# redmod-team/SympGPR

Hardware: AMD Instinct MI355X
Metric: Gram-build GB/s + Cholesky fp64 TFLOP/s at N=65536 d=2; |alpha-alpha_ref|/|alpha_ref| (higher is better)
Workload: dtype f64

## Files before the change

include/sympgpr_probe.h:

```cpp
#ifndef SYMPGPR_PROBE_H
#define SYMPGPR_PROBE_H
#include <stddef.h>
#ifdef __cplusplus
extern "C" {
#endif

int sgpr_probe_mfma_f64(int waves_per_simd, int iters, double *tflops);
int sgpr_probe_hbm_write(size_t bytes, int reps, double *gbs);
int sgpr_probe_mfma_clock(int nacc, int waves_per_simd, int iters, double *out3);
int sgpr_probe_gemm(int m, int n, int k, int lower, double *out4);
int sgpr_probe_gemm_debug(int bits);
int sgpr_probe_leaf(double *out8);
int sgpr_probe_lat(double *out8);
int sgpr_probe_xcc(int nblocks, int *host_out);
int sgpr_probe_cumask(const unsigned *mask_words, int nwords, int nblocks, int *host_out);

int sgpr_probe_generated_eval(int family, int which, int m, const double *xa, const double *ya,
                              const double *xb, const double *yb, const double *l, int nl, double *out);

int sgpr_probe_queue_plan(int n, int nworkers, int *starts_out, int max_starts, unsigned *tasks_out, int max_tasks,
                          int *counts);
int sgpr_probe_queue_plan_partial(int n, int nworkers, int nq, int *starts_out, int max_starts, unsigned *tasks_out,
                                  int max_tasks, int *counts);
int sgpr_probe_queue_trace_begin(int max_tasks);
int sgpr_probe_queue_trace_end(unsigned long long *out, int max_tasks);
int sgpr_probe_queue_trace_clear(void);
int sgpr_probe_queue_postmortem(int always);
int sgpr_probe_queue_force_giveup(int on);
int sgpr_probe_tune(const char *name, double value);
int sgpr_probe_strassen_plan(int m, int n, int k, int lower, long smin, long kslab, long scratch_doubles, long long *out,
                             int max_records, int *count);
int sgpr_probe_gemm_strassen_dev(int m, int n, int k, double alpha, const double *A, size_t lda, const double *B, size_t ldb,
                                 double beta, double *C, size_t ldc, int lower, void *stream);
int sgpr_probe_gemm_nt2_dev(int m, int n, int k, double alpha, const double *A, size_t lda, const double *B, size_t ldb,
                            double beta, double *C, size_t ldc, double alpha2, double *C2, size_t ldc2, void *stream);
int sgpr_probe_strassen2_plan(int m, int n, int k, int lower, long smin, long kslab, long smin2, long kslab2, long scratch_doubles,
                              long long *out, int max_records, int *count);
int sgpr_probe_gemm_nt4_dev(int m, int n, int k, const double *A, size_t lda, const double *B, size_t ldb, double beta, int count,
                            double *const *C, const size_t *ldc, const double *alpha, void *stream);
unsigned sgpr_probe_map_calls(void);
int sgpr_probe_map_team(int ntest, int n0);

int sgpr_probe_trsm_piece(int ticket, int cap, int strips, int out[5]);
int sgpr_probe_trsm_counts(int strips, int cap, unsigned long long out[2]);

int sgpr_probe_census(int na, int threads_a, int lds_a, int spin_a, const unsigned *mask_a, int nwords_a,
                      int nb, int threads_b, int lds_b, int spin_b, const unsigned *mask_b, int nwords_b,
                      unsigned long long *host_out);

#ifdef __cplusplus
}
#endif
#endif
```

sympgpr_amd/_lib.py:

```python
import ctypes as C
import os

import numpy as np

FAMILIES = {"A": 0, "B": 1, "C": 2, "D": 3, "USER": 4}
K_KERN, K_DXDX0, K_DYDY0, K_DXDY0 = 0, 1, 2, 3
K_DLX, K_DLY = 4, 8
K_DX, K_DY, K_DX0, K_DY0, K_DXDX0DY0, K_DYDY0DY0, K_DXDY0DY0 = 16, 17, 18, 19, 20, 21, 22
G_QQ, G_PQ, G_QP, G_PP, G_ALL, G_LOWER, G_OCML, G_DLX, G_DLY = 1, 2, 4, 8, 15, 16, 32, 64, 128
FIT_LOWER_ONLY, FIT_REG, FIT_BLOCK_QQ, FIT_BLOCK_PP = 1, 4, 8, 16
MAP_WRAP_Q, MAP_WRAP_P, MAP_EXPLICIT, MAP_LOSS_NEGP = 1, 2, 4, 8
E_ARG, E_NODEVICE, E_HIP, E_NOMEM, E_STATE = -1, -2, -3, -4, -5

ABI_VERSION = 5
_dp = C.POINTER(C.c_double)
_vp = C.c_void_p


class SympGPRError(RuntimeError):
    code = None
    detail = ""


class NoDeviceError(SympGPRError):
    pass


def lib_path():
    return os.path.join(os.path.dirname(os.path.abspath(__file__)), "lib", "libsympgpr_hip.so")


SIGNATURES = {
    "sgpr_abi_version": (C.c_int, []),
    "sgpr_last_error": (C.c_char_p, []),
    "sgpr_device_count": (C.c_int, []),
    "sgpr_set_device": (C.c_int, [C.c_int]),
    "sgpr_build_k_host": (C.c_int, [C.c_int, C.c_int, C.c_int, _dp, _dp, _dp, _dp, _dp, C.c_int, _dp, C.c_size_t]),
    "sgpr_buildkreg_host": (C.c_int, [C.c_int, C.c_int, C.c_int, _dp, _dp, _dp, _dp, _dp, C.c_int, _dp, C.c_size_t]),
    "sgpr_build_dk_host": (C.c_int, [C.c_int, C.c_int, C.c_int, C.c_int, _dp, _dp, _dp, _dp, _dp, C.c_int, _dp,
                                     C.c_size_t]),
    "sgpr_build_dkreg_host": (C.c_int, [C.c_int, C.c_int, C.c_int, C.c_int, _dp, _dp, _dp, _dp, _dp, C.c_int, _dp,
                                        C.c_size_t]),
    "sgpr_build_k_nd_host": (C.c_int, [C.c_int, C.c_int, C.c_int, C.c_int, _dp, C.c_size_t, _dp, C.c_size_t, _dp,
                                       C.c_int, _dp, C.c_size_t]),
    "sgpr_kernel_eval_host": (C.c_int, [C.c_int, C.c_int, C.c_int, _dp, _dp, _dp, _dp, _dp, C.c_int, _dp]),
    "sgpr_potrf_host": (C.c_int, [C.c_int, _dp, C.c_size_t]),
    "sgpr_potrs_host": (C.c_int, [C.c_int, _dp, C.c_size_t, _dp, C.c_size_t, C.c_int]),
    "sgpr_fit_create": (C.c_int, [C.c_int, C.c_int, _dp, _dp, _dp, _dp, C.c_int, C.c_double, C.c_uint, _vp,
                                  C.POINTER(_vp)]),
    "sgpr_fit_create_nd": (C.c_int, [C.c_int, C.c_int, C.c_int, _dp, C.c_size_t, _dp, _dp, C.c_int, C.c_double,
                                     C.c_uint, _vp, C.POINTER(_vp)]),
    "sgpr_fit_set_hyp": (C.c_int, [_vp, _dp, C.c_int, C.c_double]),
    "sgpr_fit_set_targets": (C.c_int, [_vp, _dp]),
    "sgpr_fit_build": (C.c_int, [_vp]),
    "sgpr_fit_factor": (C.c_int, [_vp]),
    "sgpr_fit_solve": (C.c_int, [_vp]),
    "sgpr_fit_run": (C.c_int, [_vp]),
    "sgpr_fit_alpha": (C.c_int, [_vp, _dp]),
    "sgpr_fit_nll": (C.c_int, [_vp, _dp]),
    "sgpr_fit_ldiag": (C.c_int, [_vp, _dp]),
    "sgpr_fit_get_matrix": (C.c_int, [_vp, _dp, C.c_size_t]),
    "sgpr_fit_solve_rhs": (C.c_int, [_vp, _dp, C.c_size_t, C.c_int]),
    "sgpr_fit_solve_rhs_dev": (C.c_int, [C.c_void_p, C.c_void_p, C.c_size_t, C.c_int]),
    "sgpr_fit_predict_rows": (C.c_int, [_vp, C.c_int, _dp, _dp, _dp, _dp]),
    "sgpr_fit_nll_grad": (C.c_int, [_vp, _dp]),
    "sgpr_fit_nll_grad_terms": (C.c_int, [_vp, _dp]),
    "sgpr_fit_eig": (C.c_int, [_vp, _dp, _dp]),
    "sgpr_syev_host": (C.c_int, [C.c_int, _dp, C.c_size_t, _dp]),
    "sgpr_fit_inverse": (C.c_int, [_vp, _dp, C.c_size_t]),
    "sgpr_fit_predict_nd": (C.c_int, [_vp, C.c_int, _dp, C.c_size_t, _dp]),
    "sgpr_fit_predict_cov": (C.c_int, [_vp, C.c_int, _dp, C.c_size_t, _dp, _dp]),
    "sgpr_fit_predict_genfun": (C.c_int, [_vp, C.c_int, _dp, C.c_size_t, _dp, _dp, _dp]),
    "sgpr_fit_nll_grad_full": (C.c_int, [_vp, _dp, C.c_int]),
    "sgpr_fit_loo": (C.c_int, [_vp, _dp, _dp, _dp, _dp]),
    "sgpr_fit_stage_ms": (C.c_int, [_vp, _dp, _dp, _dp]),
    "sgpr_fit_cond_estimate": (C.c_int, [_vp, C.c_int, _dp]),
    "sgpr_fit_trim": (C.c_int, [_vp]),
    "sgpr_fit_solve_rhs_ms": (C.c_int, [_vp, _dp]),
    "sgpr_potrf_info_dev": (C.c_int, [C.c_int, _vp]),
    "sgpr_trim": (C.c_int, []),
    "sgpr_fit_device_ptrs": (C.c_int, [_vp, C.POINTER(_vp), C.POINTER(C.c_size_t), C.POINTER(_vp)]),
    "sgpr_fit_destroy": (C.c_int, [_vp]),
    "sgpr_gram_pairs_dev": (C.c_int, [C.c_int, C.c_int, C.c_int, _vp, _vp, _vp, _vp, _dp, C.c_int, _vp, _vp, _vp,
                                      _vp, C.c_size_t, C.c_long, C.c_double, C.c_uint, _vp]),
    "sgpr_gram_nd_dev": (C.c_int, [C.c_int, C.c_int, C.c_int, C.c_int, _vp, C.c_size_t, _vp, C.c_size_t, _dp, C.c_int,
                                   _vp, C.c_size_t, C.c_size_t, C.c_size_t, C.c_long, C.c_double, _vp]),
    "sgpr_gram_reg_dev": (C.c_int, [C.c_int, C.c_int, C.c_int, _vp, _vp, _vp, _vp, _dp, C.c_int, _vp, C.c_size_t,
                                    C.c_long, C.c_double, _vp]),
    "sgpr_gram_nd_sel_dev": (C.c_int, [C.c_int, C.c_int, C.c_int, C.c_int, _vp, C.c_size_t, _vp, C.c_size_t, _dp, C.c_int,
                                       _vp, C.c_size_t, C.POINTER(C.c_long), C.POINTER(C.c_long), _vp]),
    "sgpr_potrf_workspace": (C.c_size_t, [C.c_int]),
    "sgpr_potrf_inverses_bytes": (C.c_size_t, [C.c_int]),
    "sgpr_release_device_streams": (C.c_int, [C.c_int]),
    "sgpr_family_has_p": (C.c_int, [C.c_int]),
    "sgpr_potrf_dev": (C.c_int, [C.c_int, _vp, C.c_size_t, _vp, C.c_size_t, _vp, _vp]),
    "sgpr_trsm_rlt_dev": (C.c_int, [C.c_int, C.c_int, _vp, C.c_size_t, _vp, C.c_size_t, _vp, _vp]),
    "sgpr_gemm_nt_dev": (C.c_int, [C.c_int, C.c_int, C.c_int, C.c_double, _vp, C.c_size_t, _vp, C.c_size_t,
                                   C.c_double, _vp, C.c_size_t, C.c_int, C.c_long, _vp]),
    "sgpr_profile_begin": (C.c_int, []),
    "sgpr_profile_end": (C.c_int, [_dp]),
    "sgpr_profile_launches": (C.c_int, [_dp, C.c_int]),
    "sgpr_gemm_nt_bc_dev": (C.c_int, [C.c_int, C.c_int, C.c_int, C.c_double, _vp, C.c_size_t, _vp, C.c_size_t,
                                      C.c_double, _vp, C.c_size_t, C.c_int, C.c_int, C.c_int, C.c_int, C.c_int, _vp]),
    "sgpr_trsv_dev": (C.c_int, [C.c_int, _vp, C.c_size_t, _vp, _vp, C.c_int, _vp]),
    "sgpr_gemv_sub_dev": (C.c_int, [C.c_int, C.c_int, C.c_int, _vp, C.c_size_t, _vp, _vp, _vp]),
    "sgpr_gemm_nn_dev": (C.c_int, [C.c_int, C.c_int, C.c_int, C.c_double, _vp, C.c_size_t, _vp, C.c_size_t, C.c_double, _vp,
                                   C.c_size_t, _vp]),
    "sgpr_trsm_rl_dev": (C.c_int, [C.c_int, C.c_int, _vp, C.c_size_t, _vp, C.c_size_t, _vp, _vp]),
    "sgpr_copy_blocks_dev": (C.c_int, [C.c_int, C.c_int, C.c_int, _vp, C.c_size_t, C.c_size_t, _vp, C.c_size_t, C.c_size_t, _vp]),
    "sgpr_predict_rows_dev": (C.c_int, [C.c_int, C.c_int, _vp, _vp, C.c_int, _vp, _vp, _dp, C.c_int, _vp, _vp, _vp,
                                        _vp]),
    "sgpr_predict_nd_dev": (C.c_int, [C.c_int, C.c_int, C.c_int, _vp, C.c_size_t, C.c_int, _vp, C.c_size_t, _dp, C.c_int,
                                      _vp, _vp, _vp]),
    "sgpr_predict_reg_dev": (C.c_int, [C.c_int, C.c_int, _vp, _vp, C.c_int, _vp, _vp, _dp, C.c_int, _vp, _vp, _vp]),
    "sgpr_applymap_host": (C.c_int, [C.c_int, C.c_int, C.c_int, C.c_int, _dp, C.c_int, C.c_int, _dp, _dp, _dp, _dp,
                                     C.c_int, C.c_int, _dp, _dp, _dp, _dp, _dp, _dp, _dp, _dp]),
    "sgpr_applymap_sections_host": (C.c_int, [C.c_int, C.c_int, C.c_int, C.c_int, C.c_int, C.c_int, _dp, C.c_int, C.c_int, _dp, _dp,
                                              _dp, _dp, C.c_int, C.c_int, _dp, _dp, _dp, _dp, _dp, _dp, _dp, _dp]),
    "sgpr_fit_applymap_nd": (C.c_int, [_vp, C.c_int, C.c_int, C.c_int, _dp, C.c_size_t, _dp, C.c_size_t, _dp, _dp,
                                       C.POINTER(C.c_int)]),
    "sgpr_applymap_nd_host": (C.c_int, [C.c_int, C.c_int, C.c_int, C.c_int, C.c_int, _dp, C.c_int, C.c_int, _dp, C.c_size_t,
                                        _dp, _dp, C.c_size_t, _dp, C.c_size_t, _dp, _dp, C.POINTER(C.c_int)]),
    "sgpr_fit_applymap_nd_tangent": (C.c_int, [_vp, C.c_int, C.c_int, C.c_int, _dp, C.c_size_t, _dp, C.c_size_t, _dp, _dp,
                                               C.POINTER(C.c_int), _dp, _dp, _dp]),
    "sgpr_applymap_nd_tangent_host": (C.c_int, [C.c_int, C.c_int, C.c_int, C.c_int, C.c_int, _dp, C.c_int, C.c_int, _dp,
                                                C.c_size_t, _dp, _dp, C.c_size_t, _dp, C.c_size_t, _dp, _dp, C.POINTER(C.c_int),
                                                _dp, _dp, _dp]),
    "sgpr_potrs_vec_dev": (C.c_int, [C.c_int, _vp, C.c_size_t, _vp, _vp, _vp]),
    "sgpr_solve_status_dev": (C.c_int, [C.c_int, _vp, C.c_size_t, _vp, _vp]),
    "sgpr_fit_batch_max_order": (C.c_int, []),
    "sgpr_fit_batch": (C.c_int, [C.c_int, C.c_int, C.c_int, _dp, _dp, _dp, _dp, C.c_int, _dp, C.c_uint, _dp, _dp,
                                 C.POINTER(C.c_int)]),
    "sgpr_fit_batch_grad": (C.c_int, [C.c_int, C.c_int, C.c_int, _dp, _dp, _dp, _dp, C.c_int, _dp, C.c_uint, _dp, _dp, _dp,
                                      C.POINTER(C.c_int)]),
    "sgpr_fit_batch_grad_mid": (C.c_int, [C.c_int, C.c_int, C.c_int, _dp, _dp, _dp, _dp, C.c_int, _dp, C.c_uint, _dp, _dp, _dp,
                                          C.POINTER(C.c_int)]),
    "sgpr_fit_batch_loo": (C.c_int, [C.c_int, C.c_int, C.c_int, _dp, _dp, _dp, _dp, C.c_int, _dp, C.c_uint, _dp, _dp, _dp,
                                     C.POINTER(C.c_int)]),
}

PROBE_SIGNATURES = {
    "sgpr_probe_mfma_f64": (C.c_int, [C.c_int, C.c_int, _dp]),
    "sgpr_probe_mfma_clock": (C.c_int, [C.c_int, C.c_int, C.c_int, _dp]),
    "sgpr_probe_gemm": (C.c_int, [C.c_int, C.c_int, C.c_int, C.c_int, _dp]),
    "sgpr_probe_gemm_debug": (C.c_int, [C.c_int]),
    "sgpr_probe_leaf": (C.c_int, [_dp]),
    "sgpr_probe_lat": (C.c_int, [_dp]),
    "sgpr_probe_cumask": (C.c_int, [C.POINTER(C.c_uint), C.c_int, C.c_int, C.POINTER(C.c_int)]),
    "sgpr_probe_xcc": (C.c_int, [C.c_int, C.POINTER(C.c_int)]),
    "sgpr_probe_hbm_write": (C.c_int, [C.c_size_t, C.c_int, _dp]),
    "sgpr_probe_generated_eval": (C.c_int, [C.c_int, C.c_int, C.c_int, _dp, _dp, _dp, _dp, _dp, C.c_int, _dp]),
    "sgpr_probe_queue_plan": (C.c_int, [C.c_int, C.c_int, C.POINTER(C.c_int), C.c_int, C.POINTER(C.c_uint), C.c_int,
                                        C.POINTER(C.c_int)]),
    "sgpr_probe_queue_plan_partial": (C.c_int, [C.c_int, C.c_int, C.c_int, C.POINTER(C.c_int), C.c_int, C.POINTER(C.c_uint),
                                                C.c_int, C.POINTER(C.c_int)]),
    "sgpr_probe_queue_trace_begin": (C.c_int, [C.c_int]),
    "sgpr_probe_queue_trace_end": (C.c_int, [C.POINTER(C.c_ulonglong), C.c_int]),
    "sgpr_probe_queue_postmortem": (C.c_int, [C.c_int]),
    "sgpr_probe_queue_force_giveup": (C.c_int, [C.c_int]),
    "sgpr_probe_tune": (C.c_int, [C.c_char_p, C.c_double]),
    "sgpr_probe_map_calls": (C.c_uint, []),
    "sgpr_probe_map_team": (C.c_int, [C.c_int, C.c_int]),
    "sgpr_probe_trsm_piece": (C.c_int, [C.c_int, C.c_int, C.c_int, C.POINTER(C.c_int)]),
    "sgpr_probe_trsm_counts": (C.c_int, [C.c_int, C.c_int, C.POINTER(C.c_ulonglong)]),
    "sgpr_probe_queue_trace_clear": (C.c_int, []),
    "sgpr_probe_strassen_plan": (C.c_int, [C.c_int, C.c_int, C.c_int, C.c_int, C.c_long, C.c_long, C.c_long,
                                           C.POINTER(C.c_longlong), C.c_int, C.POINTER(C.c_int)]),
    "sgpr_probe_gemm_strassen_dev": (C.c_int, [C.c_int, C.c_int, C.c_int, C.c_double, C.c_void_p, C.c_size_t, C.c_void_p, C.c_size_t,
                                               C.c_double, C.c_void_p, C.c_size_t, C.c_int, C.c_void_p]),
    "sgpr_probe_gemm_nt2_dev": (C.c_int, [C.c_int, C.c_int, C.c_int, C.c_double, C.c_void_p, C.c_size_t, C.c_void_p, C.c_size_t,
                                          C.c_double, C.c_void_p, C.c_size_t, C.c_double, C.c_void_p, C.c_size_t, C.c_void_p]),
    "sgpr_probe_strassen2_plan": (C.c_int, [C.c_int, C.c_int, C.c_int, C.c_int, C.c_long, C.c_long, C.c_long, C.c_long, C.c_long,
                                            C.POINTER(C.c_longlong), C.c_int, C.POINTER(C.c_int)]),
    "sgpr_probe_gemm_nt4_dev": (C.c_int, [C.c_int, C.c_int, C.c_int, C.c_void_p, C.c_size_t, C.c_void_p, C.c_size_t, C.c_double, C.c_int,
                                          C.POINTER(C.c_void_p), C.POINTER(C.c_size_t), C.POINTER(C.c_double), C.c_void_p]),
    "sgpr_probe_census": (C.c_int, [C.c_int, C.c_int, C.c_int, C.c_int, C.POINTER(C.c_uint), C.c_int,
                                    C.c_int, C.c_int, C.c_int, C.c_int, C.POINTER(C.c_uint), C.c_int,
                                    C.POINTER(C.c_ulonglong)]),
}

_LIB = None
_PROBE = None


def load_library():
    global _LIB
    if _LIB is not None:
        return _LIB
    path = lib_path()
    if os.environ.get("SYMPGPR_NO_TORCH_PRELOAD") != "1":
        try:
            import torch
        except ImportError:
            pass
    if not os.path.exists(path):
        raise SympGPRError("%s is missing: run `python -c 'import __graft_entry__ as g; g.build()'` "
                           "(or make -C sympgpr_amd/csrc); there is no CPU fallback" % path)
    lib = C.CDLL(path)
    for name, (res, args) in SIGNATURES.items():
        fn = getattr(lib, name)
        fn.restype = res
        fn.argtypes = args
    if lib.sgpr_abi_version() != ABI_VERSION:
        raise SympGPRError("ABI version mismatch: %s is version %d, this package binds version %d -- rebuild it "
                           "(make -C sympgpr_amd/csrc)" % (path, lib.sgpr_abi_version(), ABI_VERSION))
    _LIB = lib
    import atexit
    atexit.register(_release_streams_at_exit)
    return lib


def _release_streams_at_exit():
    lib = _LIB
    if lib is None:
        return
    try:
        for dev in range(max(0, lib.sgpr_device_count())):
            lib.sgpr_release_device_streams(dev)
    except Exception:
        pass


def load_probe_library():
    global _PROBE
    if _PROBE is not None:
        return _PROBE
    load_library()
    path = os.path.join(os.path.dirname(lib_path()), "libsympgpr_probe.so")
    if not os.path.exists(path):
        raise SympGPRError("%s is missing: run make -C sympgpr_amd/csrc" % path)
    lib = C.CDLL(path)
    for name, (res, args) in PROBE_SIGNATURES.items():
        fn = getattr(lib, name)
        fn.restype = res
        fn.argtypes = args
    _PROBE = lib
    return lib


def device_count():
    return load_library().sgpr_device_count()


def check(rc, what=""):
    if rc == 0:
        return
    if rc > 0:
        raise np.linalg.LinAlgError("%d-th leading minor of the array is not positive definite" % rc)
    msg = load_library().sgpr_last_error().decode(errors="replace")
    err = (NoDeviceError(msg) if rc == E_NODEVICE else
           SympGPRError("%s failed (%d): %s" % (what or "libsympgpr_hip call", rc, msg)))
    err.code, err.detail = rc, msg
    raise err


def dptr(a):
    return a.ctypes.data_as(_dp)


def f64(a):
    return np.ascontiguousarray(np.asarray(a, dtype=np.float64))


def family_has_p(fam):
    return bool(load_library().sgpr_family_has_p(family_id(fam)))


def family_id(fam):
    if isinstance(fam, str):
        return FAMILIES[fam]
    return int(fam)
```

sympgpr_amd/csrc/chol.hip:

```cpp
#include <algorithm>
#include <cstdlib>
#include <mutex>
#include <vector>

#include "cholq.h"
#include "common.h"
#include "gemm_tile.h"
#include "leaf.h"

namespace sgpr {

namespace {

using namespace leaf;


__global__ __launch_bounds__(LT) void leaf_kernel(int nb, double *A, size_t lda, double *inv,
                                                  int *dinfo, int goff, int mode,
                                                  unsigned long long *stamps)
{
    __shared__ double s[LEAF_LDS];
    if (nb == LEAF) leaf_body(s, (int)LEAF, A, lda, inv, dinfo, goff, mode, stamps);
    else            leaf_body(s, nb, A, lda, inv, dinfo, goff, mode, stamps);
}
// ... 472 lines not shown
            __syncthreads();
        };
        auto wait_helper = [&](int cp) -> bool {
            if (!((helped >> cp) & 1u)) return true;
            idx[0] = F0 + cp * PW_MAX + g;
            return panel_wait_ge(a.flags, idx, 1, 3, a.dinfo, sh + 1, a.abort);
        };
        for (int c = 0; c + 1 < g; ++c) {
            double *X = tileptr(g, c);
            XTile x;
            CTile cd;
            if (!wait_helper(c)) return false;
            asm volatile("s_waitcnt vmcnt(0)" ::: "memory");
            __syncthreads();
            trsm_prefetch(X, a.lda, x);
            diag_prefetch(tileptr(g, g), a.lda, cd);
            idx[0] = E0 + c;
            if (!panel_wait(a.flags, idx, 1, a.dinfo, sh + 1, a.abort)) return false;
            trsm_solve(s, tileptr(c, c), a.inv + (size_t)c * LEAF * LEAF, a.lda, x);
            trsm_store(X, a.lda, x);
            panel_publish_wt(a.flags + F0 + g * PW_MAX + c);
            diag_update_global(s, x, cd, tileptr(g, g), a.lda);
            if (c == 0 && a.NH > 0) claim_tiles();
            int cnt = 0;
            for (int cc = c + 1; cc < g; ++cc)
                if (!((helped >> cc) & 1u)) idx[cnt++] = F0 + cc * PW_MAX + c;
            if (cnt && !panel_wait(a.flags, idx, cnt, a.dinfo, sh + 1, a.abort)) return false;
            for (int t = 1; t < g - c; ++t)
                if (!((helped >> (c + t)) & 1u))
                    panel_product(s, -1.0, X, a.lda, tileptr(c + t, c), a.lda, 1.0, tileptr(g, c + t), a.lda);
        }
        if (g > 0) {
            const int c = g - 1;
            double *X = tileptr(g, c);
            XTile x;
            CTile cd;
            if (!wait_helper(c)) return false;
            asm volatile("s_waitcnt vmcnt(0)" ::: "memory");
            __syncthreads();
            trsm_prefetch(X, a.lda, x);
            diag_prefetch(tileptr(g, g), a.lda, cd);
            idx[0] = E0 + c;
            if (dbg) a.dbg[16 * g + 2] = __builtin_amdgcn_s_memrealtime();
            if (!panel_wait(a.flags, idx, 1, a.dinfo, sh + 1, a.abort)) return false;
            if (dbg) a.dbg[16 * g + 0] = __builtin_amdgcn_s_memrealtime();
            trsm_solve(s, tileptr(c, c), a.inv + (size_t)c * LEAF * LEAF, a.lda, x, a.dbg ? a.dbg + 16 * g + 6 : nullptr);
            trsm_store(X, a.lda, x);
            if (dbg) a.dbg[16 * g + 1] = __builtin_amdgcn_s_memrealtime();
            diag_update_into_leaf(s, x, cd, a.dbg ? a.dbg + 16 * g + 8 : nullptr);
            if (tid == 0) __hip_atomic_store((gint *)(a.flags + F0 + g * PW_MAX + c), 1, __ATOMIC_RELAXED, __HIP_MEMORY_SCOPE_AGENT);
        }
        asm volatile("s_waitcnt vmcnt(0)" ::: "memory");
        __syncthreads();
        if (dbg) a.dbg[16 * g + 4] = __builtin_amdgcn_s_memrealtime();
        leaf_body(s, (int)LEAF, tileptr(g, g), a.lda,
                  a.inv + (size_t)g * LEAF * LEAF, a.dinfo, a.goff + g * LEAF, (int)LEAF_FACTOR, nullptr,
                  a.flags + E0 + g, g > 0, dbg ? a.dbg + 16 * g + 11 : nullptr);
        panel_publish(a.flags + 2 + g);
        if (a.abort && tid == 0)
            __hip_atomic_fetch_add((gint *)(a.abort + (cholq::Q_PROG - cholq::Q_ABORT)), 1, __ATOMIC_RELAXED, __HIP_MEMORY_SCOPE_AGENT);
        if (dbg) a.dbg[16 * g + 5] = __builtin_amdgcn_s_memrealtime();
        if (cen && tid == 0) cen[2] = __builtin_amdgcn_s_memrealtime();
        return true;
    }
    if (g < W + a.NH) {
        int h = g - W, cp = 1, gg = 2;
        while (h >= W - 1 - cp) { h -= W - 1 - cp; ++cp; }
        gg = cp + 1 + h;
        int *word = a.flags + F0 + cp * PW_MAX + gg;
        if (tid == 0) sh[1] = atomicCAS(word, 0, 1);
        __syncthreads();
        const int old = sh[1];
        __syncthreads();
        if (old != 0) return true;
        if (a.ver) {
            idx[0] = ((a.ver_i0 + (gg >> 1)) * a.ver_ld + a.ver_j0 + cp) * (int)cholq::VS;
            if (!panel_wait_ge(a.ver, idx, 1, a.ver_need, a.dinfo, sh + 1, a.abort)) return false;
        }
        for (int c = 0; c < cp; ++c) {
            idx[0] = F0 + gg * PW_MAX + c;
            idx[1] = F0 + cp * PW_MAX + c;
            if (!panel_wait(a.flags, idx, 2, a.dinfo, sh + 1, a.abort)) return false;
            panel_product(s, -1.0, tileptr(gg, c), a.lda, tileptr(cp, c), a.lda, 1.0, tileptr(gg, cp), a.lda);
        }
        panel_publish_val(word, 3);
        return true;
    }
    const int gb = g - a.NH;
    if (a.tiles) {
        const int nbel = R - W, ntiles = nbel * W;
        int *const counter = a.flags + 2 * PFLAG_STRIDE - 1;
        for (;;) {
            if (tid == 0) sh[1] = atomicAdd(counter, 1);
            __syncthreads();
            const int q = sh[1];
            __syncthreads();
            if (q >= ntiles) return true;
            const int cp = q / nbel, r = W + q % nbel;
            const int pword = PFLAG_STRIDE + (r - W);
            if (a.ver) {
                idx[0] = ((a.ver_i0 + (r >> 1)) * a.ver_ld + a.ver_j0 + cp) * (int)cholq::VS;
                if (!panel_wait_ge(a.ver, idx, 1, a.ver_need, a.dinfo, sh + 1, a.abort)) return false;
            }
            for (int c = 0; c < cp; ++c) {
                idx[0] = pword;
                if (!panel_wait_ge(a.flags, idx, 1, c + 1, a.dinfo, sh + 1, a.abort)) return false;
                idx[0] = F0 + cp * PW_MAX + c;
                if (!panel_wait(a.flags, idx, 1, a.dinfo, sh + 1, a.abort)) return false;
                panel_product(s, -1.0, tileptr(r, c), a.lda, tileptr(cp, c), a.lda, 1.0, tileptr(r, cp), a.lda);
            }
            {
                double *X = tileptr(r, cp);
                XTile x;
                asm volatile("s_waitcnt vmcnt(0)" ::: "memory");
                __syncthreads();
                trsm_prefetch(X, a.lda, x);
                idx[0] = E0 + cp;
                if (!panel_wait(a.flags, idx, 1, a.dinfo, sh + 1, a.abort)) return false;
                trsm_solve(s, tileptr(cp, cp), a.inv + (size_t)cp * LEAF * LEAF, a.lda, x);
                trsm_store(X, a.lda, x);
            }
            asm volatile("s_waitcnt vmcnt(0)" ::: "memory");
            __syncthreads();
            if (tid == 0) __hip_atomic_store((gint *)(a.flags + pword), cp + 1, __ATOMIC_RELAXED, __HIP_MEMORY_SCOPE_AGENT);
            if (cp == W - 1) {
                if (a.tver) panel_publish_val(a.tver + (size_t)(a.tver_r0 + r) * cholq::VS, a.tver_val);
                if (a.abort && tid == 0)
                    __hip_atomic_fetch_add((gint *)(a.abort + (cholq::Q_PROG - cholq::Q_ABORT)), 1, __ATOMIC_RELAXED, __HIP_MEMORY_SCOPE_AGENT);
            }
        }
    }
    const int nw = G - W;
    const int r_first = W + (gb - W), r_step = nw > 0 ? nw : R;
    if (a.ver) {
        const int vi = a.ver_i0 + (r_first >> 1);
        for (int c = 0; c < W; ++c) idx[c] = (vi * a.ver_ld + a.ver_j0 + c) * (int)cholq::VS;
        if (r_first < R && !panel_wait_ge(a.ver, idx, W, a.ver_need, a.dinfo, sh + 1, a.abort)) return false;
    }
    const bool below_early = a.below_early != 0;
    for (int c = 0; c < W; ++c) {
        bool have_inv = false, have_early = false, have_rows = false;
        for (int r = r_first; r < R; r += r_step) {
            double *X = tileptr(r, c);
            if (c == W - 1 || below_early) {
                XTile x;
                asm volatile("s_waitcnt vmcnt(0)" ::: "memory");
                __syncthreads();
                trsm_prefetch(X, a.lda, x);
                if (!have_early) {
                    idx[0] = E0 + c;
                    if (!panel_wait(a.flags, idx, 1, a.dinfo, sh + 1, a.abort)) return false;
                    have_early = true;
                }
                trsm_solve(s, tileptr(c, c), a.inv + (size_t)c * LEAF * LEAF, a.lda, x);
                trsm_store(X, a.lda, x);
                if (c == W - 1) continue;
            } else {
                if (!have_inv) {
                    idx[0] = 2 + c;
                    if (!panel_wait(a.flags, idx, 1, a.dinfo, sh + 1, a.abort)) return false;
                    have_inv = true;
                }
                panel_product(s, 1.0, X, a.lda, a.inv + (size_t)c * LEAF * LEAF, (size_t)LEAF, 0.0, X, a.lda);
            }
            for (int t = 1; t <= W - 1 - c; ++t) {
                if (t == 1 && !have_rows) {
                    int cnt = 0;
                    for (int cc = c + 1; cc < W; ++cc) idx[cnt++] = F0 + cc * PW_MAX + c;
                    if (cnt && !panel_wait(a.flags, idx, cnt, a.dinfo, sh + 1, a.abort)) return false;
                    have_rows = true;
                }
                panel_product(s, -1.0, X, a.lda, tileptr(c + t, c), a.lda, 1.0, tileptr(r, c + t), a.lda);
            }
        }
    }
    if (a.tver && r_first < R) panel_publish_val(a.tver + (size_t)(a.tver_r0 + r_first) * cholq::VS, a.tver_val);
    if (a.abort && tid == 0)
        __hip_atomic_fetch_add((gint *)(a.abort + (cholq::Q_PROG - cholq::Q_ABORT)), 1, __ATOMIC_RELAXED, __HIP_MEMORY_SCOPE_AGENT);
    if (cen && tid == 0) cen[2] = __builtin_amdgcn_s_memrealtime();
    return true;
}

__global__ __launch_bounds__(LT) void panel_kernel(const PanelArgs a)
{
    __shared__ double s[LEAF * ILD];
    __shared__ int sh[2];
    static_assert(2 * tile::BK * 2 * (LEAF + tile::PAD) <= LEAF_LDS && LEAF_LDS <= LEAF * ILD, "product staging and the leaf fit the buffer");
    const int tid = threadIdx.x;
    const int W = a.W, G = a.G;
    if (tid == 0) {
        int t = -1;
        if ((blockIdx.x & 7) == 0) {
            t = atomicAdd(a.flags, 1);
            if (t >= W) t = -1;
        }
        if (t < 0) t = W + atomicAdd(a.flags + 1, 1);
        sh[0] = t;
    }
    __syncthreads();
    const int g = sh[0];
    __syncthreads();
    if (g >= G + a.NH) return;
    (void)panel_strip(a, g, s, sh);
}

struct PanelSeq {
    double *A;
    size_t lda;
    int nblk;
    int nblk_all;
    const int *pstart;
    double *inv;
    int *dinfo;
    int goff;
    int *flags;
    const int *ver;
    int ver_ld;
    int *tver;
    int *abort;
    unsigned long long *census;
    int helpers, tiles;
};

__global__ __launch_bounds__(LT) void panel_seq_kernel(const PanelSeq q)
{
    __shared__ double s[LEAF * ILD];
    __shared__ int sh[2];
    const int g = blockIdx.x;
    for (int k = 0; k < q.nblk; ++k) {
        const int k0 = q.pstart[k], w = q.pstart[k + 1] - k0, wnext = k + 1 < q.nblk_all ? q.pstart[k + 2] - q.pstart[k + 1] : 0;
        PanelArgs a{};
        a.P = q.A + k0 + (size_t)k0 * q.lda; a.lda = q.lda;
        a.W = w / LEAF;
        a.R = a.G = (w + wnext) / LEAF;
        a.below_early = q.tiles;
        a.NH = (q.helpers && a.W > 2 && a.G + (a.W - 1) * (a.W - 2) / 2 <= (int)gridDim.x) ? (a.W - 1) * (a.W - 2) / 2 : 0;
        if (q.tiles && wnext > 0 && a.W >= 2 && (int)gridDim.x - a.W - a.NH >= 1) {
            a.tiles = 1;
            a.G = a.W + min((int)gridDim.x - a.W - a.NH, (a.R - a.W) * a.W);
        }
        a.inv = q.inv + (size_t)(k0 / LEAF) * LEAF * LEAF;
        a.dinfo = q.dinfo; a.goff = q.goff + k0;
        a.flags = q.flags + (size_t)(k0 / LEAF) * PFLAG_STRIDE;
        a.dbg = nullptr;
        a.ver = q.ver; a.ver_ld = q.ver_ld; a.ver_i0 = k0 / cholq::TM; a.ver_j0 = k0 / cholq::TN; a.ver_need = k0 / LEAF;
        a.tver = q.tver; a.tver_r0 = k0 / LEAF; a.tver_val = (k0 + w) / LEAF;
        a.abort = q.abort;
        a.census = (q.census && k < (int)cholq::TRACE_PANELS) ? q.census + 4 * cholq::TRACE_PANEL_WGS * (size_t)k : nullptr;
        if (g < a.G + a.NH && !panel_strip(a, g, s, sh)) return;
        asm volatile("s_waitcnt vmcnt(0)" ::: "memory");
        __syncthreads();
    }
}

struct PanelBatch {
    double *A;
    size_t stride_a, lda;
    double *inv;
    size_t stride_inv;
    int *flags;
    int *info;
    int *ticket;
    int W, nbatch;
    int R;
    int k0;
    int G;
};

__global__ __launch_bounds__(LT) void panel_batch_kernel(const PanelBatch q)
{
    __shared__ double s[LEAF * ILD];
    __shared__ int sh[2];
    if (threadIdx.x == 0) sh[0] = atomicAdd(q.ticket, 1);
    __syncthreads();
    const int t = sh[0];
    __syncthreads();
    const int p = t / q.G, g = t - p * q.G;
    if (p >= q.nbatch) return;
    PanelArgs a{};
    a.P = q.A + (size_t)p * q.stride_a + (size_t)q.k0 + (size_t)q.k0 * q.lda; a.lda = q.lda;
    a.W = q.W; a.R = q.R; a.G = q.G;
    a.inv = q.inv + (size_t)p * q.stride_inv + (size_t)(q.k0 / (int)LEAF) * LEAF * LEAF;
    a.dinfo = q.info + p; a.goff = q.k0;
    a.flags = q.flags + (size_t)p * PFLAG_STRIDE;
    a.below_early = 1;
    (void)panel_strip(a, g, s, sh);
}

inline int split(int n)
{
    int n1 = ((n / 2 + LEAF - 1) / LEAF) * LEAF;
    if (n1 >= n) n1 -= LEAF;
    return n1;
}

struct Ctx {
    double *inv;
    int *dinfo;
    hipStream_t st;
    int la_max = 0;
    int *flags = nullptr;
    void *qws = nullptr;
    bool strassen = false;
};

int potrf_lookahead(int n, double *A, size_t lda, const Ctx &c, int nb, int off0);
inline int la_block(int n) { return n <= 4096 ? 256 : (n <= 24576 ? 512 : (n <= 40960 ? 1024 : 2048)); }

int trsm_rec(int m, int n, const double *L, size_t ldl, double *B, size_t ldb, int off, const Ctx &c)
{
    if (n <= LEAF) {
        return gemm_nt(m, n, n, 1.0, B, ldb, c.inv + (size_t)(off / LEAF) * LEAF * LEAF, LEAF, 0.0,
                       B, ldb, 0, 0, c.st);
    }
    const int n1 = split(n), n2 = n - n1;
    int rc = trsm_rec(m, n1, L, ldl, B, ldb, off, c);
    if (rc) return rc;
    if (c.strassen) rc = gemm_nt_strassen(m, n2, n1, -1.0, B, ldb, L + n1, ldl, 1.0, B + (size_t)n1 * ldb, ldb, 0, c.st);
    else            rc = gemm_nt(m, n2, n1, -1.0, B, ldb, L + n1, ldl, 1.0, B + (size_t)n1 * ldb, ldb, 0, 0, c.st);
    if (rc) return rc;
    return trsm_rec(m, n2, L + n1 + (size_t)n1 * ldl, ldl, B + (size_t)n1 * ldb, ldb, off + n1, c);
}

int trsm_rl_rec(int m, int n, const double *L, size_t ldl, double *B, size_t ldb, int off, const Ctx &c)
{
    if (n <= LEAF)
        return gemm_nn(m, n, n, 1.0, B, ldb, c.inv + (size_t)(off / LEAF) * LEAF * LEAF, LEAF, 0.0, B, ldb, c.st);
    const int n1 = split(n), n2 = n - n1;
    int rc = trsm_rl_rec(m, n2, L + n1 + (size_t)n1 * ldl, ldl, B + (size_t)n1 * ldb, ldb, off + n1, c);
    if (rc) return rc;
    rc = gemm_nn(m, n1, n2, -1.0, B + (size_t)n1 * ldb, ldb, L + n1, ldl, 1.0, B, ldb, c.st);
    if (rc) return rc;
    return trsm_rl_rec(m, n1, L, ldl, B, ldb, off, c);
}

int potrf_rec(int n, double *A, size_t lda, int off, const Ctx &c)
{
    if (n <= LEAF) {
        hipLaunchKernelGGL(leaf_kernel, dim3(1), dim3(LT), 0, c.st, n, A, lda,
                           c.inv + (size_t)(off / LEAF) * LEAF * LEAF, c.dinfo, off, (int)LEAF_FACTOR,
                           (unsigned long long *)nullptr);
        SGPR_CHECK_LAUNCH();
        return 0;
    }
    if (n > 4 * LEAF && n <= c.la_max) return potrf_lookahead(n, A, lda, c, 0, off);
    const int n1 = split(n), n2 = n - n1;
    double *A21 = A + n1, *A22 = A + n1 + (size_t)n1 * lda;
    int rc = potrf_rec(n1, A, lda, off, c);
    if (rc) return rc;
    rc = trsm_rec(n2, n1, A, lda, A21, lda, off, c);
    if (rc) return rc;
    if (c.strassen) rc = gemm_nt_strassen(n2, n2, n1, -1.0, A21, lda, A21, lda, 1.0, A22, lda, 1, c.st);
    else            rc = gemm_nt(n2, n2, n1, -1.0, A21, lda, A21, lda, 1.0, A22, lda, 1, 0, c.st);
    if (rc) return rc;
    return potrf_rec(n2, A22, lda, off + n1, c);
}

int trsv_n_rec(int n, const double *L, size_t ldl, double *b, int off, const Ctx &c)
{
    if (n <= LEAF) {
        hipLaunchKernelGGL(leaf_matvec_kernel, dim3(1), dim3(MV_T), 0, c.st, n,
                           c.inv + (size_t)(off / LEAF) * LEAF * LEAF, b, 0);
        SGPR_CHECK_LAUNCH();
        return 0;
    }
    if (n <= TRSV_BLOCK) {
        hipLaunchKernelGGL(trsv_block_kernel, dim3(1), dim3(MV_T), 0, c.st, n, L, ldl,
                           c.inv + (size_t)(off / LEAF) * LEAF * LEAF, b, 0);
        SGPR_CHECK_LAUNCH();
        return 0;
    }
    const int n1 = split(n), n2 = n - n1;
    int rc = trsv_n_rec(n1, L, ldl, b, off, c);
    if (rc) return rc;
    rc = gemv_n_sub(n2, n1, L + n1, ldl, b, b + n1, c.st);
    if (rc) return rc;
    return trsv_n_rec(n2, L + n1 + (size_t)n1 * ldl, ldl, b + n1, off + n1, c);
}

int trsv_t_rec(int n, const double *L, size_t ldl, double *b, int off, const Ctx &c)
{
    if (n <= LEAF) {
        hipLaunchKernelGGL(leaf_matvec_kernel, dim3(1), dim3(MV_T), 0, c.st, n,
                           c.inv + (size_t)(off / LEAF) * LEAF * LEAF, b, 1);
        SGPR_CHECK_LAUNCH();
        return 0;
    }
    if (n <= TRSV_BLOCK) {
        hipLaunchKernelGGL(trsv_block_kernel, dim3(1), dim3(MV_T), 0, c.st, n, L, ldl,
                           c.inv + (size_t)(off / LEAF) * LEAF * LEAF, b, 1);
        SGPR_CHECK_LAUNCH();
        return 0;
    }
    const int n1 = split(n), n2 = n - n1;
    int rc = trsv_t_rec(n2, L + n1 + (size_t)n1 * ldl, ldl, b + n1, off + n1, c);
    if (rc) return rc;
    rc = gemv_t_sub(n2, n1, L + n1, ldl, b + n1, b, c.st);
    if (rc) return rc;
    return trsv_t_rec(n1, L, ldl, b, off, c);
}

int leaves_invert_only(int n, double *L, size_t ldl, const Ctx &c)
{
    for (int off = 0; off < n; off += LEAF) {
        const int nb = n - off < LEAF ? n - off : LEAF;
        hipLaunchKernelGGL(leaf_kernel, dim3(1), dim3(LT), 0, c.st, nb, L + off + (size_t)off * ldl, ldl,
                           c.inv + (size_t)(off / LEAF) * LEAF * LEAF, c.dinfo, off,
                           (int)LEAF_INVERT_ONLY, (unsigned long long *)nullptr);
        SGPR_CHECK_LAUNCH();
    }
    return 0;
}

inline size_t inv_bytes(int n)
{
    return (size_t)((n + LEAF - 1) / LEAF) * LEAF * LEAF * sizeof(double);
}
inline size_t flag_bytes(int n)
{
    return (((size_t)((n + LEAF - 1) / LEAF) * PFLAG_STRIDE * sizeof(int)) + 255) / 256 * 256;
}


}

inline size_t pub_bytes(int n) { return ((size_t)2 * n * sizeof(double) + 255) / 256 * 256; }
size_t potrf_workspace(int n) { return n <= 0 ? 256 : inv_bytes(n) + flag_bytes(n) + pub_bytes(n) + cholq::ws_bytes(n) + 256; }

namespace {

struct EventPool {
    std::vector<hipEvent_t> ev;
    size_t top = 0;
};
thread_local EventPool t_event_pool[64];

struct EventSet {
    std::vector<hipEvent_t> ev;
    EventPool *pool = nullptr;
    size_t base = 0;
    int create(size_t count)
    {
        int dev = 0;
        SGPR_HIP(hipGetDevice(&dev));
        if (dev < 0 || dev >= 64) { set_error("potrf: device index out of range"); return SGPR_E_ARG; }
        pool = &t_event_pool[dev];
        base = pool->top;
        while (pool->ev.size() < base + count) {
            hipEvent_t e = nullptr;
            SGPR_HIP(hipEventCreateWithFlags(&e, hipEventDisableTiming));
            pool->ev.push_back(e);
        }
        pool->top = base + count;
        ev.assign(pool->ev.begin() + (long)base, pool->ev.begin() + (long)(base + count));
        return 0;
    }
    ~EventSet()
    {
        if (pool) pool->top = base;
    }
};
struct StreamJoin {
    hipStream_t side, caller;
    hipEvent_t ev;
    ~StreamJoin()
    {
        if (hipEventRecord(ev, side) != hipSuccess || hipStreamWaitEvent(caller, ev, 0) != hipSuccess)
            (void)hipStreamSynchronize(side);
        gemm_set_overlap(0);
    }
};

hipStream_t g_side[64] = {};
std::mutex g_side_mu;

void release_all_streams_at_exit();
void register_exit_release()
{
    static std::once_flag once;
    std::call_once(once, [] { (void)atexit(release_all_streams_at_exit); });
}

int side_stream(hipStream_t caller, hipStream_t *out, int *dev_out)
{
    hipStream_t *const side = g_side;
    int dev = -1;
    if (caller) {
        SGPR_HIP(hipStreamGetDevice(caller, &dev));
    } else {
        SGPR_HIP(hipGetDevice(&dev));
    }
    if (dev < 0 || dev >= 64) { set_error("potrf: device index out of range"); return SGPR_E_ARG; }
    std::lock_guard<std::mutex> lock(g_side_mu);
    if (!side[dev]) {
        int cur = -1, lo = 0, hi = 0;
        SGPR_HIP(hipGetDevice(&cur));
        if (cur != dev) SGPR_HIP(hipSetDevice(dev));
        hipError_t e = hipDeviceGetStreamPriorityRange(&lo, &hi);
        if (e == hipSuccess) e = hipStreamCreateWithPriority(&side[dev], hipStreamNonBlocking, hi);
        if (e == hipSuccess) register_exit_release();
        if (cur != dev) (void)hipSetDevice(cur);
        SGPR_HIP(e);
    }
    *out = side[dev];
    *dev_out = dev;
    return 0;
}

struct QueueDevice {
    std::mutex mu;
    hipEvent_t done = nullptr;
    int ncu = 0;
    hipStream_t workers[4] = {}, panels[4] = {};
    bool overlap_ok[4] = {};
    bool failed = false;
};
QueueDevice g_qdev[64];

__global__ void overlap_probe_kernel(int *w, int me)
{
    __hip_atomic_store((gint *)(w + me), 1, __ATOMIC_RELAXED, __HIP_MEMORY_SCOPE_AGENT);
    const unsigned long long t0 = __builtin_amdgcn_s_memrealtime();
    int seen = 0;
    while (!(seen = __hip_atomic_load((gint *)(w + 1 - me), __ATOMIC_RELAXED, __HIP_MEMORY_SCOPE_AGENT))) {
        __builtin_amdgcn_s_sleep(32);
        if (__builtin_amdgcn_s_memrealtime() - t0 > 5000000ull) break;
    }
    w[2 + me] = seen ? 1 : 2;
}
static bool queue_overlap_ok(hipStream_t sw, hipStream_t sp)
{
    int *w = nullptr;
    if (hipMalloc((void **)&w, 4 * sizeof(int)) != hipSuccess) { (void)hipGetLastError(); return false; }
    int h[4] = {0, 0, 0, 0};
    bool ok = hipMemset(w, 0, sizeof(h)) == hipSuccess;
    if (ok) {
        hipLaunchKernelGGL(overlap_probe_kernel, dim3(1), dim3(1), 0, sp, w, 0);
        hipLaunchKernelGGL(overlap_probe_kernel, dim3(1), dim3(1), 0, sw, w, 1);
        ok = hipGetLastError() == hipSuccess && hipStreamSynchronize(sp) == hipSuccess && hipStreamSynchronize(sw) == hipSuccess &&
             hipMemcpy(h, w, sizeof(h), hipMemcpyDeviceToHost) == hipSuccess && h[2] == 1 && h[3] == 1;
    }
    (void)hipFree(w);
    (void)hipGetLastError();
    return ok;
}

int queue_streams(QueueDevice &qd, int dev, int R, hipStream_t *sw, hipStream_t *sp)
{
    if (!qd.workers[R - 1]) {
        int cur = -1;
        SGPR_HIP(hipGetDevice(&cur));
        if (cur != dev) SGPR_HIP(hipSetDevice(dev));
        const int words = qd.ncu / 32;
        std::vector<uint32_t> mp((size_t)words, 0u), mw((size_t)words, 0xFFFFFFFFu);
        for (int b = 0; b < 8 * R; ++b) { mp[b / 32] |= 1u << (b % 32); mw[b / 32] &= ~(1u << (b % 32)); }
        hipError_t e = hipExtStreamCreateWithCUMask(&qd.panels[R - 1], (uint32_t)words, mp.data());
        if (e == hipSuccess) e = hipExtStreamCreateWithCUMask(&qd.workers[R - 1], (uint32_t)words, mw.data());
        if (e == hipSuccess) register_exit_release();
        if (cur != dev) (void)hipSetDevice(cur);
        if (e != hipSuccess) {
            (void)hipGetLastError();
            qd.failed = true;
            return SGPR_E_HIP;
        }
    }
    if (!qd.overlap_ok[R - 1]) {
        if (!queue_overlap_ok(qd.workers[R - 1], qd.panels[R - 1])) {
            qd.failed = true;
            return SGPR_E_HIP;
        }
        qd.overlap_ok[R - 1] = true;
    }
    *sw = qd.workers[R - 1];
    *sp = qd.panels[R - 1];
    return 0;
}

thread_local bool t_last_potrf_used_queue = false;

int potrf_queue(int n, double *A, size_t lda, const Ctx &c, int off0)
{
    int dev = -1;
    if (c.st) {
        SGPR_HIP(hipStreamGetDevice(c.st, &dev));
    } else {
        SGPR_HIP(hipGetDevice(&dev));
    }
    if (dev < 0 || dev >= 64) { set_error("potrf: device index out of range"); return SGPR_E_ARG; }
    QueueDevice &qd = g_qdev[dev];
    std::lock_guard<std::mutex> lock(qd.mu);
    if (qd.failed) return 1;
    if (!qd.ncu) {
        SGPR_HIP(hipDeviceGetAttribute(&qd.ncu, hipDeviceAttributeMultiprocessorCount, dev));
        SGPR_HIP(hipEventCreateWithFlags(&qd.done, hipEventDisableTiming));
        SGPR_HIP(hipEventRecord(qd.done, c.st));
    }
    if (qd.ncu % 64 != 0 || qd.ncu < 64) { qd.failed = true; return 1; }
    const std::vector<int> starts = cholq::default_starts(n);
    int band = 0;
    for (size_t k = 0; k + 1 < starts.size(); ++k)
        band = std::max(band, (starts[k + 1] - starts[k] + (k + 2 < starts.size() ? starts[k + 2] - starts[k + 1] : 0)) / LEAF);
    static const int q_helpers = (int)tune("q_helpers", 0), q_tiles = (int)tune("q_tiles", 0);
    int nh_max = 0;
    for (size_t k = 0; k + 1 < starts.size(); ++k) {
        const int W = (starts[k + 1] - starts[k]) / LEAF;
        if (q_helpers && W > 2) nh_max = std::max(nh_max, (W - 1) * (W - 2) / 2);
    }
    const int pgrid = band + nh_max + std::max(0, q_tiles);
    const int R = (pgrid + 7) / 8;
    if (R > 4) return 1;
    hipStream_t sw = nullptr, sp = nullptr;
    if (queue_streams(qd, dev, R, &sw, &sp)) return 1;
    static const int qslack = (int)tune("q_slack", 0);
    const int nworkers = qd.ncu - 8 * R - std::max(0, std::min(qslack, 64));
    const cholq::Plan *plan = cholq::get_plan(n, nworkers);
    if (!plan) return 1;
    const cholq::Ws ws = cholq::carve(c.qws, n);
    const hipStream_t su = c.st;
    int rc;
    SGPR_HIP(hipStreamWaitEvent(su, qd.done, 0));
    if ((rc = cholq::prepare(*plan, ws, su))) return rc;
    if (cholq::forced_giveup()) {
        static const int k_timeout = POTRF_HANDOFF_TIMEOUT;
        SGPR_HIP(hipMemcpyAsync(c.dinfo, &k_timeout, sizeof(int), hipMemcpyHostToDevice, su));
    }
    EventSet es;
    if ((rc = es.create(3))) return rc;
    const int tn = n / cholq::TN;
    double *inv_blk = c.inv + (size_t)(off0 / LEAF) * LEAF * LEAF;
    int *flags_blk = c.flags + (size_t)(off0 / LEAF) * PFLAG_STRIDE;
    {
        SGPR_HIP(hipEventRecord(es.ev[0], su));
        SGPR_HIP(hipStreamWaitEvent(sp, es.ev[0], 0));
        SGPR_HIP(hipStreamWaitEvent(sw, es.ev[0], 0));
        StreamJoin join_p{sp, su, es.ev[1]};
        StreamJoin join_w{sw, su, es.ev[2]};
        PanelSeq ps{};
        ps.A = A; ps.lda = lda; ps.nblk = plan->nq; ps.nblk_all = plan->nblk; ps.pstart = ws.pstart;
        ps.inv = inv_blk; ps.dinfo = c.dinfo; ps.goff = off0; ps.flags = flags_blk;
        ps.ver = ws.ver; ps.ver_ld = tn; ps.tver = ws.tver; ps.abort = cholq::abort_word(ws);
        ps.census = cholq::trace_panel_base((int)(plan->tasks.size() / 2));
        ps.helpers = q_helpers != 0; ps.tiles = q_tiles > 0;
        t_last_potrf_used_queue = true;
        hipLaunchKernelGGL(panel_seq_kernel, dim3(pgrid), dim3(LT), 0, sp, ps);
        SGPR_CHECK_LAUNCH();
        if ((rc = cholq::launch_workers(*plan, ws, A, lda, inv_blk, flags_blk, c.dinfo, PFLAG_STRIDE, sw))) return rc;
    }
    SGPR_HIP(hipEventRecord(qd.done, su));
    cholq::remember(ws, n, (int)(plan->tasks.size() / 2));
    cholq::remember_plan(plan);
    static const bool qdebug = tune("q_debug", 0) != 0;
    if (qdebug) {
        SGPR_HIP(hipStreamSynchronize(su));
        cholq::postmortem(false);
    }
    if (plan->nq < plan->nblk) {
        const int S = plan->starts[plan->nq];
        Ctx ct = c;
        ct.qws = nullptr;
        static const bool nosync = tune("q_nosync", 0) != 0;
        if (!nosync) SGPR_HIP(hipStreamSynchronize(su));
        return potrf_lookahead(n - S, A + S + (size_t)S * lda, lda, ct, 0, off0 + S);
    }
    return 0;
}

void release_all_streams_at_exit()
{
    int ndev = 0;
    if (hipGetDeviceCount(&ndev) != hipSuccess) { (void)hipGetLastError(); return; }
    for (int dev = 0; dev < ndev && dev < 64; ++dev) {
        hipStream_t drop[9] = {};
        int nd = 0;
        {
            std::lock_guard<std::mutex> lock(g_side_mu);
            if (g_side[dev]) { drop[nd++] = g_side[dev]; g_side[dev] = nullptr; }
        }
        {
            QueueDevice &qd = g_qdev[dev];
            std::lock_guard<std::mutex> lock(qd.mu);
            for (int r = 0; r < 4; ++r) {
                if (qd.workers[r]) { drop[nd++] = qd.workers[r]; qd.workers[r] = nullptr; }
                if (qd.panels[r]) { drop[nd++] = qd.panels[r]; qd.panels[r] = nullptr; }
            }
            qd.failed = true;
        }
        if (!nd) continue;
        int cur = -1;
        (void)hipGetDevice(&cur);
        if (cur != dev) (void)hipSetDevice(dev);
        for (int q = 0; q < nd; ++q) (void)hipStreamDestroy(drop[q]);
        if (cur != dev && cur >= 0) (void)hipSetDevice(cur);
    }
    (void)hipGetLastError();
}

int release_streams(int dev)
{
    {
        bool any = false;
        {
            std::lock_guard<std::mutex> lock(g_side_mu);
            any = g_side[dev] != nullptr;
        }
        QueueDevice &qd = g_qdev[dev];
        std::lock_guard<std::mutex> lock(qd.mu);
        for (int r = 0; r < 4; ++r) any = any || qd.workers[r] || qd.panels[r];
        any = any || qd.done;
        if (!any) return 0;
    }
    int cur = -1;
    SGPR_HIP(hipGetDevice(&cur));
    if (cur != dev) SGPR_HIP(hipSetDevice(dev));
    hipError_t first = hipSuccess;
    auto drop = [&](hipStream_t &s) {
        if (!s) return;
        hipError_t e = hipStreamSynchronize(s);
        if (e == hipSuccess) e = hipStreamDestroy(s);
        if (e != hipSuccess && first == hipSuccess) first = e;
        s = nullptr;
    };
    {
        std::lock_guard<std::mutex> lock(g_side_mu);
        drop(g_side[dev]);
    }
    {
        QueueDevice &qd = g_qdev[dev];
        std::lock_guard<std::mutex> lock(qd.mu);
        for (int r = 0; r < 4; ++r) { drop(qd.workers[r]); drop(qd.panels[r]); }
        if (qd.done) {
            const hipError_t e = hipEventDestroy(qd.done);
            if (e != hipSuccess && first == hipSuccess) first = e;
            qd.done = nullptr;
        }
        qd.ncu = 0;
        qd.failed = false;
        for (int r = 0; r < 4; ++r) qd.overlap_ok[r] = false;
    }
    if (cur != dev) (void)hipSetDevice(cur);
    SGPR_HIP(first);
    return 0;
}

int potrf_lookahead(int n, double *A, size_t lda, const Ctx &c, int nb, int off0)
{
    if (nb == 0 && c.qws && c.flags && cholq::eligible(n) && (lda & 1) == 0 && (((uintptr_t)A & 15) == 0) && off0 % LEAF == 0) {
        const int rq = potrf_queue(n, A, lda, c, off0);
        if (rq <= 0) return rq;
    }
    hipStream_t sp = nullptr;
    {
        int dev = -1;
        const int rc0 = side_stream(c.st, &sp, &dev);
        if (rc0) return rc0;
    }
    static const int pmode = (int)tune("la_panel", 3);
    const bool fused_cap = pmode == 3 && c.flags && n % LEAF == 0 && (lda & 1) == 0 && (((uintptr_t)A & 15) == 0) &&
                           off0 % LEAF == 0;
    std::vector<int> starts;
    {
        static const int t0_env = (int)tune("la_t0", 0);
        const int t0 = t0_env > 0 ? t0_env : (n >= 24576 ? 12288 : 1 << 30);
        static const int t1 = (int)tune("la_t1", 6144);
        static const int t2 = (int)tune("la_t2", 2048);
        for (int pos = 0; pos < n;) {
            starts.push_back(pos);
            const int rem = n - pos;
            int w = nb > 0 ? nb : (rem > t0 ? 2048 : (rem > t1 ? 1024 : (rem > t2 ? 512 : 256)));
            if (nb == 0 && !fused_cap) w = la_block(n);
            pos += std::min(w, rem);
        }
        starts.push_back(n);
    }
    const int nblk = (int)starts.size() - 1;
    int wmax = 0;
    for (int k = 0; k < nblk; ++k) wmax = std::max(wmax, starts[k + 1] - starts[k]);
    EventSet es;
    {
        const int rc0 = es.create(3 * (size_t)nblk + 3);
        if (rc0) return rc0;
    }
    std::vector<hipEvent_t> &ev = es.ev;
    const hipStream_t su = c.st;
    Ctx cp{c.inv, c.dinfo, sp, 0, c.flags};
    const bool fused_ok = fused_cap && wmax % LEAF == 0 && wmax / LEAF <= PW_MAX;
    const bool left = pmode != 2, right_in = pmode == 0 || pmode == 3;
    auto panel = [&](int k) -> int {
        const int k0 = starts[k], w = starts[k + 1] - k0, rows = n - k0, below = rows - w;
        double *Akk = A + k0 + (size_t)k0 * lda;
        if (fused_ok) {
            PanelArgs pa{};
            pa.P = Akk; pa.lda = lda;
            pa.R = rows / LEAF; pa.W = w / LEAF;
            const int nbelow = pa.R - pa.W;
            const double m_u2 = (double)(rows + w);
            const double u2_us = k > 0 ? m_u2 * m_u2 * (starts[k] - starts[k - 1]) / 55e6 : 0.0;
            static const double split_ratio = tune("panel_split_ratio", 3.0);
            const bool split = nbelow > 0 && k > 0 && u2_us > split_ratio * (125.0 * pa.W + 100.0);
            if (split) {
                pa.R = pa.W;
                pa.G = pa.W;
            } else {
                const double strip_us = 30.0 * (pa.W * (pa.W + 1) / 2 + pa.W), chain_us = 125.0 * pa.W;
                int per_wg = (int)((0.7 * u2_us - 0.5 * chain_us) / strip_us);
                per_wg = std::max(1, std::min(per_wg, 4));
                const int nwg = std::min((nbelow + per_wg - 1) / per_wg, PANEL_G_MAX - pa.W);
                pa.G = pa.W + (nbelow > 0 ? std::max(1, nwg) : 0);
            }
            static const bool helpers_on = tune("panel_helpers", 1) != 0, below_early_on = tune("panel_below_early", 1) != 0;
            pa.NH = helpers_on && pa.W > 2 ? (pa.W - 1) * (pa.W - 2) / 2 : 0;
            if (pa.G + pa.NH > PANEL_G_MAX) pa.NH = 0;
            pa.below_early = below_early_on ? 1 : 0;
            static const bool tiles_on = tune("panel_tiles", 1) != 0;
            static const double tile_mult = tune("panel_tile_mult", 1.0);
            if (tiles_on && !split && nbelow > 0 && pa.W >= 2 && nbelow < PFLAG_STRIDE) {
                const double chain_us = 60.0 * pa.W + 50.0;
                int nt = u2_us < chain_us ? nbelow * pa.W : (int)(tile_mult * (pa.G - pa.W));
                nt = std::max(1, std::min(std::min(nt, nbelow * pa.W), PANEL_G_MAX - pa.W - pa.NH));
                pa.tiles = 1;
                pa.G = pa.W + nt;
            }
            const int t0 = (off0 + k0) / LEAF;
            pa.inv = cp.inv + (size_t)t0 * LEAF * LEAF;
            pa.dinfo = cp.dinfo; pa.goff = off0 + k0;
            pa.flags = c.flags + (size_t)t0 * PFLAG_STRIDE;
            pa.dbg = (PANEL_DBG && g_panel_dbg) ? g_panel_dbg + (size_t)16 * t0 : nullptr;
            hipLaunchKernelGGL(panel_kernel, dim3(std::max(pa.G + pa.NH, 8 * (pa.W - 1) + 1)), dim3(LT), 0, sp, pa);
            SGPR_CHECK_LAUNCH();
            if (split) return trsm_rec(below, w, Akk, lda, Akk + w, lda, off0 + k0, cp);
            return 0;
        }
        if (!left) {
            int rc = potrf_rec(w, Akk, lda, off0 + k0, cp);
            if (rc) return rc;
            if (below > 0) rc = trsm_rec(below, w, Akk, lda, Akk + w, lda, off0 + k0, cp);
            return rc;
        }
        for (int c0 = 0; c0 < w; c0 += LEAF) {
            const int nj = std::min((int)LEAF, w - c0), mrows = rows - c0;
            double *Pj = Akk + c0 + (size_t)c0 * lda;
            int rc;
            if (!right_in && c0 > 0 &&
                (rc = gemm_nt(mrows, nj, c0, -1.0, Akk + c0, lda, Akk + c0, lda, 1.0, Pj, lda, 0, 0, sp)))
                return rc;
            double *invj = cp.inv + (size_t)((off0 + k0 + c0) / LEAF) * LEAF * LEAF;
            hipLaunchKernelGGL(leaf_kernel, dim3(1), dim3(LT), 0, sp, nj, Pj, lda, invj, cp.dinfo, off0 + k0 + c0,
                               (int)LEAF_FACTOR, (unsigned long long *)nullptr);
            SGPR_CHECK_LAUNCH();
            if (mrows > nj && (rc = gemm_nt(mrows - nj, nj, nj, 1.0, Pj + nj, lda, invj, LEAF, 0.0, Pj + nj, lda, 0, 0, sp)))
                return rc;
            const int ncols = w - c0 - nj;
            if (right_in && ncols > 0 &&
                (rc = gemm_nt(mrows - nj, ncols, nj, -1.0, Pj + nj, lda, Pj + nj, lda, 1.0, Pj + nj + (size_t)nj * lda, lda, 1, 0, sp)))
                return rc;
        }
        return 0;
    };
    int rc;
    SGPR_HIP(hipEventRecord(ev[2 * nblk], su));
    SGPR_HIP(hipStreamWaitEvent(sp, ev[2 * nblk], 0));
    StreamJoin join{sp, su, ev[2 * nblk + 1]};
    gemm_set_overlap(1);
    if ((rc = panel(0))) return rc;
    SGPR_HIP(hipEventRecord(ev[0], sp));
    for (int k = 0; k < nblk; ++k) {
        const int k0 = starts[k], w = starts[k + 1] - k0;
        const int k1 = k0 + w;
        if (k1 >= n) break;
        const int w1 = starts[k + 2] - k1, k2 = k1 + w1;
        const double *Lk = A + (size_t)k0 * lda;
        if (k > 0) SGPR_HIP(hipStreamWaitEvent(sp, ev[2 * (k - 1) + 1], 0));
        if ((rc = gemm_nt(n - k1, w1, w, -1.0, Lk + k1, lda, Lk + k1, lda, 1.0, A + k1 + (size_t)k1 * lda, lda, 1, 0, sp)))
            return rc;
        const double u2_us = (double)(n - k2) * (n - k2) * w / 55e6;
        const bool chain_bound = u2_us < 1.5 * (125.0 * (w1 / LEAF) + 100.0);
        if (chain_bound) SGPR_HIP(hipEventRecord(ev[2 * nblk + 2 + k], sp));
        if ((rc = panel(k + 1))) return rc;
        SGPR_HIP(hipEventRecord(ev[2 * (k + 1)], sp));
        SGPR_HIP(hipStreamWaitEvent(su, chain_bound ? ev[2 * nblk + 2 + k] : ev[2 * k], 0));
        if (k2 < n &&
            (rc = gemm_nt(n - k2, n - k2, w, -1.0, Lk + k2, lda, Lk + k2, lda, 1.0, A + k2 + (size_t)k2 * lda, lda, 1, 0, su)))
            return rc;
        SGPR_HIP(hipEventRecord(ev[2 * k + 1], su));
    }
    return 0;
}

}

size_t potrf_batch_flag_bytes(int nbatch) { return ((size_t)nbatch * PFLAG_STRIDE + 1) * sizeof(int); }
int potrf_batch_max_order() { return PW_MAX * (int)LEAF; }

int potrf_batch(int nbatch, int npad, double *A, size_t stride_a, size_t lda, double *inv, size_t stride_inv, int *flags,
                int *info, hipStream_t st)
{
    if (nbatch < 0 || npad <= 0 || npad % LEAF != 0 || npad > PW_MAX * (int)LEAF || lda < (size_t)npad || (lda & 1) != 0 ||
        ((uintptr_t)A & 15) != 0 || (stride_a & 1) != 0) {
        set_error("potrf_batch: bad order / leading dimension / alignment");
        return SGPR_E_ARG;
    }
    if (nbatch == 0) return 0;
    SGPR_HIP(hipMemsetAsync(info, 0, (size_t)nbatch * sizeof(int), st));
    return potrf_batch_panel(nbatch, npad, 0, npad / (int)LEAF, A, stride_a, lda, inv, stride_inv, flags, info, st);
}

int potrf_batch_panel(int nbatch, int npad, int k0, int Wd, double *A, size_t stride_a, size_t lda, double *inv, size_t stride_inv,
                      int *flags, int *info, hipStream_t st)
{
    const int R = (npad - k0) / (int)LEAF;
    if (nbatch <= 0 || k0 < 0 || k0 % LEAF != 0 || Wd < 1 || Wd > PW_MAX || Wd > R || R > PANEL_G_MAX) {
        set_error("potrf_batch_panel: bad panel");
        return SGPR_E_ARG;
    }
    SGPR_HIP(hipMemsetAsync(flags, 0, potrf_batch_flag_bytes(nbatch), st));
    const int below_max = (int)tune("batch_below", 0);
    const int below = R - Wd <= 0 ? 0 : (below_max > 0 && below_max < R - Wd ? below_max : R - Wd);
    PanelBatch q{A, stride_a, lda, inv, stride_inv, flags, info, flags + (size_t)nbatch * PFLAG_STRIDE, Wd, nbatch, R, k0, Wd + below};
    hipLaunchKernelGGL(panel_batch_kernel, dim3((unsigned)(nbatch * (Wd + below))), dim3(LT), 0, st, q);
    SGPR_CHECK_LAUNCH();
    return 0;
}

bool potrf_queue_mark_failed(hipStream_t st)
{
    const bool used = t_last_potrf_used_queue;
    if (!used) return false;
    int dev = -1;
    if ((st ? hipStreamGetDevice(st, &dev) : hipGetDevice(&dev)) != hipSuccess || dev < 0 || dev >= 64) { (void)hipGetLastError(); return false; }
    QueueDevice &qd = g_qdev[dev];
    std::lock_guard<std::mutex> lock(qd.mu);
    qd.failed = true;
    return true;
}

int potrf_trim()
{
    for (int dev = 0; dev < 64; ++dev) {
        EventPool &p = t_event_pool[dev];
        if (p.ev.empty() || p.top != 0) continue;
        for (hipEvent_t e : p.ev) (void)hipEventDestroy(e);
        p.ev.clear();
    }
    (void)hipGetLastError();
    return strassen_trim();
}

int release_device_streams(int dev)
{
    if (dev < 0 || dev >= 64) { set_error("release_device_streams: device index out of range"); return SGPR_E_ARG; }
    return release_streams(dev);
}

int potrf(int n, double *A, size_t lda, void *work, size_t lwork, int *dinfo, hipStream_t st)
{
    if (n < 0 || (n > 0 && lda < (size_t)n)) { set_error("potrf: bad n / lda"); return SGPR_E_ARG; }
    if (lwork < potrf_workspace(n)) { set_error("potrf: workspace too small"); return SGPR_E_ARG; }
    SGPR_HIP(hipMemsetAsync(dinfo, 0, sizeof(int), st));
    if (n == 0) return 0;
    int *flags = reinterpret_cast<int *>(static_cast<char *>(work) + inv_bytes(n));
    SGPR_HIP(hipMemsetAsync(flags, 0, flag_bytes(n), st));
    static const int mode = [] { const char *e = getenv("SGPR_POTRF"); return !e ? 0 : (e[0] == 'r' ? 1 : 2); }();
    static const int nb_env = [] { const char *e = getenv("SGPR_POTRF_NB"); return e ? atoi(e) : 0; }();
    static const int la_max_env = [] { const char *e = getenv("SGPR_LA_MAX"); return (int)tune("la_max", e ? atoi(e) : 57344); }();
    t_last_potrf_used_queue = false;
    Ctx c{static_cast<double *>(work), dinfo, st, mode == 1 ? 0 : la_max_env, flags};
    if (cholq::ws_bytes(n) > 0) c.qws = static_cast<char *>(work) + inv_bytes(n) + flag_bytes(n) + pub_bytes(n);
    c.strassen = true;
    if (n > c.la_max && n > LEAF) {
        const int n1 = split(n), n2 = n - n1, n11 = split(n1);
        auto need = [&](int levels) {
            return std::max(strassen_scratch_doubles(n2, n2, n1, 1, levels), strassen_scratch_doubles(n2, n1 - n11, n11, 0, levels));
        };
        strassen_reserve(need(2), need(1), st);
    }
    const bool dbg = PANEL_DBG && getenv("SGPR_PANEL_DBG") != nullptr;
    const int T = (n + LEAF - 1) / LEAF;
    if (dbg) {
        (void)hipMalloc((void **)&g_panel_dbg, sizeof(unsigned long long) * 16 * T);
        (void)hipMemset(g_panel_dbg, 0, sizeof(unsigned long long) * 16 * T);
    }
    int rc;
    if (mode == 2 || (nb_env > 0 && mode == 0 && n > 4 * LEAF && n <= c.la_max))
        rc = potrf_lookahead(n, A, lda, c, nb_env > 0 ? nb_env : 0, 0);
    else
        rc = potrf_rec(n, A, lda, 0, c);
    if (dbg) {
        (void)hipStreamSynchronize(st);
        std::vector<unsigned long long> h(16 * (size_t)T);
        (void)hipMemcpy(h.data(), g_panel_dbg, h.size() * 8, hipMemcpyDeviceToHost);
        (void)hipFree(g_panel_dbg);
        g_panel_dbg = nullptr;
        std::vector<double> d[9];
        for (int t = 1; t + 1 < T; ++t) {
            const unsigned long long *p = &h[16 * t], *q = &h[16 * (t + 1)];
            if (!p[0] || !p[5] || !q[0]) continue;
            d[0].push_back((p[1] - p[0]) * 0.01);
            d[1].push_back((p[2] - p[1]) * 0.01);
            d[2].push_back((p[3] - p[2]) * 0.01);
            d[3].push_back((p[4] - p[3]) * 0.01);
            d[4].push_back(((double)q[0] - (double)p[4]) * 0.01);
            d[5].push_back((p[5] - p[4]) * 0.01);
            d[3].back() = ((double)p[4] - (double)p[1]) * 0.01;
            d[1].back() = (p[6] - p[0]) * 0.01;
            d[2].back() = (p[7] - p[6]) * 0.01;
            d[6].push_back((p[11] - p[4]) * 0.01);
            d[7].push_back((p[12] - p[11]) * 0.01);
            d[8].push_back(((double)q[2] - (double)p[4]) * 0.01);
            if (getenv("SGPR_PANEL_DBG_ALL"))
                fprintf(stderr, "  col %3d: leaf entry -> factor %.1f -> flag %.1f | next strip at wait %.1f, saw E %.1f | its solve %.1f, update %.1f\n", t,
                        (p[11] - p[4]) * 0.01, (p[12] - p[4]) * 0.01, ((double)q[2] - (double)p[4]) * 0.01, ((double)q[0] - (double)p[4]) * 0.01,
                        (q[1] - q[0]) * 0.01, ((double)q[4] - (double)q[1]) * 0.01);
        }
        auto med = [](std::vector<double> &x) { std::sort(x.begin(), x.end()); return x.empty() ? 0.0 : x[x.size() / 2]; };
        fprintf(stderr, "panel chain n=%d (%zu columns): E seen -> solve stored %.1f | E seen -> staged %.1f | -> MFMA part done %.1f | (solve stored -> leaf entry %.1f) | "
                "leaf entry -> next E seen %.1f (factor %.1f, -> flag set %.1f; next strip at its wait %.1f) | whole leaf %.1f us\n", n, d[0].size(), med(d[0]), med(d[1]), med(d[2]), med(d[3]), med(d[4]),
                med(d[6]), med(d[7]), med(d[8]), med(d[5]));
    }
    return rc;
}

int trsm_rlt(int m, int n, const double *L, size_t ldl, double *B, size_t ldb, const void *work,
             hipStream_t st)
{
    if (m <= 0 || n <= 0) return 0;
    Ctx c{const_cast<double *>(static_cast<const double *>(work)), nullptr, st};
    return trsm_rec(m, n, L, ldl, B, ldb, 0, c);
}

static bool use_strips(int n, const double *L, size_t ldl)
{
    static const bool off = [] { const char *e = getenv("SGPR_TRSV"); return e && e[0] == 'r'; }();
    return !off && n > TRSV_BLOCK && trsv_strips_ok(n, L, ldl);
}
static int *solve_state(int n, const void *work)
{
    return reinterpret_cast<int *>(const_cast<char *>(static_cast<const char *>(work)) + inv_bytes(n));
}
static double *solve_pub(int n, const void *work)
{
    return reinterpret_cast<double *>(const_cast<char *>(static_cast<const char *>(work)) + inv_bytes(n) + flag_bytes(n));
}

bool trsv_uses_strips(int n, const double *L, size_t ldl) { return use_strips(n, L, ldl); }

int solve_status(int n, const double *L, size_t ldl, const void *work, hipStream_t st)
{
    if (n <= 0 || !use_strips(n, L, ldl)) { SGPR_HIP(hipStreamSynchronize(st)); return 0; }
    int h[8] = {};
    SGPR_HIP(hipMemcpyAsync(h, solve_state(n, work), sizeof(h), hipMemcpyDeviceToHost, st));
    SGPR_HIP(hipStreamSynchronize(st));
    if (h[2] || h[6]) { set_error("triangular solve: a hand-off between strips timed out"); return SGPR_E_HIP; }
    return 0;
}
const int *trsv_state(int n, const void *work) { return solve_state(n, work); }

int potrs_vec(int n, const double *L, size_t ldl, void *work, double *b, hipStream_t st)
{
    if (n <= 0) return 0;
    Ctx c{const_cast<double *>(static_cast<const double *>(work)), nullptr, st};
    if (use_strips(n, L, ldl)) {
        int *state = solve_state(n, work);
        double *pub = solve_pub(n, work);
        SGPR_HIP(hipMemsetAsync(state, 0, 8 * sizeof(int), st));
        SGPR_HIP(hipMemsetAsync(pub, 0xFF, (size_t)2 * n * sizeof(double), st));
        int rc = trsv_strips(n, L, ldl, c.inv, b, 0, state, pub, st);
        if (rc) return rc;
        return trsv_strips(n, L, ldl, c.inv, b, 1, state + 4, pub + n, st);
    }
    int rc = trsv_n_rec(n, L, ldl, b, 0, c);
    if (rc) return rc;
    return trsv_t_rec(n, L, ldl, b, 0, c);
}

int trsm_rl(int m, int n, const double *L, size_t ldl, double *B, size_t ldb, const void *work, hipStream_t st)
{
    if (m <= 0 || n <= 0) return 0;
    Ctx c{const_cast<double *>(static_cast<const double *>(work)), nullptr, st};
    return trsm_rl_rec(m, n, L, ldl, B, ldb, 0, c);
}

int trsm_rlt_off(int m, int n, const double *L, size_t ldl, double *B, size_t ldb, const void *work, int off, hipStream_t st)
{
    if (m <= 0 || n <= 0) return 0;
    if (off < 0 || off % (int)LEAF) { set_error("trsm_rlt_off: offset not on a leaf boundary"); return SGPR_E_ARG; }
    Ctx c{const_cast<double *>(static_cast<const double *>(work)), nullptr, st};
    return trsm_rec(m, n, L, ldl, B, ldb, off, c);
}
int trsm_rl_off(int m, int n, const double *L, size_t ldl, double *B, size_t ldb, const void *work, int off, hipStream_t st)
{
    if (m <= 0 || n <= 0) return 0;
    if (off < 0 || off % (int)LEAF) { set_error("trsm_rl_off: offset not on a leaf boundary"); return SGPR_E_ARG; }
    Ctx c{const_cast<double *>(static_cast<const double *>(work)), nullptr, st};
    return trsm_rl_rec(m, n, L, ldl, B, ldb, off, c);
}

bool potrs_mat_uses_strips(int n, int nrhs, const double *L, size_t ldl)
{
    return nrhs >= 2 && nrhs <= 256 && use_strips(n, L, ldl) && trsm_strips_ok(n, L, ldl);
}
size_t potrs_mat_scratch(int n, int nrhs, const double *L, size_t ldl)
{
    if (n <= 0 || nrhs <= 0) return 8;
    return potrs_mat_uses_strips(n, nrhs, L, ldl) ? trsm_strips_scratch(n) : (size_t)n * nrhs * sizeof(double);
}

int potrs_mat(int n, const double *L, size_t ldl, const void *work, double *B, size_t ldb, int nrhs,
              double *scratch, hipStream_t st)
{
    if (n <= 0 || nrhs <= 0) return 0;
    if (potrs_mat_uses_strips(n, nrhs, L, ldl))
        return potrs_strips(n, L, ldl, static_cast<const double *>(work), B, ldb, nrhs, solve_state(n, work), scratch, st);
    int rc = transpose(n, nrhs, B, ldb, scratch, (size_t)nrhs, st);
    if (rc) return rc;
    if ((rc = trsm_rlt(nrhs, n, L, ldl, scratch, (size_t)nrhs, work, st))) return rc;
    if ((rc = trsm_rl(nrhs, n, L, ldl, scratch, (size_t)nrhs, work, st))) return rc;
    return transpose(nrhs, n, scratch, (size_t)nrhs, B, ldb, st);
}

int potrs_mat_fwd(int n, const double *L, size_t ldl, const void *work, double *B, size_t ldb, int nrhs,
                  double *scratch, hipStream_t st)
{
    if (n <= 0 || nrhs <= 0) return 0;
    if (potrs_mat_uses_strips(n, nrhs, L, ldl))
        return trsm_strips_fwd(n, L, ldl, static_cast<const double *>(work), B, ldb, nrhs, solve_state(n, work), scratch, st);
    int rc = transpose(n, nrhs, B, ldb, scratch, (size_t)nrhs, st);
    if (rc) return rc;
    if ((rc = trsm_rlt(nrhs, n, L, ldl, scratch, (size_t)nrhs, work, st))) return rc;
    return transpose(nrhs, n, scratch, (size_t)nrhs, B, ldb, st);
}

int trsv(int n, const double *L, size_t ldl, void *work, double *b, int trans, hipStream_t st)
{
    if (n <= 0) return 0;
    Ctx c{const_cast<double *>(static_cast<const double *>(work)), nullptr, st};
    if (use_strips(n, L, ldl)) {
        int *state = solve_state(n, work);
        double *pub = solve_pub(n, work);
        SGPR_HIP(hipMemsetAsync(state, 0, 4 * sizeof(int), st));
        SGPR_HIP(hipMemsetAsync(pub, 0xFF, (size_t)n * sizeof(double), st));
        return trsv_strips(n, L, ldl, c.inv, b, trans, state, pub, st);
    }
    return trans ? trsv_t_rec(n, L, ldl, b, 0, c) : trsv_n_rec(n, L, ldl, b, 0, c);
}

int leaf_probe(double *A, size_t lda, double *inv, int *dinfo, unsigned long long *stamps, hipStream_t st)
{
    hipLaunchKernelGGL(leaf_kernel, dim3(1), dim3(LT), 0, st, (int)LEAF, A, lda, inv, dinfo, 0, (int)LEAF_FACTOR, stamps);
    SGPR_CHECK_LAUNCH();
    return 0;
}

int leaf_inverses(int n, const double *L, size_t ldl, void *work, int *dinfo, hipStream_t st)
{
    if (n <= 0) return 0;
    Ctx c{static_cast<double *>(work), dinfo, st};
    return leaves_invert_only(n, const_cast<double *>(L), ldl, c);
}

}
```

sympgpr_amd/csrc/common.h:

```cpp
#pragma once
#include <hip/hip_runtime.h>
#include <cstddef>
#include <cstdint>
#include <string>
#include <type_traits>
#include <vector>

#include "../../include/sympgpr_hip.h"

namespace sgpr {

void set_error(const std::string &msg);
double tune(const char *name, double dflt);
void tune_set(const char *name, double v);
int hip_fail(hipError_t e, const char *what, const char *file, int line);

#define SGPR_HIP(call)                                                          \
    do {                                                                        \
        hipError_t e__ = (call);                                                \
        if (e__ != hipSuccess) return ::sgpr::hip_fail(e__, #call, __FILE__, __LINE__); \
    } while (0)

#define SGPR_CHECK_LAUNCH() SGPR_HIP(hipGetLastError())

struct KConst {
    double lx, ly, p, sig;
    double lx2, ly2;
    double inv_lx2, inv_ly2;
    double cxx, cyy, cxy;
    double hscale;
    double inv_lx, inv_ly, inv_lx3, inv_ly3;
    double gxx;
};
enum { DERIV_NONE = 0, DERIV_LX = 1, DERIV_LY = 2 };
int make_kconst(int family, const double *hyp, int nhyp, KConst *out);
bool family_has_p(int family);
int make_kconst_l(int family, const double *l, int nl, KConst *out);

template <typename F>
int dispatch_family(int family, F &&f)
{
    switch (family) {
    case SGPR_FAM_A: return f(std::integral_constant<int, SGPR_FAM_A>());
    case SGPR_FAM_B: return f(std::integral_constant<int, SGPR_FAM_B>());
    case SGPR_FAM_C: return f(std::integral_constant<int, SGPR_FAM_C>());
    case SGPR_FAM_D: return f(std::integral_constant<int, SGPR_FAM_D>());
    case SGPR_FAM_USER: return f(std::integral_constant<int, SGPR_FAM_USER>());
    }
    set_error("unknown kernel family");
    return SGPR_E_ARG;
}

int gram_pairs(int family, int mi, int mj, const double *xb, const double *yb, const double *xa,
               const double *ya, const KConst &kc, double *qq, double *Pq, double *qP, double *PP,
               size_t ld, long diag_off, double noise, unsigned flags, hipStream_t st);
int gram_reg(int family, int mi, int mj, const double *xb, const double *yb, const double *xa,
             const double *ya, const KConst &kc, double *G, size_t ld, long diag_off, double noise,
             hipStream_t st, int deriv = DERIV_NONE);
int kernel_eval(int family, int which, int m, const double *xa, const double *ya, const double *xb,
                const double *yb, const KConst &kc, double *out, hipStream_t st);
int predict_rows(int family, int m, const double *q, const double *P, int n0, const double *xtr,
                 const double *ytr, const KConst &kc, const double *alpha, double *out_p,
                 double *out_q, hipStream_t st);
int predict_reg(int family, int m, const double *q, const double *P, int n0, const double *xtr,
                const double *ytr, const KConst &kc, const double *alpha, double *out,
                hipStream_t st);

int applymap_team(int ntest, int n0);
size_t applymap_team_ws(int ntest, int n0);
int applymap(int family, int mode, int nm, int ntest, int n0, const double *xtr, const double *ytr,
             const KConst &kc, const double *alpha, int n0p, const double *xtrp, const double *ytrp,
             const KConst &kcp, const double *alphap, const double *Q0, const double *P0, double *qmap,
             double *pmap, double *pdiff, void *team_ws, hipStream_t st);
int applymap_status(const void *team_ws, int ntest, int n0);
unsigned applymap_last_calls();
int applymap_sections(int family, int mode, int nsec, int first, int nm, int ntest, int n0, const double *xtr, const double *ytr,
                      const double *alpha, const KConst *kcs, int n0p, const double *xtrp, const double *ytrp,
                      const double *alphap, const KConst *kcps, const double *Q0, const double *P0, double *qmap, double *pmap,
                      double *pdiff, hipStream_t st);

int gram_nd(int family, int d, int mi, int mj, const double *Xb, size_t ldxb, const double *Xa, size_t ldxa,
            const double *hyp, int nhyp, double *K, size_t ld, size_t rstride, size_t cstride, long diag_off,
            double noise, hipStream_t st);
int gram_nd_sel(int family, int d, int mi, int mj, const double *Xb, size_t ldxb, const double *Xa, size_t ldxa,
                const double *hyp, int nhyp, double *K, size_t ld, const long *roff, const long *coff, hipStream_t st);
int predict_nd(int family, int d, int m, const double *Xt, size_t ldxt, int n0, const double *Xtr, size_t ldxtr,
               const double *hyp, int nhyp, const double *alpha, double *out, hipStream_t st);
int applymap_nd(int family, int d, int mode, int nm, int ntest, int n0, const double *Xtr, size_t ldxtr, const double *hyp,
                int nhyp, const double *alpha, const double *Q0, const double *P0, double *qmap, double *pmap, int *iters,
                hipStream_t st);
int applymap_nd_tangent(int family, int d, int mode, int nm, int ntest, int n0, const double *Xtr, size_t ldxtr, const double *hyp,
                        int nhyp, const double *alpha, const double *Q0, const double *P0, double *qmap, double *pmap, int *iters,
                        double *jac, double *mono, double *lyap, hipStream_t st);
int genfun_nd(int family, int d, int m, const double *Xt, size_t ldxt, bool has_ref, int n0, const double *Xtr, size_t ldxtr,
              const double *hyp, int nhyp, const double *alpha, double *F, hipStream_t st);
int genfun_cross_nd(int family, int d, int mc, const double *Xt, size_t ldxt, const double *x0, size_t ldx0, int n0,
                    const double *Xtr, size_t ldxtr, const double *hyp, int nhyp, double *V, size_t ldv, double *prior,
                    size_t prior_stride, hipStream_t st);
bool family_is_sum(int family);

int gemm_nt(int m, int n, int k, double alpha, const double *A, size_t lda, const double *B,
            size_t ldb, double beta, double *C, size_t ldc, int lower, long diag_off,
            hipStream_t st);
int gemm_nt_bc(int m, int n, int k, double alpha, const double *A, size_t lda, const double *B,
               size_t ldb, double beta, double *C, size_t ldc, int lower, const int *bc5,
               hipStream_t st);
int gemm_nn(int m, int n, int k, double alpha, const double *A, size_t lda, const double *B, size_t ldb,
            double beta, double *C, size_t ldc, hipStream_t st);
int gemm_nt_two(int m, int n, int k, double alpha, const double *A, size_t lda, const double *B, size_t ldb, double beta,
             double *C, size_t ldc, double alpha2, double *C2, size_t ldc2, hipStream_t st);
constexpr int STRASSEN_REC = 16;
enum { PLAN_SUM = 1, PLAN_PROD = 2, PLAN_CLASSIC = 3 };
int gemm_nt_strassen(int m, int n, int k, double alpha, const double *A, size_t lda, const double *B, size_t ldb, double beta,
                     double *C, size_t ldc, int lower, hipStream_t st);
int strassen_plan(int m, int n, int k, int lower, long smin, long kslab, size_t scratch_doubles, std::vector<long long> &out);
enum { PLAN2_SUM = 4, PLAN2_PROD = 5 };
int strassen_outer_plan(int m, int n, int k, int lower, long smin, long kslab, long smin2, long kslab2, size_t scratch_doubles,
                   std::vector<long long> &out);
int gemm_nt_multi(int m, int n, int k, const double *A, size_t lda, const double *B, size_t ldb, double beta, int count,
                  double *const *C, const size_t *ldc, const double *alpha, hipStream_t st);
size_t strassen_scratch_doubles(int m, int n, int k, int lower, int levels);
void strassen_reserve(size_t both, size_t one, hipStream_t st);
int strassen_trim();
int gemm_profile_begin();
int gemm_profile_end(double *out12);
int gemm_profile_launches(double *buf, int max_records);
void gemm_set_overlap(int on);
int gemm_nt_diag(int m, int n, int k, double alpha, const double *A, size_t lda, const double *B, size_t ldb,
                 double beta, double *C, size_t ldc, int lower, unsigned long long *stamps, int dbg, hipStream_t st);

constexpr int LEAF = 128;
constexpr int POTRF_HANDOFF_TIMEOUT = -1000001;
constexpr int SOLVE_HANDOFF_TIMEOUT = -1000002;
inline int info_status(int info)
{
    if (info >= 0) return info;
    set_error(info == POTRF_HANDOFF_TIMEOUT ? "potrf: a hand-off inside the panel kernel timed out"
              : info == SOLVE_HANDOFF_TIMEOUT ? "solve: a hand-off between the strips of a triangular solve timed out" : "potrf: internal error");
    return SGPR_E_HIP;
}
size_t potrf_workspace(int n);
int potrf(int n, double *A, size_t lda, void *work, size_t lwork, int *dinfo, hipStream_t st);
size_t potrf_batch_flag_bytes(int nbatch);
int potrf_batch_max_order();
int potrf_batch(int nbatch, int npad, double *A, size_t stride_a, size_t lda, double *inv, size_t stride_inv, int *flags,
                int *info, hipStream_t st);
int potrf_batch_panel(int nbatch, int npad, int k0, int Wd, double *A, size_t stride_a, size_t lda, double *inv, size_t stride_inv,
                      int *flags, int *info, hipStream_t st);
bool potrf_queue_mark_failed(hipStream_t st);
int release_device_streams(int dev);
int trsm_rlt(int m, int n, const double *L, size_t ldl, double *B, size_t ldb, const void *work,
             hipStream_t st);
int potrs_vec(int n, const double *L, size_t ldl, void *work, double *b, hipStream_t st);
int solve_status(int n, const double *L, size_t ldl, const void *work, hipStream_t st);
int trsm_rl(int m, int n, const double *L, size_t ldl, double *B, size_t ldb, const void *work, hipStream_t st);
int trsm_rlt_off(int m, int n, const double *L, size_t ldl, double *B, size_t ldb, const void *work, int off, hipStream_t st);
int trsm_rl_off(int m, int n, const double *L, size_t ldl, double *B, size_t ldb, const void *work, int off, hipStream_t st);
int potrs_mat(int n, const double *L, size_t ldl, const void *work, double *B, size_t ldb, int nrhs, double *scratch,
              hipStream_t st);
int potrs_mat_fwd(int n, const double *L, size_t ldl, const void *work, double *B, size_t ldb, int nrhs, double *scratch,
                  hipStream_t st);
size_t potrs_mat_scratch(int n, int nrhs, const double *L, size_t ldl);
bool potrs_mat_uses_strips(int n, int nrhs, const double *L, size_t ldl);
int trsv(int n, const double *L, size_t ldl, void *work, double *b, int trans, hipStream_t st);
bool trsv_uses_strips(int n, const double *L, size_t ldl);
const int *trsv_state(int n, const void *work);
int leaf_probe(double *A, size_t lda, double *inv, int *dinfo, unsigned long long *stamps, hipStream_t st);
int leaf_inverses(int n, const double *L, size_t ldl, void *work, int *dinfo, hipStream_t st);

bool trsv_strips_ok(int n, const double *L, size_t ldl);
int trsv_strips(int n, const double *L, size_t ldl, const double *inv, double *b, int trans, int *state ,
                double *pub , hipStream_t st);
int trsv_strips_batch(int nbatch, int n, const double *L, size_t sL, size_t ldl, const double *inv, size_t sInv, double *b, size_t sB,
                      int trans, int *state, int sState, double *pub, hipStream_t st);

constexpr int TRSM_YLD = 80;
constexpr int TRSM_FOLD = 5;
constexpr int TRSM_STATE_INTS = 16;
bool trsm_strips_ok(int n, const double *L, size_t ldl);
void trsm_piece_of(int u, int C, int T, int out[5]);
void trsm_piece_counts(int T, int C, size_t out[2]);
size_t trsm_strips_scratch(int n);
int potrs_strips(int n, const double *L, size_t ldl, const double *inv, double *B, size_t ldb, int nrhs, int *state ,
                 double *scratch, hipStream_t st);
int trsm_strips_fwd(int n, const double *L, size_t ldl, const double *inv, double *B, size_t ldb, int nrhs, int *state,
                    double *scratch, hipStream_t st);

constexpr int POSTCOV_COLS = 256;
size_t postcov_partial_doubles(int n, int D, int mc);
int postcov(int D, int n, int mc, const double *V, size_t ldv, const double *Kss, size_t ldk, double *part, double *cov,
            hipStream_t st);

size_t nll_grad_full_scratch(int n, int N, int nacc);
int nll_grad_full(int family, int d, bool reg, int N, int n, const double *L, size_t ldl, const void *work, const double *X,
                  const double *alpha, const double *l, const double *pp, int nacc, double *scratch, double *out,
                  hipStream_t st);

int kyinv_panel_width(int n, const char *knob);
int kyinv_row_panel(int n, int J, int rows, const double *L, size_t ldl, const void *work, double *R, size_t ldr, hipStream_t st);

struct LooLayout { size_t panel, blocks, part, resid, cov, lpd, sums, total; };
LooLayout loo_layout(int n, int N, int D);
int fit_loo(int D, int N, int n, const double *L, size_t ldl, const void *work, const double *alpha, double *scratch,
            hipStream_t st);

int fit_batch_max_order();
int fit_batch_trim();
int potrf_trim();
int fit_batch(int family, int nbatch, int npts, const double *x, const double *y, const double *z, const double *hyp,
              int nhyp, const double *sig2n, unsigned flags, double *alpha, double *nll, int *info);
int fit_batch_grad_max_order();
int fit_batch_grad(int family, int nbatch, int npts, const double *x, const double *y, const double *z, const double *hyp,
                   int nhyp, const double *sig2n, unsigned flags, double *alpha, double *nll, double *grad, int *info);
int fit_batch_grad_mid(int family, int nbatch, int npts, const double *x, const double *y, const double *z, const double *hyp,
                       int nhyp, const double *sig2n, unsigned flags, double *alpha, double *nll, double *grad, int *info);
int fit_batch_loo(int family, int nbatch, int npts, const double *x, const double *y, const double *z, const double *hyp,
                  int nhyp, const double *sig2n, unsigned flags, double *alpha, double *nll, double *loo, int *info);

int zero_strict_upper(int n, double *A, size_t lda, hipStream_t st);
int sym_fill_upper(int n, double *A, size_t lda, hipStream_t st);
int nll_reduce(int n, const double *L, size_t ldl, const double *z, const double *alpha,
               double *dout , hipStream_t st);
int copy_diag(int n, const double *A, size_t lda, double *d, hipStream_t st);
int dot(int n, const double *a, const double *b, double *out, hipStream_t st);
constexpr int SUMSQ_SCRATCH = 1024;
int syev_jacobi(int n, double *A, size_t lda, double *V, size_t ldv, double *w_host, int max_sweeps,
                int *sweeps_done, hipStream_t st);
int sumsq(size_t count, const double *a, double *part, double *out, hipStream_t st);
int trace(int n, const double *A, size_t lda, double *out, hipStream_t st);
int transpose(int m, int n, const double *A, size_t lda, double *B, size_t ldb, hipStream_t st);
int gemv_n_sub(int m, int k, const double *A, size_t lda, const double *x, double *y,
               hipStream_t st);
int gemv_t_sub(int m, int k, const double *A, size_t lda, const double *x, double *y,
               hipStream_t st);

}
```

sympgpr_amd/csrc/gemm_f64.hip:

```cpp
#include <algorithm>
#include <atomic>
#include <cstdlib>
#include <mutex>
#include <type_traits>
#include <vector>

#include "common.h"
#include "gemm_tile.h"

namespace sgpr {

namespace {

struct ProfRec { double flop; int big; int m, n, k, lower, overlap; };
struct Prof {
    std::mutex mu;
    std::atomic<bool> on{false};
    std::vector<hipEvent_t> pool;
    std::vector<ProfRec> recs;
    long dropped = 0;
};
constexpr int PROF_POOL = 8192;
Prof g_prof;
thread_local int t_overlap = 0;

using namespace tile;

template <int BM, int BN>
__global__ __launch_bounds__(64 * (BM / 64) * (BN / 64), (BM >= 128 ? 2 : 1)) void gemm_nt_kernel(const GemmArgs g)
{
    constexpr int LDA_S = BM + PAD, LDB_S = BN + PAD;
    constexpr int STAGES = (BM == 256 && BN == 128) ? SGPR_GEMM_STAGES : 2;
    __shared__ double smem[STAGES * BK * (LDA_S + LDB_S)];
    int tile_r, tile_c;
    if (!tile_of<(SR * BM) / (4 * BN)>(g, tile_r, tile_c)) return;
    const int row0 = tile_r * BM, col0 = tile_c * BN;
    if (g.lower) {
        const long rb = ((long)min(row0 + BM, g.m) - 1) / g.lblk, cb = (long)col0 / g.lblk;
        if (rb * g.lpr + g.lpi < cb * g.lpc + g.lpj) return;
    }
    const bool aligned = ((((uintptr_t)g.A | (uintptr_t)g.B) & 15) == 0) && (((g.lda | g.ldb) & 1) == 0);
    const bool fast = aligned && (row0 + BM <= g.m) && (col0 + BN <= g.n) && (g.k % BK == 0);
    if (g.transb) {
        if (fast) gemm_body<BM, BN, true, true>(g, smem, tile_r, tile_c);
        else      gemm_body<BM, BN, false, true>(g, smem, tile_r, tile_c);
        return;
    }
    if constexpr (BM % 128 == 0) {
        if (fast && !(g.dbg & 16)) { gemm_body_dma<BM, BN, STAGES>(g, smem, tile_r, tile_c); return; }
    }
    if (fast) gemm_body<BM, BN, true>(g, smem, tile_r, tile_c);
    else      gemm_body<BM, BN, false>(g, smem, tile_r, tile_c);
}

__global__ __launch_bounds__(512, 2) void gemm_nt2_kernel(const GemmArgs g)
{
    constexpr int BM = 256, BN = 128, LDA_S = BM + PAD, LDB_S = BN + PAD;
    __shared__ double smem[SGPR_GEMM_STAGES * BK * (LDA_S + LDB_S)];
    int tile_r, tile_c;
    if (!tile_of<(SR * BM) / (4 * BN)>(g, tile_r, tile_c)) return;
    const int row0 = tile_r * BM, col0 = tile_c * BN;
    const bool aligned = ((((uintptr_t)g.A | (uintptr_t)g.B) & 15) == 0) && (((g.lda | g.ldb) & 1) == 0);
    const bool fast = aligned && (row0 + BM <= g.m) && (col0 + BN <= g.n) && (g.k % BK == 0);
    if (fast) gemm_body_dma<BM, BN, SGPR_GEMM_STAGES, true>(g, smem, tile_r, tile_c);
    else      gemm_body<BM, BN, false, false, true>(g, smem, tile_r, tile_c);
}

__global__ __launch_bounds__(512, 2) void gemm_nt4_kernel(const GemmArgs g)
{
    constexpr int BM = 256, BN = 128, LDA_S = BM + PAD, LDB_S = BN + PAD;
    __shared__ double smem[SGPR_GEMM_STAGES * BK * (LDA_S + LDB_S)];
    int tile_r, tile_c;
    if (!tile_of<(SR * BM) / (4 * BN)>(g, tile_r, tile_c)) return;
    const int row0 = tile_r * BM, col0 = tile_c * BN;
    const bool aligned = ((((uintptr_t)g.A | (uintptr_t)g.B) & 15) == 0) && (((g.lda | g.ldb) & 1) == 0);
    const bool fast = aligned && (row0 + BM <= g.m) && (col0 + BN <= g.n) && (g.k % BK == 0);
    if (fast) gemm_body_dma<BM, BN, SGPR_GEMM_STAGES, false, true>(g, smem, tile_r, tile_c);
    else      gemm_body<BM, BN, false, false, false, true>(g, smem, tile_r, tile_c);
}

struct Dst { double *C; size_t ld; double alpha; };

__global__ __launch_bounds__(256) void block_sum_kernel(int rows, int cols, const double *X, size_t ldx, const double *Y, size_t ldy,
                                                        double sign, double *T)
{
    const int nrc = (rows + 511) / 512, ncg = (cols + 3) / 4;
    const long pieces = (long)nrc * ncg;
    for (long p = blockIdx.x; p < pieces; p += gridDim.x) {
        const int cg = (int)(p / nrc), rc = (int)(p - (long)cg * nrc);
        const int r = rc * 512 + 2 * (int)threadIdx.x;
        if (r >= rows) continue;
        double2_t x[4], y[4];
#pragma unroll
        for (int u = 0; u < 4; ++u) {
            const int c = min(cg * 4 + u, cols - 1);
            x[u] = *reinterpret_cast<const double2_t *>(X + (size_t)r + (size_t)c * ldx);
            y[u] = *reinterpret_cast<const double2_t *>(Y + (size_t)r + (size_t)c * ldy);
        }
#pragma unroll
        for (int u = 0; u < 4; ++u) {
            const int c = cg * 4 + u;
            if (c < cols) *reinterpret_cast<double2_t *>(T + (size_t)r + (size_t)c * (size_t)rows) = x[u] + sign * y[u];
        }
    }
}

}

int gemm_nt(int m, int n, int k, double alpha, const double *A, size_t lda, const double *B,
            size_t ldb, double beta, double *C, size_t ldc, int lower, long diag_off,
            hipStream_t st)
{
    const int bc[5] = {1, 1, (int)diag_off, 1, 0};
    return gemm_nt_bc(m, n, k, alpha, A, lda, B, ldb, beta, C, ldc, lower, bc, st);
}

static int gemm_launch(int m, int n, int k, double alpha, const double *A, size_t lda, const double *B,
                       size_t ldb, double beta, double *C, size_t ldc, int lower, const int *bc, int transb,
                       hipStream_t st, unsigned long long *stamps = nullptr, int dbg = 0, const Dst *x = nullptr, int nx = 0,
                       bool k4 = false);

static int gemm_chunked(int m, int n, int k, double alpha, const double *A, size_t lda, const double *B,
                        size_t ldb, double beta, double *C, size_t ldc, int lower, const int *bc,
                        hipStream_t st, const Dst *x, int nx, bool k4)
{
    static const int kmax = [] { const char *e = getenv("SGPR_GEMM_KMAX"); return e ? atoi(e) : 8192; }();
    if (kmax >= 128 && k > kmax) {
        const int nchunk = (k + kmax - 1) / kmax;
        const int step = ((k + nchunk - 1) / nchunk + 127) / 128 * 128;
        for (int k0 = 0; k0 < k; k0 += step) {
            const int rc = gemm_launch(m, n, std::min(step, k - k0), alpha, A + (size_t)k0 * lda, lda, B + (size_t)k0 * ldb, ldb,
                                       k0 == 0 ? beta : 1.0, C, ldc, lower, bc, 0, st, nullptr, 0, x, nx, k4);
            if (rc) return rc;
        }
        return 0;
    }
    return gemm_launch(m, n, k, alpha, A, lda, B, ldb, beta, C, ldc, lower, bc, 0, st, nullptr, 0, x, nx, k4);
}

int gemm_nt_bc(int m, int n, int k, double alpha, const double *A, size_t lda, const double *B,
               size_t ldb, double beta, double *C, size_t ldc, int lower, const int *bc,
               hipStream_t st)
{
    return gemm_chunked(m, n, k, alpha, A, lda, B, ldb, beta, C, ldc, lower, bc, st, nullptr, 0, false);
}

int gemm_nt_two(int m, int n, int k, double alpha, const double *A, size_t lda, const double *B, size_t ldb, double beta,
             double *C, size_t ldc, double alpha2, double *C2, size_t ldc2, hipStream_t st)
{
    const int bc[5] = {1, 1, 0, 1, 0};
    if (!C2) { set_error("gemm_nt_two: null second destination"); return SGPR_E_ARG; }
    const Dst x{C2, ldc2, alpha2};
    return gemm_chunked(m, n, k, alpha, A, lda, B, ldb, beta, C, ldc, 0, bc, st, &x, 1, false);
}

int gemm_nt_multi(int m, int n, int k, const double *A, size_t lda, const double *B, size_t ldb, double beta, int count,
                  double *const *C, const size_t *ldc, const double *alpha, hipStream_t st)
{
    const int bc[5] = {1, 1, 0, 1, 0};
    if (count < 2 || count > 4 || !C || !ldc || !alpha) { set_error("gemm_nt_multi: 2 to 4 destinations"); return SGPR_E_ARG; }
    Dst x[3];
    for (int d = 0; d < count; ++d) {
        if (!C[d]) { set_error("gemm_nt_multi: null destination"); return SGPR_E_ARG; }
        if (d) x[d - 1] = Dst{C[d], ldc[d], alpha[d]};
    }
    return gemm_chunked(m, n, k, alpha[0], A, lda, B, ldb, beta, C[0], ldc[0], 0, bc, st, x, count - 1, true);
}

static int gemm_launch(int m, int n, int k, double alpha, const double *A, size_t lda, const double *B,
                       size_t ldb, double beta, double *C, size_t ldc, int lower, const int *bc, int transb,
                       hipStream_t st, unsigned long long *stamps, int dbg, const Dst *x, int nx, bool k4)
{
    const bool plain = bc[0] == 1 && bc[1] == 1 && bc[3] == 1 && bc[4] == 0;
    const long diag_off = plain ? bc[2] : 1;
    if (bc[0] < 1 || bc[1] < 1 || bc[3] < 1) { set_error("gemm_nt: bad block-cyclic descriptor"); return SGPR_E_ARG; }
    if (m < 0 || n < 0 || k < 0) { set_error("gemm_nt: negative extent"); return SGPR_E_ARG; }
    if (m == 0 || n == 0) return 0;
    if (lda < (size_t)m || ldb < (size_t)(transb ? k : n) || ldc < (size_t)m) {
        set_error("gemm: leading dimension too small");
        return SGPR_E_ARG;
    }
    if (nx < 0 || nx > 3 || (nx && !x)) { set_error("gemm: bad destination count"); return SGPR_E_ARG; }
    Dst d[3] = {};
    for (int i = 0; i < nx; ++i) {
        d[i] = x[i];
        if (!d[i].C || lower || transb || d[i].ld < (size_t)m) { set_error("gemm: bad second destination"); return SGPR_E_ARG; }
    }
    GemmArgs g{m, n, k, alpha, beta, A, lda, B, ldb, C, ldc, lower, diag_off, transb, stamps, 0, 0, 0, 0, 0, 0,
               0, 0, bc[0], bc[1], bc[2], bc[3], bc[4], dbg, nullptr, d[0].C, d[0].ld, d[0].alpha,
               d[1].C, d[1].ld, d[1].alpha, d[2].C, d[2].ld, d[2].alpha, nx + 1};
    auto set_map = [&](int bm, int bn) {
        g.tiles_m = (m + bm - 1) / bm;
        g.tiles_n = (n + bn - 1) / bn;
        const int SC = (SR * bm) / (4 * bn);
        g.n_sr = (g.tiles_m + SR - 1) / SR;
        g.n_sc = (g.tiles_n + SC - 1) / SC;
        g.tri = (lower && diag_off == 0 && m == n) ? 1 : 0;
        if (g.tri) {
            long full = 0;
            for (int sc = 0; sc < g.n_sc; ++sc) full += std::max(g.n_sr - sc / 4 - 1, 0);
            g.n_full = (int)full;
            g.n_grp = (g.n_sc + 3) / 4;
            g.n_super = g.n_full + 4 * g.n_grp;
        }
        if (!g.tri) g.n_super = g.n_sr * g.n_sc;
        return (unsigned)(((g.n_super + 7) / 8) * 8 * SR * SC);
    };
    int slot = -1;
    ProfRec rec{};
    if (g_prof.on.load(std::memory_order_acquire)) {
        std::lock_guard<std::mutex> lock(g_prof.mu);
        if (g_prof.on.load(std::memory_order_relaxed)) {
            if ((int)g_prof.recs.size() < PROF_POOL) {
                double elems = (double)m * n;
                if (lower && plain) {
                    elems = 0.0;
                    for (int j = 0; j < n; ++j) {
                        long first = (long)j - diag_off;
                        if (first < 0) first = 0;
                        if (first < m) elems += (double)(m - first);
                    }
                } else if (lower) {
                    elems = 0.0;
                    const long blk = bc[0];
                    for (long j = 0; j < n; ++j) {
                        const long cbg = (j / blk) * bc[3] + bc[4], jo = j % blk;
                        for (long rb = 0; rb * blk < m; ++rb) {
                            const long rbg = rb * bc[1] + bc[2], rows = std::min(blk, (long)m - rb * blk);
                            if (rbg > cbg) elems += (double)rows;
                            else if (rbg == cbg) elems += (double)std::max(0L, rows - jo);
                        }
                    }
                }
                rec.flop = 2.0 * k * elems;
                rec.m = m; rec.n = n; rec.k = k; rec.lower = lower; rec.overlap = t_overlap;
                slot = (int)g_prof.recs.size();
                g_prof.recs.push_back(rec);
            } else {
                ++g_prof.dropped;
            }
        }
    }
    if (slot >= 0) SGPR_HIP(hipEventRecord(g_prof.pool[2 * slot], st));
    const long big = (long)((m + 255) / 256) * ((n + 127) / 128);
    static const bool prefer_big = tune("gemm_small_tile", 0) == 0;
    static const double small_mb = tune("gemm_small_mb", 0.0);
    const double op_bytes = 8.0 * (double)k * ((A == B && lda == ldb) ? (double)std::max(m, n) : (double)m + n);
    const bool small_k = op_bytes <= small_mb * 1e6 && m > 128 && n > 128;
    if (nx) {
        const dim3 grid(set_map(256, 128));
        if (k4 || nx > 1) hipLaunchKernelGGL(gemm_nt4_kernel, grid, dim3(512), 0, st, g);
        else              hipLaunchKernelGGL(gemm_nt2_kernel, grid, dim3(512), 0, st, g);
        rec.big = 1;
    } else if (n <= 128 && m <= 32768 && !(dbg & 8)) {
        const dim3 grid(set_map(64, 128));
        hipLaunchKernelGGL((gemm_nt_kernel<64, 128>), grid, dim3(128), 0, st, g);
    } else if (prefer_big && !(dbg & 8) && !small_k && (big >= 256 || (m >= 256 && n == 128))) {
        const dim3 grid(set_map(256, 128));
        hipLaunchKernelGGL((gemm_nt_kernel<256, 128>), grid, dim3(512), 0, st, g);
        rec.big = 1;
    } else {
        const dim3 grid(set_map(128, 128));
        hipLaunchKernelGGL((gemm_nt_kernel<128, 128>), grid, dim3(256), 0, st, g);
    }
    SGPR_CHECK_LAUNCH();
    if (slot >= 0) {
        SGPR_HIP(hipEventRecord(g_prof.pool[2 * slot + 1], st));
        if (rec.big) {
            std::lock_guard<std::mutex> lock(g_prof.mu);
            if (slot < (int)g_prof.recs.size()) g_prof.recs[slot].big = 1;
        }
    }
    return 0;
}

int gemm_nt_diag(int m, int n, int k, double alpha, const double *A, size_t lda, const double *B, size_t ldb,
                 double beta, double *C, size_t ldc, int lower, unsigned long long *stamps, int dbg, hipStream_t st)
{
    const int bc[5] = {1, 1, 0, 1, 0};
    return gemm_launch(m, n, k, alpha, A, lda, B, ldb, beta, C, ldc, lower, bc, 0, st, stamps, dbg);
}

int gemm_nn(int m, int n, int k, double alpha, const double *A, size_t lda, const double *B, size_t ldb,
            double beta, double *C, size_t ldc, hipStream_t st)
{
    const int bc[5] = {1, 1, 0, 1, 0};
    return gemm_launch(m, n, k, alpha, A, lda, B, ldb, beta, C, ldc, 0, bc, 1, st);
}

void gemm_set_overlap(int on) { t_overlap = on; }

int gemm_profile_begin()
{
    std::lock_guard<std::mutex> lock(g_prof.mu);
    if (g_prof.pool.empty()) {
        g_prof.pool.resize(2 * (size_t)PROF_POOL);
        for (size_t i = 0; i < g_prof.pool.size(); ++i) {
            const hipError_t e = hipEventCreate(&g_prof.pool[i]);
            if (e != hipSuccess) {
                for (size_t j = 0; j < i; ++j) (void)hipEventDestroy(g_prof.pool[j]);
                g_prof.pool.clear();
                return hip_fail(e, "hipEventCreate (profile pool)", __FILE__, __LINE__);
            }
        }
        g_prof.recs.reserve(PROF_POOL);
    }
    g_prof.recs.clear();
    g_prof.dropped = 0;
    g_prof.on = true;
    return 0;
}

static std::vector<double> g_last_launches;
int gemm_profile_launches(double *buf, int max_records)
{
    std::lock_guard<std::mutex> lock(g_prof.mu);
    const int n = (int)(g_last_launches.size() / 7);
    if (buf)
        for (int i = 0; i < n && i < max_records; ++i)
            for (int j = 0; j < 7; ++j) buf[7 * i + j] = g_last_launches[7 * i + j];
    return n;
}

int gemm_profile_end(double *out)
{
    std::lock_guard<std::mutex> lock(g_prof.mu);
    g_prof.on = false;
    g_last_launches.clear();
    for (int i = 0; i < 12; ++i) out[i] = 0.0;
    out[11] = (double)g_prof.dropped;
    for (size_t i = 0; i < g_prof.recs.size(); ++i) {
        const ProfRec &r = g_prof.recs[i];
        SGPR_HIP(hipEventSynchronize(g_prof.pool[2 * i + 1]));
        float ms = 0.f;
        SGPR_HIP(hipEventElapsedTime(&ms, g_prof.pool[2 * i], g_prof.pool[2 * i + 1]));
        const int o = r.big ? (r.overlap ? 8 : 0) : 3;
        out[o] += 1.0; out[o + 1] += r.flop; out[o + 2] += ms;
        if (r.flop > out[6]) { out[6] = r.flop; out[7] = ms; }
        for (double v : {(double)r.m, (double)r.n, (double)r.k, (double)r.lower, (double)r.big, (double)ms, (double)r.overlap})
            g_last_launches.push_back(v);
    }
    g_prof.recs.clear();
    return 0;
}

namespace {
struct PlanCfg {
    long smin;
    long kslab;
    size_t scratch;
};
void put(std::vector<long long> &out, std::initializer_list<long long> v)
{
    size_t i = 0;
    for (long long x : v) { out.push_back(x); ++i; }
    for (; i < STRASSEN_REC; ++i) out.push_back(0);
}
long slab_of(long k, const PlanCfg &c)
{
    if (k <= 0 || k % 32 != 0 || c.kslab < 32) return 0;
    const long nslab = (k + c.kslab - 1) / c.kslab;
    const long step = ((k + nslab - 1) / nslab + 31) / 32 * 32;
    const long kmin = std::max(c.smin / 2, 16L);
    const long last = k - (nslab - 1) * step;
    if (last <= 0 || step / 2 < kmin || last / 2 < kmin) return 0;
    return step;
}
bool qualifies(long m, long n, long k, const PlanCfg &c)
{
    if (m <= 0 || n <= 0 || m % 512 != 0 || n % 256 != 0) return false;
    if (m / 2 < c.smin || n / 2 < c.smin) return false;
    const long step = slab_of(k, c);
    if (!step) return false;
    return (size_t)(m / 2 + n / 2) * (size_t)(step / 2) <= c.scratch;
}
void seven(int kind_sum, int kind_prod, long m2, long n2, long k2, long k0, long ar, long br, long cr, long cc, std::vector<long long> &out)
{
    const long a1 = ar, a2 = ar + m2, b1 = br, b2 = br + n2, j1 = k0, j2 = k0 + k2;
    const long c1r = cr, c2r = cr + m2, c1c = cc, c2c = cc + n2;
    auto sum = [&](int side, long xr, long xc, long yr, long yc, int sign) {
        put(out, {kind_sum, side, side ? n2 : m2, k2, xr, xc, yr, yc, sign});
    };
    auto prod = [&](int as, long pr, long pc, int bs, long qr, long qc, long d1r, long d1c, int s1, long d2r, long d2c, int s2) {
        put(out, {kind_prod, as, pr, pc, bs, qr, qc, m2, n2, k2, d1r, d1c, s1, d2r, d2c, s2});
    };
    sum(0, a1, j1, a2, j2, +1); sum(1, b1, j1, b2, j2, +1);
    prod(1, 0, 0, 1, 0, 0, c1r, c1c, +1, c2r, c2c, +1);
    sum(0, a2, j1, a2, j2, +1);
    prod(1, 0, 0, 0, b1, j1, c2r, c1c, +1, c2r, c2c, -1);
    sum(1, b2, j1, b2, j2, -1);
    prod(0, a1, j1, 1, 0, 0, c1r, c2c, +1, c2r, c2c, +1);
    sum(1, b1, j2, b1, j1, -1);
    prod(0, a2, j2, 1, 0, 0, c1r, c1c, +1, c2r, c1c, +1);
    sum(0, a1, j1, a1, j2, +1);
    prod(1, 0, 0, 0, b2, j2, c1r, c1c, -1, c1r, c2c, +1);
    sum(0, a2, j1, a1, j1, -1); sum(1, b1, j1, b2, j1, +1);
    prod(1, 0, 0, 1, 0, 0, c2r, c2c, +1, 0, 0, 0);
    sum(0, a1, j2, a2, j2, -1); sum(1, b1, j2, b2, j2, +1);
    prod(1, 0, 0, 1, 0, 0, c1r, c1c, +1, 0, 0, 0);
}
void plan_gemm(long m, long n, long k, long ar, long br, long cr, long cc, const PlanCfg &c, std::vector<long long> &out)
{
    if (!qualifies(m, n, k, c)) {
        put(out, {PLAN_CLASSIC, 0, ar, 0, br, 0, m, n, k, cr, cc});
        return;
    }
    const long step = slab_of(k, c);
    for (long k0 = 0; k0 < k; k0 += step) seven(PLAN_SUM, PLAN_PROD, m / 2, n / 2, std::min(step, k - k0) / 2, k0, ar, br, cr, cc, out);
}
void plan_syrk(long n, long k, long r0, const PlanCfg &c, std::vector<long long> &out)
{
    const long h = n / 2;
    if (n % 2 != 0 || !qualifies(h, h, k, c)) {
        put(out, {PLAN_CLASSIC, 1, r0, 0, r0, 0, n, n, k, r0, r0});
        return;
    }
    plan_syrk(h, k, r0, c, out);
    plan_gemm(h, h, k, r0 + h, r0, r0 + h, r0, c, out);
    plan_syrk(h, k, r0 + h, c, out);
}
size_t plan_need(const std::vector<long long> &plan)
{
    size_t need[2] = {0, 0};
    for (size_t i = 0; i + STRASSEN_REC <= plan.size(); i += STRASSEN_REC)
        if (plan[i] == PLAN_SUM) need[plan[i + 1]] = std::max(need[plan[i + 1]], (size_t)plan[i + 2] * (size_t)plan[i + 3]);
    return need[0] + need[1];
}

int strassen_levels()
{
    static const int lv = [] { const char *e = getenv("SGPR_GEMM_STRASSEN"); return !e ? 2 : (e[0] == '0' ? 0 : (e[0] == '1' ? 1 : 2)); }();
    return lv;
}
bool strassen_on() { return strassen_levels() > 0; }
PlanCfg default_cfg()
{
    static const long smin = std::max(128L, (long)tune("gemm_strassen_min", 8192));
    static const long kslab = std::max(32L, (long)tune("gemm_strassen_kslab", 16384));
    return PlanCfg{smin, kslab, ~(size_t)0};
}

struct Plan2Cfg {
    PlanCfg in;
    long smin2;
    long kslab2;
    size_t scratch;
};
Plan2Cfg default_cfg2()
{
    static const long smin2 = std::max(256L, (long)tune("gemm_strassen2_min", 16384));
    static const long kslab2 = std::max(64L, (long)tune("gemm_strassen2_kslab", 32768));
    return Plan2Cfg{default_cfg(), smin2, kslab2, ~(size_t)0};
}
bool outer_noscratch()
{
    static const bool forced_fail = tune("gemm_strassen2_noscratch", 0) != 0;
    return forced_fail;
}
bool qualifies2(long m, long n, long k, const Plan2Cfg &c)
{
    if (m <= 0 || n <= 0 || m % 1024 != 0 || n % 512 != 0) return false;
    if (m / 2 < c.smin2 || n / 2 < c.smin2) return false;
    if (c.kslab2 < 64 || c.kslab2 % 64 != 0 || k < c.kslab2) return false;
    const size_t pair = (size_t)(m / 2 + n / 2) * (size_t)(c.kslab2 / 2);
    if (pair > c.scratch) return false;
    PlanCfg ci = c.in;
    ci.scratch = c.scratch - pair;
    return qualifies(m / 2, n / 2, c.kslab2 / 2, ci);
}
PlanCfg inner_of(const Plan2Cfg &c)
{
    PlanCfg ci = c.in;
    ci.scratch = c.scratch;
    return ci;
}
void plan2_gemm(long m, long n, long k, long ar, long br, long cr, long cc, const Plan2Cfg &c, std::vector<long long> &out)
{
    if (!qualifies2(m, n, k, c)) { plan_gemm(m, n, k, ar, br, cr, cc, inner_of(c), out); return; }
    long k0 = 0;
    for (; k0 + c.kslab2 <= k; k0 += c.kslab2) seven(PLAN2_SUM, PLAN2_PROD, m / 2, n / 2, c.kslab2 / 2, k0, ar, br, cr, cc, out);
    if (k0 == k) return;
    size_t i = out.size();
    plan_gemm(m, n, k - k0, ar, br, cr, cc, inner_of(c), out);
    for (; i + STRASSEN_REC <= out.size(); i += STRASSEN_REC) {
        long long *r = &out[i];
        if (r[0] == PLAN_SUM) { r[5] += k0; r[7] += k0; }
        else if (r[0] == PLAN_PROD) { if (!r[1]) r[3] += k0; if (!r[4]) r[6] += k0; }
        else { r[3] += k0; r[5] += k0; }
    }
}
void plan2_syrk(long n, long k, long r0, const Plan2Cfg &c, std::vector<long long> &out)
{
    const long h = n / 2;
    if (n % 2 != 0 || !qualifies2(h, h, k, c)) { plan_syrk(n, k, r0, inner_of(c), out); return; }
    plan2_syrk(h, k, r0, c, out);
    plan2_gemm(h, h, k, r0 + h, r0, r0 + h, r0, c, out);
    plan2_syrk(h, k, r0 + h, c, out);
}
void inner_plan(const long long *r, const PlanCfg &ci, std::vector<long long> &out)
{
    out.clear();
    plan_gemm(r[7], r[8], r[9], 0, 0, 0, 0, ci, out);
}
struct Need2 { size_t v[4] = {0, 0, 0, 0}; size_t inner() const { return v[0] + v[1]; } size_t total() const { return v[0] + v[1] + v[2] + v[3]; } };
Need2 plan2_need(const std::vector<long long> &plan, const Plan2Cfg &c)
{
    Need2 nd;
    std::vector<long long> in;
    auto sums = [&](const long long *r, int base) {
        size_t &v = nd.v[base + r[1]];
        v = std::max(v, (size_t)r[2] * (size_t)r[3]);
    };
    PlanCfg ci = c.in;
    ci.scratch = ~(size_t)0;
    for (size_t i = 0; i + STRASSEN_REC <= plan.size(); i += STRASSEN_REC) {
        const long long *r = &plan[i];
        if (r[0] == PLAN_SUM) sums(r, 0);
        else if (r[0] == PLAN2_SUM) sums(r, 2);
        else if (r[0] == PLAN2_PROD) {
            inner_plan(r, ci, in);
            for (size_t j = 0; j + STRASSEN_REC <= in.size(); j += STRASSEN_REC)
                if (in[j] == PLAN_SUM) sums(&in[j], 0);
        }
    }
    return nd;
}

struct Scratch {
    std::mutex mu;
    double *p = nullptr;
    size_t cap = 0, failed = 0;
    hipEvent_t ev = nullptr;
    hipStream_t last = nullptr;
    bool used = false;
};
Scratch g_scratch[64];

bool scratch_ensure(Scratch &s, size_t need)
{
    static const bool forced_fail = tune("gemm_strassen_noscratch", 0) != 0;
    if (forced_fail) return false;
    if (s.cap >= need) return true;
    if (s.failed && need >= s.failed) return false;
    if (s.p) { (void)hipFree(s.p); s.p = nullptr; s.cap = 0; s.used = false; }
    if (hipMalloc((void **)&s.p, need * sizeof(double)) != hipSuccess) {
        (void)hipGetLastError();
        s.p = nullptr;
        s.failed = need;
        return false;
    }
    s.cap = need;
    return true;
}
int device_of(hipStream_t st)
{
    int dev = -1;
    if ((st ? hipStreamGetDevice(st, &dev) : hipGetDevice(&dev)) != hipSuccess) { (void)hipGetLastError(); return -1; }
    return (dev >= 0 && dev < 64) ? dev : -1;
}

int block_sum(int rows, int cols, const double *X, size_t ldx, const double *Y, size_t ldy, double sign, double *T, hipStream_t st)
{
    const long pieces = (long)((rows + 511) / 512) * ((cols + 3) / 4);
    hipLaunchKernelGGL(block_sum_kernel, dim3((unsigned)std::min(pieces, 2048L)), dim3(256), 0, st, rows, cols, X, ldx, Y, ldy, sign, T);
    SGPR_CHECK_LAUNCH();
    return 0;
}

int run_plan(const long long *recs, size_t nrec, double alpha, const double *A, size_t lda, const double *B, size_t ldb,
             double beta, double *C, size_t ldc, double alpha2, double *C2, size_t ldc2, double *SA, double *SB, hipStream_t st)
{
    for (size_t i = 0; i < nrec; ++i) {
        const long long *r = recs + i * STRASSEN_REC;
        int rc = 0;
        if (r[0] == PLAN_SUM) {
            const double *P = r[1] ? B : A;
            const size_t ld = r[1] ? ldb : lda;
            rc = block_sum((int)r[2], (int)r[3], P + r[4] + (size_t)r[5] * ld, ld, P + r[6] + (size_t)r[7] * ld, ld, (double)r[8],
                           r[1] ? SB : SA, st);
        } else if (r[0] == PLAN_PROD) {
            const int m = (int)r[7], n = (int)r[8], k = (int)r[9];
            const double *Ap = r[1] ? SA : A + r[2] + (size_t)r[3] * lda;
            const double *Bp = r[4] ? SB : B + r[5] + (size_t)r[6] * ldb;
            const size_t la = r[1] ? (size_t)m : lda, lb = r[4] ? (size_t)n : ldb;
            double *C1 = C + r[10] + (size_t)r[11] * ldc;
            if (C2) {
                double *cs[4] = {C1, nullptr, nullptr, nullptr};
                size_t ls[4] = {ldc, 0, 0, 0};
                double as[4] = {alpha * (double)r[12], 0.0, 0.0, 0.0};
                int cnt = 1;
                auto add = [&](double *p, size_t l, double a) { cs[cnt] = p; ls[cnt] = l; as[cnt] = a; ++cnt; };
                if (r[15]) add(C + r[13] + (size_t)r[14] * ldc, ldc, alpha * (double)r[15]);
                add(C2 + r[10] + (size_t)r[11] * ldc2, ldc2, alpha2 * (double)r[12]);
                if (r[15]) add(C2 + r[13] + (size_t)r[14] * ldc2, ldc2, alpha2 * (double)r[15]);
                if (cnt == 2) rc = gemm_nt_two(m, n, k, as[0], Ap, la, Bp, lb, 1.0, cs[0], ls[0], as[1], cs[1], ls[1], st);
                else          rc = gemm_nt_multi(m, n, k, Ap, la, Bp, lb, 1.0, cnt, cs, ls, as, st);
            } else if (r[15]) {
                rc = gemm_nt_two(m, n, k, alpha * (double)r[12], Ap, la, Bp, lb, 1.0, C1, ldc,
                                 alpha * (double)r[15], C + r[13] + (size_t)r[14] * ldc, ldc, st);
            } else {
                rc = gemm_nt(m, n, k, alpha * (double)r[12], Ap, la, Bp, lb, 1.0, C1, ldc, 0, 0, st);
            }
        } else if (r[0] == PLAN_CLASSIC) {
            const double *Ap = A + r[2] + (size_t)r[3] * lda, *Bp = B + r[4] + (size_t)r[5] * ldb;
            if (C2) rc = gemm_nt_two((int)r[6], (int)r[7], (int)r[8], alpha, Ap, lda, Bp, ldb, beta, C + r[9] + (size_t)r[10] * ldc, ldc,
                                     alpha2, C2 + r[9] + (size_t)r[10] * ldc2, ldc2, st);
            else    rc = gemm_nt((int)r[6], (int)r[7], (int)r[8], alpha, Ap, lda, Bp, ldb, beta, C + r[9] + (size_t)r[10] * ldc, ldc, (int)r[1], 0, st);
        } else {
            set_error("run_plan: unknown record");
            rc = SGPR_E_ARG;
        }
        if (rc) return rc;
    }
    return 0;
}
int run_plan(const std::vector<long long> &plan, double alpha, const double *A, size_t lda, const double *B, size_t ldb,
             double beta, double *C, size_t ldc, double *SA, double *SB, hipStream_t st)
{
    return run_plan(plan.data(), plan.size() / STRASSEN_REC, alpha, A, lda, B, ldb, beta, C, ldc, 0.0, nullptr, 0, SA, SB, st);
}
int run_plan2(const std::vector<long long> &plan, const Plan2Cfg &c, const Need2 &nd, double alpha, const double *A, size_t lda,
              const double *B, size_t ldb, double beta, double *C, size_t ldc, double *S, hipStream_t st)
{
    double *const SA = S, *const SB = S + nd.v[0], *const OA = SB + nd.v[1], *const OB = OA + nd.v[2];
    PlanCfg ci = c.in;
    ci.scratch = nd.inner();
    std::vector<long long> in;
    for (size_t i = 0; i + STRASSEN_REC <= plan.size(); i += STRASSEN_REC) {
        const long long *r = &plan[i];
        int rc = 0;
        if (r[0] == PLAN2_SUM) {
            const double *P = r[1] ? B : A;
            const size_t ld = r[1] ? ldb : lda;
            rc = block_sum((int)r[2], (int)r[3], P + r[4] + (size_t)r[5] * ld, ld, P + r[6] + (size_t)r[7] * ld, ld, (double)r[8],
                           r[1] ? OB : OA, st);
        } else if (r[0] == PLAN2_PROD) {
            const double *X = r[1] ? OA : A + r[2] + (size_t)r[3] * lda;
            const double *Y = r[4] ? OB : B + r[5] + (size_t)r[6] * ldb;
            inner_plan(r, ci, in);
            rc = run_plan(in.data(), in.size() / STRASSEN_REC, alpha * (double)r[12], X, r[1] ? (size_t)r[7] : lda, Y, r[4] ? (size_t)r[8] : ldb,
                          1.0, C + r[10] + (size_t)r[11] * ldc, ldc, alpha * (double)r[15], r[15] ? C + r[13] + (size_t)r[14] * ldc : nullptr, ldc,
                          SA, SB, st);
        } else {
            rc = run_plan(r, 1, alpha, A, lda, B, ldb, beta, C, ldc, 0.0, nullptr, 0, SA, SB, st);
        }
        if (rc) return rc;
    }
    return 0;
}
}

int strassen_plan(int m, int n, int k, int lower, long smin, long kslab, size_t scratch_doubles, std::vector<long long> &out)
{
    if (m < 0 || n < 0 || k < 0 || (lower && m != n)) { set_error("strassen_plan: bad extents"); return SGPR_E_ARG; }
    PlanCfg c = default_cfg();
    if (smin >= 0) c.smin = std::max(128L, smin);
    if (kslab >= 0) c.kslab = std::max(32L, kslab);
    c.scratch = scratch_doubles;
    out.clear();
    if (lower) plan_syrk(n, k, 0, c, out);
    else       plan_gemm(m, n, k, 0, 0, 0, 0, c, out);
    return 0;
}

namespace {
Plan2Cfg cfg2_of(long smin, long kslab, long smin2, long kslab2, size_t scratch_doubles)
{
    Plan2Cfg c = default_cfg2();
    if (smin >= 0) c.in.smin = std::max(128L, smin);
    if (kslab >= 0) c.in.kslab = std::max(32L, kslab);
    if (smin2 >= 0) c.smin2 = std::max(256L, smin2);
    if (kslab2 >= 0) c.kslab2 = std::max(64L, kslab2);
    c.scratch = scratch_doubles;
    return c;
}
}

int strassen_outer_plan(int m, int n, int k, int lower, long smin, long kslab, long smin2, long kslab2, size_t scratch_doubles,
                   std::vector<long long> &out)
{
    if (m < 0 || n < 0 || k < 0 || (lower && m != n)) { set_error("strassen_outer_plan: bad extents"); return SGPR_E_ARG; }
    const Plan2Cfg c = cfg2_of(smin, kslab, smin2, kslab2, scratch_doubles);
    out.clear();
    if (lower) plan2_syrk(n, k, 0, c, out);
    else       plan2_gemm(m, n, k, 0, 0, 0, 0, c, out);
    return 0;
}

size_t strassen_scratch_doubles(int m, int n, int k, int lower, int levels)
{
    std::vector<long long> plan;
    if (!strassen_on()) return 0;
    if (levels >= 2 && strassen_levels() >= 2) {
        if (strassen_outer_plan(m, n, k, lower, -1, -1, -1, -1, ~(size_t)0, plan)) return 0;
        return plan2_need(plan, default_cfg2()).total();
    }
    if (strassen_plan(m, n, k, lower, -1, -1, ~(size_t)0, plan)) return 0;
    return plan_need(plan);
}

void strassen_reserve(size_t both, size_t one, hipStream_t st)
{
    const int dev = device_of(st);
    if (dev < 0 || !strassen_on()) return;
    Scratch &s = g_scratch[dev];
    std::lock_guard<std::mutex> lock(s.mu);
    if (both > one && !outer_noscratch() && scratch_ensure(s, both)) return;
    if (one) (void)scratch_ensure(s, one);
}

int strassen_trim()
{
    for (Scratch &s : g_scratch) {
        std::lock_guard<std::mutex> lock(s.mu);
        if (s.p) (void)hipFree(s.p);
        if (s.ev) (void)hipEventDestroy(s.ev);
        s.p = nullptr; s.ev = nullptr; s.cap = 0; s.failed = 0; s.used = false; s.last = nullptr;
    }
    (void)hipGetLastError();
    return 0;
}

int gemm_nt_strassen(int m, int n, int k, double alpha, const double *A, size_t lda, const double *B, size_t ldb, double beta,
                     double *C, size_t ldc, int lower, hipStream_t st)
{
    const bool aligned = ((((uintptr_t)A | (uintptr_t)B) & 15) == 0) && (((lda | ldb) & 1) == 0);
    if (std::min(m, n) / 2 < default_cfg().smin || !strassen_on() || !aligned || beta != 1.0 || (lower && m != n))
        return gemm_nt(m, n, k, alpha, A, lda, B, ldb, beta, C, ldc, lower, 0, st);
    std::vector<long long> plan;
    int rc = 0;
    const int dev = device_of(st);
    auto enqueue = [&](Scratch &s, auto &&run) {
        if (!s.ev) SGPR_HIP(hipEventCreateWithFlags(&s.ev, hipEventDisableTiming));
        if (s.used && s.last != st) SGPR_HIP(hipStreamWaitEvent(st, s.ev, 0));
        const int r = run();
        SGPR_HIP(hipEventRecord(s.ev, st));
        s.last = st;
        s.used = true;
        return r;
    };
    const Plan2Cfg c2 = default_cfg2();
    if (strassen_levels() >= 2 && dev >= 0 && !outer_noscratch() && std::min(lower ? m / 2 : m, lower ? n / 2 : n) / 2 >= c2.smin2) {
        if ((rc = strassen_outer_plan(m, n, k, lower, -1, -1, -1, -1, ~(size_t)0, plan))) return rc;
        const Need2 nd = plan2_need(plan, c2);
        if (nd.v[2] + nd.v[3]) {
            Scratch &s = g_scratch[dev];
            std::lock_guard<std::mutex> lock(s.mu);
            if (scratch_ensure(s, nd.total()))
                return enqueue(s, [&] { return run_plan2(plan, c2, nd, alpha, A, lda, B, ldb, beta, C, ldc, s.p, st); });
        }
    }
    rc = strassen_plan(m, n, k, lower, -1, -1, ~(size_t)0, plan);
    if (rc) return rc;
    const size_t need = plan_need(plan);
    if (!need) return run_plan(plan, alpha, A, lda, B, ldb, beta, C, ldc, nullptr, nullptr, st);
    if (dev < 0) return gemm_nt(m, n, k, alpha, A, lda, B, ldb, beta, C, ldc, lower, 0, st);
    Scratch &s = g_scratch[dev];
    std::lock_guard<std::mutex> lock(s.mu);
    if (!scratch_ensure(s, need)) {
        if ((rc = strassen_plan(m, n, k, lower, -1, -1, s.cap, plan))) return rc;
        if (!plan_need(plan)) return run_plan(plan, alpha, A, lda, B, ldb, beta, C, ldc, nullptr, nullptr, st);
    }
    size_t na = 0;
    for (size_t i = 0; i + STRASSEN_REC <= plan.size(); i += STRASSEN_REC)
        if (plan[i] == PLAN_SUM && plan[i + 1] == 0) na = std::max(na, (size_t)plan[i + 2] * (size_t)plan[i + 3]);
    return enqueue(s, [&] { return run_plan(plan, alpha, A, lda, B, ldb, beta, C, ldc, s.p, s.p + na, st); });
}

}
```

sympgpr_amd/csrc/probe.hip:

```cpp
#include <algorithm>
#include <cstdlib>
#include <vector>

#include "cholq.h"
#include "common.h"
#include "../../include/sympgpr_probe.h"
#include "generated/pair_generated.h"

namespace sgpr {
namespace {
typedef double double4_t __attribute__((ext_vector_type(4)));
typedef double double2_t __attribute__((ext_vector_type(2)));

template <int NACC>
__global__ __launch_bounds__(256) void mfma_clock_kernel(int iters, double *out, unsigned long long *stamps)
{
    double4_t acc[NACC];
    const double a = 1.0 + threadIdx.x * 1e-9, b = 1.0 - threadIdx.x * 1e-9;
#pragma unroll
    for (int i = 0; i < NACC; ++i) acc[i] = double4_t{0.0, 0.0, 0.0, 0.0};
    const unsigned long long t0 = __builtin_amdgcn_s_memtime(), r0 = __builtin_amdgcn_s_memrealtime();
    for (int it = 0; it < iters; ++it) {
#pragma unroll
        for (int i = 0; i < NACC; ++i)
// ... 213 lines not shown
#pragma unroll
    for (int j = 0; j < 16; ++j) {
        const int rj = j >> 2;
        if (V == 0) {
            const double v = D[rj] * rl;
            D = __builtin_amdgcn_mfma_f64_16x16x4f64(v, v, D, 0, 0, 0);
        } else if (V == 1) {
            const double v = D[rj] * rl, x = X[rj] * rl;
            D = __builtin_amdgcn_mfma_f64_16x16x4f64(v, v, D, 0, 0, 0);
            X = __builtin_amdgcn_mfma_f64_16x16x4f64(v, x, X, 0, 0, 0);
        } else if (V == 2) {
            const double a = bcast(acc, (j + 1) & 63), b = bcast(rl, (j + 17) & 63);
            rl = nr(__builtin_fma(-b, b, a + 5.0));
            acc += rl;
        } else if (V == 3) {
            rl = __builtin_amdgcn_rsq(rl + 1.0);
        } else if (V == 4) {
#pragma unroll
            for (int q = 0; q < 8; ++q) rl = __builtin_fma(rl, acc, 0.5);
        } else if (V == 5) {
            rl = bcast(rl, (j + 1) & 63) + acc;
        } else if (V == 6) {
            sh[lane] = rl;
            rl = sh[(lane + 1) & 63] + 1.0;
        } else if (V >= 8) {
            const int g = j & 3;
            const double v = D[rj] * rl;
            const double x = X[rj] * rl;
            double rn = 0.0;
            if (j + 1 < 16) {
                const double dnext = bcast(D[(j + 1) >> 2], (j + 1) + 16 * ((j + 1) & 3));
                const double lnext = bcast(v, (j + 1) + 16 * g);
                rn = nr(__builtin_fma(-lnext, lnext, dnext));
            }
            if (V == 8 || V == 9) {
                if (l4 == g) big[j * 130 + l15] = v;
                sh[j] = rl;
            }
            const double nv = v * mneg[j];
            D = __builtin_amdgcn_mfma_f64_16x16x4f64(nv, v, D, 0, 0, 0);
            if (V == 8 || V == 10) X = __builtin_amdgcn_mfma_f64_16x16x4f64(nv, x, X, 0, 0, 0);
            rl = rn;
        } else if (V == 7) {
            const double v = D[rj] * rl;
            D = __builtin_amdgcn_mfma_f64_16x16x4f64(v, v, D, 0, 0, 0);
            rl = bcast(D[0], 0) * 1e-3;
        }
    }
    double ssum = rl + acc + D[0] + D[1] + D[2] + D[3] + X[0] + X[1] + X[2] + X[3];
    asm volatile("s_nop 0\n\ts_memtime %0\n\ts_waitcnt lgkmcnt(0)" : "=s"(t1), "+v"(ssum) : : "memory");
    if (lane == 0) cyc[V] = t1 - t0;
    if (ssum == 12345.678) io[2] = ssum + big[lane] + sh[lane];
}
} }

extern "C" int sgpr_probe_lat(double *out8 )
{
    double *io = nullptr;
    unsigned long long *cyc = nullptr;
    SGPR_HIP(hipMalloc((void **)&io, 64));
    SGPR_HIP(hipMalloc((void **)&cyc, 128));
    const double h[3] = {0.49, 1.25, 0.0};
    SGPR_HIP(hipMemcpy(io, h, sizeof(h), hipMemcpyHostToDevice));
    for (int rep = 0; rep < 2; ++rep) {
        hipLaunchKernelGGL((sgpr::lat_probe_kernel<0>), dim3(1), dim3(256), 0, 0, io, cyc);
        hipLaunchKernelGGL((sgpr::lat_probe_kernel<1>), dim3(1), dim3(256), 0, 0, io, cyc);
        hipLaunchKernelGGL((sgpr::lat_probe_kernel<2>), dim3(1), dim3(256), 0, 0, io, cyc);
        hipLaunchKernelGGL((sgpr::lat_probe_kernel<3>), dim3(1), dim3(256), 0, 0, io, cyc);
        hipLaunchKernelGGL((sgpr::lat_probe_kernel<4>), dim3(1), dim3(256), 0, 0, io, cyc);
        hipLaunchKernelGGL((sgpr::lat_probe_kernel<5>), dim3(1), dim3(256), 0, 0, io, cyc);
        hipLaunchKernelGGL((sgpr::lat_probe_kernel<6>), dim3(1), dim3(256), 0, 0, io, cyc);
        hipLaunchKernelGGL((sgpr::lat_probe_kernel<7>), dim3(1), dim3(256), 0, 0, io, cyc);
        hipLaunchKernelGGL((sgpr::lat_probe_kernel<8>), dim3(1), dim3(256), 0, 0, io, cyc);
        hipLaunchKernelGGL((sgpr::lat_probe_kernel<9>), dim3(1), dim3(256), 0, 0, io, cyc);
        hipLaunchKernelGGL((sgpr::lat_probe_kernel<10>), dim3(1), dim3(256), 0, 0, io, cyc);
        hipLaunchKernelGGL((sgpr::lat_probe_kernel<11>), dim3(1), dim3(256), 0, 0, io, cyc);
        SGPR_HIP(hipDeviceSynchronize());
    }
    unsigned long long hs[12];
    SGPR_HIP(hipMemcpy(hs, cyc, 96, hipMemcpyDeviceToHost));
    for (int i = 0; i < 12; ++i) out8[i] = (double)hs[i] / 16.0;
    (void)hipFree(io); (void)hipFree(cyc);
    return 0;
}

extern "C" int sgpr_probe_leaf(double *out8)
{
    const int n = LEAF;
    std::vector<double> h((size_t)n * n, 0.0);
    for (int i = 0; i < n; ++i)
        for (int j = 0; j <= i; ++j) h[i + (size_t)j * n] = (i == j) ? 4.0 + 0.01 * i : 1.0 / (1.0 + i + j);
    double *A = nullptr, *inv = nullptr;
    int *info = nullptr;
    unsigned long long *st = nullptr;
    SGPR_HIP(hipMalloc((void **)&A, sizeof(double) * n * n));
    SGPR_HIP(hipMalloc((void **)&inv, sizeof(double) * n * n));
    SGPR_HIP(hipMalloc((void **)&info, 16));
    SGPR_HIP(hipMalloc((void **)&st, 64));
    SGPR_HIP(hipMemset(info, 0, 16));
    for (int rep = 0; rep < 2; ++rep) {
        SGPR_HIP(hipMemcpy(A, h.data(), sizeof(double) * n * n, hipMemcpyHostToDevice));
        int rc = leaf_probe(A, n, inv, info, st, nullptr);
        if (rc) return rc;
        SGPR_HIP(hipDeviceSynchronize());
    }
    unsigned long long hs[8];
    SGPR_HIP(hipMemcpy(hs, st, 64, hipMemcpyDeviceToHost));
    for (int i = 0; i < 8; ++i) out8[i] = (double)hs[i];
    (void)hipFree(A); (void)hipFree(inv); (void)hipFree(info); (void)hipFree(st);
    return 0;
}

namespace sgpr { namespace {
__global__ __launch_bounds__(512) void xcc_probe_kernel(int *out)
{
    const int x = __builtin_amdgcn_s_getreg(20 | (0 << 6) | (3 << 11));
    if (threadIdx.x == 0) out[blockIdx.x] = x;
    unsigned long long t0 = __builtin_amdgcn_s_memtime();
    while (__builtin_amdgcn_s_memtime() - t0 < 20000) {}
}
} }
extern "C" int sgpr_probe_xcc(int nblocks, int *host_out)
{
    int *d = nullptr;
    SGPR_HIP(hipMalloc((void **)&d, sizeof(int) * nblocks));
    hipLaunchKernelGGL(sgpr::xcc_probe_kernel, dim3(nblocks), dim3(512), 0, nullptr, d);
    SGPR_HIP(hipMemcpy(host_out, d, sizeof(int) * nblocks, hipMemcpyDeviceToHost));
    (void)hipFree(d);
    return 0;
}

namespace sgpr { namespace {
__global__ __launch_bounds__(512) void cumask_probe_kernel(int *out)
{
    const int x = __builtin_amdgcn_s_getreg(20 | (0 << 6) | (3 << 11));
    const int hw = __builtin_amdgcn_s_getreg(4 | (0 << 6) | (31 << 11));
    if (threadIdx.x == 0) { out[2 * blockIdx.x] = x; out[2 * blockIdx.x + 1] = hw; }
    unsigned long long t0 = __builtin_amdgcn_s_memtime();
    while (__builtin_amdgcn_s_memtime() - t0 < 200000) {}
}
} }
extern "C" int sgpr_probe_cumask(const unsigned *mask_words, int nwords, int nblocks, int *host_out)
{
    hipStream_t st = nullptr;
    SGPR_HIP(hipExtStreamCreateWithCUMask(&st, (uint32_t)nwords, mask_words));
    int *d = nullptr;
    SGPR_HIP(hipMalloc((void **)&d, sizeof(int) * 2 * nblocks));
    hipLaunchKernelGGL(sgpr::cumask_probe_kernel, dim3(nblocks), dim3(512), 0, st, d);
    SGPR_HIP(hipStreamSynchronize(st));
    SGPR_HIP(hipMemcpy(host_out, d, sizeof(int) * 2 * nblocks, hipMemcpyDeviceToHost));
    (void)hipFree(d);
    (void)hipStreamDestroy(st);
    return 0;
}


namespace sgpr {
template <int FAM>
__global__ void generated_eval_kernel(int which, int m, const double *xa, const double *ya, const double *xb,
                                      const double *yb, double lx, double ly, double p, double *out)
{
    const int i = blockIdx.x * blockDim.x + threadIdx.x;
    if (i >= m) return;
    double o[4];
    const int dl = which >> 2;
    if (dl == 0)      gen::pair<FAM>(xa[i], ya[i], xb[i], yb[i], lx, ly, p, o);
    else if (dl == 1) gen::pair_dlx<FAM>(xa[i], ya[i], xb[i], yb[i], lx, ly, p, o);
    else              gen::pair_dly<FAM>(xa[i], ya[i], xb[i], yb[i], lx, ly, p, o);
    out[i] = o[which & 3];
}
}

extern "C" int sgpr_probe_generated_eval(int family, int which, int m, const double *xa, const double *ya,
                                         const double *xb, const double *yb, const double *l, int nl, double *out)
{
    using namespace sgpr;
    if (m <= 0) return 0;
    if (which < 0 || which > 11 || !l || nl < 2 || (family == SGPR_FAM_D && nl < 3)) { set_error("generated_eval: bad arguments"); return SGPR_E_ARG; }
    double *d[5] = {};
    const double *h[4] = {xa, ya, xb, yb};
    for (int k = 0; k < 5; ++k) SGPR_HIP(hipMalloc((void **)&d[k], sizeof(double) * m));
    for (int k = 0; k < 4; ++k) SGPR_HIP(hipMemcpy(d[k], h[k], sizeof(double) * m, hipMemcpyHostToDevice));
    const double p = family == SGPR_FAM_D ? l[2] : 0.0;
    const dim3 grid((m + 255) / 256);
    switch (family) {
    case SGPR_FAM_A: hipLaunchKernelGGL(generated_eval_kernel<SGPR_FAM_A>, grid, dim3(256), 0, nullptr, which, m, d[0], d[1], d[2], d[3], l[0], l[1], p, d[4]); break;
    case SGPR_FAM_B: hipLaunchKernelGGL(generated_eval_kernel<SGPR_FAM_B>, grid, dim3(256), 0, nullptr, which, m, d[0], d[1], d[2], d[3], l[0], l[1], p, d[4]); break;
    case SGPR_FAM_C: hipLaunchKernelGGL(generated_eval_kernel<SGPR_FAM_C>, grid, dim3(256), 0, nullptr, which, m, d[0], d[1], d[2], d[3], l[0], l[1], p, d[4]); break;
    case SGPR_FAM_D: hipLaunchKernelGGL(generated_eval_kernel<SGPR_FAM_D>, grid, dim3(256), 0, nullptr, which, m, d[0], d[1], d[2], d[3], l[0], l[1], p, d[4]); break;
    default: set_error("unknown kernel family"); return SGPR_E_ARG;
    }
    SGPR_CHECK_LAUNCH();
    SGPR_HIP(hipMemcpy(out, d[4], sizeof(double) * m, hipMemcpyDeviceToHost));
    for (int k = 0; k < 5; ++k) (void)hipFree(d[k]);
    return 0;
}

extern "C" int sgpr_probe_queue_plan(int n, int nworkers, int *starts_out, int max_starts, unsigned *tasks_out,
                                     int max_tasks, int *counts)
{
    cholq::Plan p;
    const int rc = cholq::build_plan(n, cholq::default_starts(n), nworkers, p);
    if (rc) return rc;
    counts[0] = p.nblk;
    counts[1] = (int)(p.tasks.size() / 2);
    counts[2] = (int)p.model_us;
    for (int k = 0; k <= p.nblk && k < max_starts; ++k) starts_out[k] = p.starts[k];
    for (size_t t = 0; t < p.tasks.size() && (int)(t / 2) < max_tasks; ++t) tasks_out[t] = p.tasks[t];
    return 0;
}

extern "C" int sgpr_probe_queue_plan_partial(int n, int nworkers, int nq, int *starts_out, int max_starts, unsigned *tasks_out,
                                             int max_tasks, int *counts)
{
    cholq::Plan p;
    const std::vector<int> st = cholq::default_starts(n);
    const int rc = cholq::build_plan(n, st, nworkers, p, nq < 0 ? cholq::default_nq(n, st) : nq);
    if (rc) return rc;
    counts[0] = p.nblk;
    counts[1] = (int)(p.tasks.size() / 2);
    counts[2] = (int)p.model_us;
    counts[3] = p.nq;
    for (int k = 0; k <= p.nblk && k < max_starts; ++k) starts_out[k] = p.starts[k];
    for (size_t t = 0; t < p.tasks.size() && (int)(t / 2) < max_tasks; ++t) tasks_out[t] = p.tasks[t];
    return 0;
}

static unsigned long long *g_qtrace = nullptr;
static int g_qtrace_cap = 0;
extern "C" int sgpr_probe_queue_trace_begin(int max_tasks)
{
    if (g_qtrace) { cholq::set_trace(nullptr, 0); (void)hipFree(g_qtrace); g_qtrace = nullptr; }
    SGPR_HIP(hipMalloc((void **)&g_qtrace, sizeof(unsigned long long) * cholq::trace_words((size_t)max_tasks)));
    SGPR_HIP(hipMemset(g_qtrace, 0, sizeof(unsigned long long) * cholq::trace_words((size_t)max_tasks)));
    g_qtrace_cap = max_tasks;
    cholq::set_trace(g_qtrace, (size_t)max_tasks);
    return max_tasks;
}
extern "C" int sgpr_probe_queue_trace_clear()
{
    if (!g_qtrace) return 0;
    SGPR_HIP(hipMemset(g_qtrace, 0, sizeof(unsigned long long) * cholq::trace_words((size_t)g_qtrace_cap)));
    return 0;
}
extern "C" int sgpr_probe_queue_trace_end(unsigned long long *out, int max_tasks)
{
    if (!g_qtrace) return 0;
    SGPR_HIP(hipDeviceSynchronize());
    cholq::set_trace(nullptr, 0);
    if (max_tasks < g_qtrace_cap) { set_error("queue_trace_end: buffer smaller than the capacity given to _begin"); return SGPR_E_ARG; }
    const size_t words = cholq::trace_words((size_t)g_qtrace_cap);
    SGPR_HIP(hipMemcpy(out, g_qtrace, sizeof(unsigned long long) * words, hipMemcpyDeviceToHost));
    (void)hipFree(g_qtrace);
    g_qtrace = nullptr;
    return (int)words;
}

extern "C" int sgpr_probe_queue_postmortem(int always) { return cholq::postmortem(always != 0); }
extern "C" int sgpr_probe_queue_force_giveup(int on) { cholq::force_giveup(on); return 0; }
extern "C" int sgpr_probe_tune(const char *name, double value)
{
    if (!name) { set_error("probe_tune: null name"); return SGPR_E_ARG; }
    tune_set(name, value);
    return 0;
}

extern "C" int sgpr_probe_strassen_plan(int m, int n, int k, int lower, long smin, long kslab, long scratch_doubles, long long *out,
                                        int max_records, int *count)
{
    if (!count || scratch_doubles < 0) { set_error("probe_strassen_plan: bad arguments"); return SGPR_E_ARG; }
    std::vector<long long> plan;
    const int rc = strassen_plan(m, n, k, lower, smin, kslab, (size_t)scratch_doubles, plan);
    if (rc) return rc;
    *count = (int)(plan.size() / STRASSEN_REC);
    for (size_t i = 0; out && i < plan.size() && (int)(i / STRASSEN_REC) < max_records; ++i) out[i] = plan[i];
    return 0;
}
extern "C" int sgpr_probe_gemm_strassen_dev(int m, int n, int k, double alpha, const double *A, size_t lda, const double *B, size_t ldb,
                                            double beta, double *C, size_t ldc, int lower, void *stream)
{
    return gemm_nt_strassen(m, n, k, alpha, A, lda, B, ldb, beta, C, ldc, lower, static_cast<hipStream_t>(stream));
}
extern "C" int sgpr_probe_gemm_nt2_dev(int m, int n, int k, double alpha, const double *A, size_t lda, const double *B, size_t ldb,
                                       double beta, double *C, size_t ldc, double alpha2, double *C2, size_t ldc2, void *stream)
{
    return gemm_nt_two(m, n, k, alpha, A, lda, B, ldb, beta, C, ldc, alpha2, C2, ldc2, static_cast<hipStream_t>(stream));
}
extern "C" int sgpr_probe_strassen2_plan(int m, int n, int k, int lower, long smin, long kslab, long smin2, long kslab2,
                                         long scratch_doubles, long long *out, int max_records, int *count)
{
    if (!count || scratch_doubles < 0) { set_error("probe_strassen2_plan: bad arguments"); return SGPR_E_ARG; }
    std::vector<long long> plan;
    const int rc = strassen_outer_plan(m, n, k, lower, smin, kslab, smin2, kslab2, (size_t)scratch_doubles, plan);
    if (rc) return rc;
    *count = (int)(plan.size() / STRASSEN_REC);
    for (size_t i = 0; out && i < plan.size() && (int)(i / STRASSEN_REC) < max_records; ++i) out[i] = plan[i];
    return 0;
}
extern "C" int sgpr_probe_gemm_nt4_dev(int m, int n, int k, const double *A, size_t lda, const double *B, size_t ldb, double beta,
                                       int count, double *const *C, const size_t *ldc, const double *alpha, void *stream)
{
    return gemm_nt_multi(m, n, k, A, lda, B, ldb, beta, count, C, ldc, alpha, static_cast<hipStream_t>(stream));
}
extern "C" unsigned sgpr_probe_map_calls(void) { return applymap_last_calls(); }
extern "C" int sgpr_probe_map_team(int ntest, int n0) { return applymap_team(ntest, n0); }
extern "C" int sgpr_probe_trsm_piece(int ticket, int cap, int strips, int out[5]) { if (ticket < 0 || cap < 1 || strips < 0 || !out) return SGPR_E_ARG; trsm_piece_of(ticket, cap, strips, out); return 0; }
extern "C" int sgpr_probe_trsm_counts(int strips, int cap, unsigned long long out[2])
{
    if (strips < 0 || cap < 1 || !out) return SGPR_E_ARG;
    size_t c[2];
    trsm_piece_counts(strips, cap, c);
    out[0] = c[0]; out[1] = c[1];
    return 0;
}

namespace sgpr { namespace {
__global__ void census_kernel(unsigned long long *out, int spin_us)
{
    extern __shared__ double dyn[];
    const unsigned long long t0 = __builtin_amdgcn_s_memrealtime();
    if (threadIdx.x == 0) {
        dyn[0] = 1.0;
        out[4 * blockIdx.x + 0] = (unsigned long long)__builtin_amdgcn_s_getreg(20 | (0 << 6) | (3 << 11));
        out[4 * blockIdx.x + 1] = (unsigned long long)__builtin_amdgcn_s_getreg(4 | (0 << 6) | (31 << 11));
        out[4 * blockIdx.x + 2] = t0;
    }
    while (__builtin_amdgcn_s_memrealtime() - t0 < (unsigned long long)spin_us * 100ull) __builtin_amdgcn_s_sleep(32);
    if (threadIdx.x == 0) out[4 * blockIdx.x + 3] = __builtin_amdgcn_s_memrealtime();
}
} }
extern "C" int sgpr_probe_census(int na, int threads_a, int lds_a, int spin_a, const unsigned *mask_a, int nwords_a,
                                 int nb, int threads_b, int lds_b, int spin_b, const unsigned *mask_b, int nwords_b,
                                 unsigned long long *host_out)
{
    hipStream_t sa = nullptr, sb = nullptr;
    if (nwords_a > 0) SGPR_HIP(hipExtStreamCreateWithCUMask(&sa, (uint32_t)nwords_a, mask_a));
    else              SGPR_HIP(hipStreamCreateWithFlags(&sa, hipStreamNonBlocking));
    if (nwords_b > 0) SGPR_HIP(hipExtStreamCreateWithCUMask(&sb, (uint32_t)nwords_b, mask_b));
    else {
        int lo = 0, hi = 0;
        SGPR_HIP(hipDeviceGetStreamPriorityRange(&lo, &hi));
        SGPR_HIP(hipStreamCreateWithPriority(&sb, hipStreamNonBlocking, hi));
    }
    unsigned long long *d = nullptr;
    const size_t words = 4 * (size_t)(na + nb);
    SGPR_HIP(hipMalloc((void **)&d, sizeof(unsigned long long) * words));
    SGPR_HIP(hipMemset(d, 0, sizeof(unsigned long long) * words));
    SGPR_HIP(hipFuncSetAttribute((const void *)sgpr::census_kernel, hipFuncAttributeMaxDynamicSharedMemorySize, 160 * 1024));
    SGPR_HIP(hipDeviceSynchronize());
    hipLaunchKernelGGL(sgpr::census_kernel, dim3(na), dim3(threads_a), lds_a, sa, d, spin_a);
    SGPR_CHECK_LAUNCH();
    hipLaunchKernelGGL(sgpr::census_kernel, dim3(nb), dim3(threads_b), lds_b, sb, d + 4 * (size_t)na, spin_b);
    SGPR_CHECK_LAUNCH();
    SGPR_HIP(hipStreamSynchronize(sa));
    SGPR_HIP(hipStreamSynchronize(sb));
    SGPR_HIP(hipMemcpy(host_out, d, sizeof(unsigned long long) * words, hipMemcpyDeviceToHost));
    (void)hipFree(d);
    (void)hipStreamDestroy(sa);
    (void)hipStreamDestroy(sb);
    return 0;
}
```

Measured before the change: 78.93.

## Fuse Strassen operand sums into five-slot kernels and size scratch per product

Adds a block_sum5 kernel that reads the four quadrants of an operand once and writes all five Strassen sum combinations into separate scratch slots. This replaces ten separate block_sum launches per Strassen level, and the products then index into the matching slot. Scratch reservation for potrf now walks every recursive product to choose among several size options, and per-call Strassen thresholds can be set through a StrassenSet. The cost is five times the scratch memory, with fallbacks to the unfused path when that allocation fails.

```diff
diff --git a/include/sympgpr_probe.h b/include/sympgpr_probe.h
--- a/include/sympgpr_probe.h
+++ b/include/sympgpr_probe.h
@@ -38,6 +38,11 @@
                               long long *out, int max_records, int *count);
 int sgpr_probe_gemm_nt4_dev(int m, int n, int k, const double *A, size_t lda, const double *B, size_t ldb, double beta, int count,
                             double *const *C, const size_t *ldc, const double *alpha, void *stream);
+int sgpr_probe_strassen_fuse_groups(const long long *recs, int nrec, int *out3, int *groups);
+int sgpr_probe_potrf_scratch(int n, int la_max, long smin, long smin2, long kslab2b, long long out[4]);
+int sgpr_probe_potrf_products(int n, int la_max, long smin, long smin2, long kslab2b, long long *out, int max_products, int *count);
+int sgpr_probe_strassen_reserved(int dev, long long out[2]);
+int sgpr_probe_strassen_sum_launches(long long out[2]);
 unsigned sgpr_probe_map_calls(void);
 int sgpr_probe_map_team(int ntest, int n0);
 
diff --git a/sympgpr_amd/_lib.py b/sympgpr_amd/_lib.py
--- a/sympgpr_amd/_lib.py
+++ b/sympgpr_amd/_lib.py
@@ -174,6 +174,12 @@
                                             C.POINTER(C.c_longlong), C.c_int, C.POINTER(C.c_int)]),
     "sgpr_probe_gemm_nt4_dev": (C.c_int, [C.c_int, C.c_int, C.c_int, C.c_void_p, C.c_size_t, C.c_void_p, C.c_size_t, C.c_double, C.c_int,
                                           C.POINTER(C.c_void_p), C.POINTER(C.c_size_t), C.POINTER(C.c_double), C.c_void_p]),
+    "sgpr_probe_strassen_fuse_groups": (C.c_int, [C.POINTER(C.c_longlong), C.c_int, C.POINTER(C.c_int), C.POINTER(C.c_int)]),
+    "sgpr_probe_potrf_scratch": (C.c_int, [C.c_int, C.c_int, C.c_long, C.c_long, C.c_long, C.POINTER(C.c_longlong)]),
+    "sgpr_probe_potrf_products": (C.c_int, [C.c_int, C.c_int, C.c_long, C.c_long, C.c_long, C.POINTER(C.c_longlong), C.c_int,
+                                            C.POINTER(C.c_int)]),
+    "sgpr_probe_strassen_sum_launches": (C.c_int, [C.POINTER(C.c_longlong)]),
+    "sgpr_probe_strassen_reserved": (C.c_int, [C.c_int, C.POINTER(C.c_longlong)]),
     "sgpr_probe_census": (C.c_int, [C.c_int, C.c_int, C.c_int, C.c_int, C.POINTER(C.c_uint), C.c_int,
                                     C.c_int, C.c_int, C.c_int, C.c_int, C.POINTER(C.c_uint), C.c_int,
                                     C.POINTER(C.c_ulonglong)]),
diff --git a/sympgpr_amd/csrc/chol.hip b/sympgpr_amd/csrc/chol.hip
--- a/sympgpr_amd/csrc/chol.hip
+++ b/sympgpr_amd/csrc/chol.hip
@@ -798,6 +798,7 @@
     int *flags = nullptr;
     void *qws = nullptr;
     bool strassen = false;
+    StrassenSet sset;
 };
 
 int potrf_lookahead(int n, double *A, size_t lda, const Ctx &c, int nb, int off0);
@@ -812,7 +813,7 @@
     const int n1 = split(n), n2 = n - n1;
     int rc = trsm_rec(m, n1, L, ldl, B, ldb, off, c);
     if (rc) return rc;
-    if (c.strassen) rc = gemm_nt_strassen(m, n2, n1, -1.0, B, ldb, L + n1, ldl, 1.0, B + (size_t)n1 * ldb, ldb, 0, c.st);
+    if (c.strassen) rc = gemm_nt_strassen(m, n2, n1, -1.0, B, ldb, L + n1, ldl, 1.0, B + (size_t)n1 * ldb, ldb, 0, c.st, &c.sset);
     else            rc = gemm_nt(m, n2, n1, -1.0, B, ldb, L + n1, ldl, 1.0, B + (size_t)n1 * ldb, ldb, 0, 0, c.st);
     if (rc) return rc;
     return trsm_rec(m, n2, L + n1 + (size_t)n1 * ldl, ldl, B + (size_t)n1 * ldb, ldb, off + n1, c);
@@ -846,7 +847,7 @@
     if (rc) return rc;
     rc = trsm_rec(n2, n1, A, lda, A21, lda, off, c);
     if (rc) return rc;
-    if (c.strassen) rc = gemm_nt_strassen(n2, n2, n1, -1.0, A21, lda, A21, lda, 1.0, A22, lda, 1, c.st);
+    if (c.strassen) rc = gemm_nt_strassen(n2, n2, n1, -1.0, A21, lda, A21, lda, 1.0, A22, lda, 1, c.st, &c.sset);
     else            rc = gemm_nt(n2, n2, n1, -1.0, A21, lda, A21, lda, 1.0, A22, lda, 1, 0, c.st);
     if (rc) return rc;
     return potrf_rec(n2, A22, lda, off + n1, c);
@@ -1447,6 +1448,64 @@
     return release_streams(dev);
 }
 
+static int la_max_default()
+{
+    static const int v = [] { const char *e = getenv("SGPR_LA_MAX"); return (int)tune("la_max", e ? atoi(e) : 57344); }();
+    return v;
+}
+static const StrassenSet &rec_set()
+{
+    static const StrassenSet s = [] {
+        auto get = [](const char *env, const char *name, double dflt) { const char *e = getenv(env); return (long)tune(name, e ? atof(e) : dflt); };
+        StrassenSet v;
+        v.smin = get("SGPR_REC_STRASSEN_MIN", "rec_strassen_min", 0);
+        v.smin2 = get("SGPR_REC_STRASSEN2_MIN", "rec_strassen2_min", 0);
+        v.kslab2b = get("SGPR_REC_STRASSEN2_KSLAB_B", "rec_strassen2_kslab_b", 0);
+        return v;
+    }();
+    return s;
+}
+
+template <class F> static void trsm_products(int m, int n, F &&fn)
+{
+    if (n <= LEAF) return;
+    const int n1 = split(n), n2 = n - n1;
+    trsm_products(m, n1, fn);
+    fn(m, n2, n1, 0);
+    trsm_products(m, n2, fn);
+}
+template <class F> static void rec_products(int n, int la_max, F &&fn)
+{
+    if (n <= LEAF || (n > 4 * LEAF && n <= la_max)) return;
+    const int n1 = split(n), n2 = n - n1;
+    rec_products(n1, la_max, fn);
+    trsm_products(n2, n1, fn);
+    fn(n2, n2, n1, 1);
+    rec_products(n2, la_max, fn);
+}
+int potrf_products(int n, int la_max, const StrassenSet *set, std::vector<long long> &out)
+{
+    if (n < 0) { set_error("potrf_products: bad order"); return SGPR_E_ARG; }
+    if (!set) set = &rec_set();
+    out.clear();
+    rec_products(n, la_max < 0 ? la_max_default() : la_max, [&](int m, int nn, int k, int lower) {
+        for (long long v : {(long long)m, (long long)nn, (long long)k, (long long)lower, (long long)strassen_levels_of(m, nn, k, lower, set)})
+            out.push_back(v);
+    });
+    return 0;
+}
+void potrf_scratch_options(int n, int la_max, const StrassenSet *set, size_t opt[4])
+{
+    if (!set) set = &rec_set();
+    for (int i = 0; i < 4; ++i) opt[i] = 0;
+    rec_products(n, la_max < 0 ? la_max_default() : la_max, [&](int m, int nn, int k, int lower) {
+        if (!strassen_levels_of(m, nn, k, lower, set)) return;
+        size_t o[4];
+        strassen_scratch_options(m, nn, k, lower, o, set);
+        for (int i = 0; i < 4; ++i) opt[i] = std::max(opt[i], o[i]);
+    });
+}
+
 int potrf(int n, double *A, size_t lda, void *work, size_t lwork, int *dinfo, hipStream_t st)
 {
     if (n < 0 || (n > 0 && lda < (size_t)n)) { set_error("potrf: bad n / lda"); return SGPR_E_ARG; }
@@ -1457,17 +1516,16 @@
     SGPR_HIP(hipMemsetAsync(flags, 0, flag_bytes(n), st));
     static const int mode = [] { const char *e = getenv("SGPR_POTRF"); return !e ? 0 : (e[0] == 'r' ? 1 : 2); }();
     static const int nb_env = [] { const char *e = getenv("SGPR_POTRF_NB"); return e ? atoi(e) : 0; }();
-    static const int la_max_env = [] { const char *e = getenv("SGPR_LA_MAX"); return (int)tune("la_max", e ? atoi(e) : 57344); }();
+    const int la_max_env = la_max_default();
     t_last_potrf_used_queue = false;
     Ctx c{static_cast<double *>(work), dinfo, st, mode == 1 ? 0 : la_max_env, flags};
     if (cholq::ws_bytes(n) > 0) c.qws = static_cast<char *>(work) + inv_bytes(n) + flag_bytes(n) + pub_bytes(n);
     c.strassen = true;
+    c.sset = rec_set();
     if (n > c.la_max && n > LEAF) {
-        const int n1 = split(n), n2 = n - n1, n11 = split(n1);
-        auto need = [&](int levels) {
-            return std::max(strassen_scratch_doubles(n2, n2, n1, 1, levels), strassen_scratch_doubles(n2, n1 - n11, n11, 0, levels));
-        };
-        strassen_reserve(need(2), need(1), st);
+        size_t opt[4];
+        potrf_scratch_options(n, c.la_max, &c.sset, opt);
+        strassen_reserve(opt, st);
     }
     const bool dbg = PANEL_DBG && getenv("SGPR_PANEL_DBG") != nullptr;
     const int T = (n + LEAF - 1) / LEAF;
diff --git a/sympgpr_amd/csrc/common.h b/sympgpr_amd/csrc/common.h
--- a/sympgpr_amd/csrc/common.h
+++ b/sympgpr_amd/csrc/common.h
@@ -111,16 +111,27 @@
              double *C, size_t ldc, double alpha2, double *C2, size_t ldc2, hipStream_t st);
 constexpr int STRASSEN_REC = 16;
 enum { PLAN_SUM = 1, PLAN_PROD = 2, PLAN_CLASSIC = 3 };
+struct StrassenSet {
+    long smin = 0;
+    long smin2 = 0;
+    long kslab2b = 0;
+};
 int gemm_nt_strassen(int m, int n, int k, double alpha, const double *A, size_t lda, const double *B, size_t ldb, double beta,
-                     double *C, size_t ldc, int lower, hipStream_t st);
+                     double *C, size_t ldc, int lower, hipStream_t st, const StrassenSet *set = nullptr);
 int strassen_plan(int m, int n, int k, int lower, long smin, long kslab, size_t scratch_doubles, std::vector<long long> &out);
 enum { PLAN2_SUM = 4, PLAN2_PROD = 5 };
 int strassen_outer_plan(int m, int n, int k, int lower, long smin, long kslab, long smin2, long kslab2, size_t scratch_doubles,
                    std::vector<long long> &out);
 int gemm_nt_multi(int m, int n, int k, const double *A, size_t lda, const double *B, size_t ldb, double beta, int count,
                   double *const *C, const size_t *ldc, const double *alpha, hipStream_t st);
-size_t strassen_scratch_doubles(int m, int n, int k, int lower, int levels);
-void strassen_reserve(size_t both, size_t one, hipStream_t st);
+void strassen_scratch_options(int m, int n, int k, int lower, size_t out[4], const StrassenSet *set = nullptr);
+int strassen_levels_of(int m, int n, int k, int lower, const StrassenSet *set = nullptr);
+void strassen_reserve(const size_t opt[4], hipStream_t st);
+int strassen_reserved(int dev, size_t *cap);
+int strassen_fuse_groups(const long long *recs, size_t nrec, int *out3);
+void strassen_sum_launches(long long out[2]);
+int potrf_products(int n, int la_max, const StrassenSet *set, std::vector<long long> &out);
+void potrf_scratch_options(int n, int la_max, const StrassenSet *set, size_t opt[4]);
 int strassen_trim();
 int gemm_profile_begin();
 int gemm_profile_end(double *out12);
diff --git a/sympgpr_amd/csrc/gemm_f64.hip b/sympgpr_amd/csrc/gemm_f64.hip
--- a/sympgpr_amd/csrc/gemm_f64.hip
+++ b/sympgpr_amd/csrc/gemm_f64.hip
@@ -101,6 +101,40 @@
         for (int u = 0; u < 4; ++u) {
             const int c = cg * 4 + u;
             if (c < cols) *reinterpret_cast<double2_t *>(T + (size_t)r + (size_t)c * (size_t)rows) = x[u] + sign * y[u];
+        }
+    }
+}
+
+template <int SIDE>
+__global__ __launch_bounds__(256) void block_sum5_kernel(int rows, int cols, const double *Q11, const double *Q12, const double *Q21,
+                                                         const double *Q22, size_t ld, double *T, size_t slot)
+{
+    const int nrc = (rows + 511) / 512, ncg = (cols + 3) / 4;
+    const long pieces = (long)nrc * ncg;
+    for (long p = blockIdx.x; p < pieces; p += gridDim.x) {
+        const int cg = (int)(p / nrc), rc = (int)(p - (long)cg * nrc);
+        const int r = rc * 512 + 2 * (int)threadIdx.x;
+        if (r >= rows) continue;
+        double2_t q11[4], q12[4], q21[4], q22[4];
+#pragma unroll
+        for (int u = 0; u < 4; ++u) {
+            const size_t o = (size_t)r + (size_t)min(cg * 4 + u, cols - 1) * ld;
+            q11[u] = *reinterpret_cast<const double2_t *>(Q11 + o);
+            q12[u] = *reinterpret_cast<const double2_t *>(Q12 + o);
+            q21[u] = *reinterpret_cast<const double2_t *>(Q21 + o);
+            q22[u] = *reinterpret_cast<const double2_t *>(Q22 + o);
+        }
+#pragma unroll
+        for (int u = 0; u < 4; ++u) {
+            const int c = cg * 4 + u;
+            if (c >= cols) continue;
+            double *t = T + (size_t)r + (size_t)c * (size_t)rows;
+            auto st = [&](int s, double2_t v) { *reinterpret_cast<double2_t *>(t + (size_t)s * slot) = v; };
+            if constexpr (SIDE == 0) {
+                st(0, q11[u] + q22[u]); st(1, q21[u] + q22[u]); st(2, q11[u] + q12[u]); st(3, q21[u] - q11[u]); st(4, q12[u] - q22[u]);
+            } else {
+                st(0, q11[u] + q22[u]); st(1, q21[u] - q22[u]); st(2, q12[u] - q11[u]); st(3, q11[u] + q21[u]); st(4, q12[u] + q22[u]);
+            }
         }
     }
 }
@@ -526,10 +560,52 @@
     return nd;
 }
 
+struct FuseRec {
+    int group = -1;
+    int sa = -1;
+    int sb = -1;
+};
+int fuse_match(const long long *recs, size_t nrec, int kinds, std::vector<FuseRec> &out)
+{
+    constexpr size_t G = 17;
+    out.assign(nrec, FuseRec{});
+    std::vector<long long> want;
+    int groups = 0;
+    for (size_t i = 0; i + G <= nrec;) {
+        const long long *r0 = recs + i * STRASSEN_REC, *r1 = r0 + STRASSEN_REC;
+        const bool inner = r0[0] == PLAN_SUM && (kinds & 1), outer = r0[0] == PLAN2_SUM && (kinds & 2);
+        bool ok = (inner || outer) && r1[0] == r0[0] && r0[1] == 0 && r1[1] == 1 && r0[2] > 0 && r0[3] > 0 && r1[2] > 0;
+        if (ok) {
+            want.clear();
+            seven((int)r0[0], inner ? PLAN_PROD : PLAN2_PROD, r0[2], r1[2], r0[3], r0[5], r0[4], r1[4], 0, 0, want);
+            for (size_t j = 0; ok && j < G; ++j) {
+                const long long *r = r0 + j * STRASSEN_REC, *w = &want[j * STRASSEN_REC];
+                const int words = (w[0] == r0[0]) ? STRASSEN_REC : 10;
+                for (int t = 0; ok && t < words; ++t) ok = r[t] == w[t];
+            }
+        }
+        if (!ok) { ++i; continue; }
+        int slot[2] = {-1, -1};
+        for (size_t j = 0; j < G; ++j) {
+            const long long *r = r0 + j * STRASSEN_REC;
+            FuseRec &f = out[i + j];
+            f.group = groups;
+            if (r[0] == r0[0]) (r[1] ? f.sb : f.sa) = ++slot[r[1]];
+            else { f.sa = r[1] ? slot[0] : -1; f.sb = r[4] ? slot[1] : -1; }
+        }
+        ++groups;
+        i += G;
+    }
+    return groups;
+}
+bool fuse_on() { static const bool on = tune("gemm_strassen_fuse", 1) != 0; return on; }
+int fuse_refused() { static const int v = (int)tune("gemm_strassen_fuse_noscratch", 0); return v; }
+
 struct Scratch {
     std::mutex mu;
     double *p = nullptr;
     size_t cap = 0, failed = 0;
+    int got = 0;
     hipEvent_t ev = nullptr;
     hipStream_t last = nullptr;
     bool used = false;
@@ -559,29 +635,56 @@
     return (dev >= 0 && dev < 64) ? dev : -1;
 }
 
+std::atomic<long long> g_sum_launches[2];
+
 int block_sum(int rows, int cols, const double *X, size_t ldx, const double *Y, size_t ldy, double sign, double *T, hipStream_t st)
 {
+    g_sum_launches[0].fetch_add(1, std::memory_order_relaxed);
     const long pieces = (long)((rows + 511) / 512) * ((cols + 3) / 4);
     hipLaunchKernelGGL(block_sum_kernel, dim3((unsigned)std::min(pieces, 2048L)), dim3(256), 0, st, rows, cols, X, ldx, Y, ldy, sign, T);
     SGPR_CHECK_LAUNCH();
     return 0;
 }
 
+int block_sum5(int side, const long long *s, const double *P, size_t ld, double *T, hipStream_t st)
+{
+    const int rows = (int)s[2], cols = (int)s[3];
+    const double *Q11 = P + s[4] + (size_t)s[5] * ld, *Q22 = P + s[6] + (size_t)s[7] * ld;
+    const double *Q12 = P + s[4] + (size_t)s[7] * ld, *Q21 = P + s[6] + (size_t)s[5] * ld;
+    const long pieces = (long)((rows + 511) / 512) * ((cols + 3) / 4);
+    const dim3 grid((unsigned)std::min(pieces, 2048L));
+    const size_t slot = (size_t)rows * (size_t)cols;
+    g_sum_launches[1].fetch_add(1, std::memory_order_relaxed);
+    if (side) hipLaunchKernelGGL(block_sum5_kernel<1>, grid, dim3(256), 0, st, rows, cols, Q11, Q12, Q21, Q22, ld, T, slot);
+    else      hipLaunchKernelGGL(block_sum5_kernel<0>, grid, dim3(256), 0, st, rows, cols, Q11, Q12, Q21, Q22, ld, T, slot);
+    SGPR_CHECK_LAUNCH();
+    return 0;
+}
+
 int run_plan(const long long *recs, size_t nrec, double alpha, const double *A, size_t lda, const double *B, size_t ldb,
-             double beta, double *C, size_t ldc, double alpha2, double *C2, size_t ldc2, double *SA, double *SB, hipStream_t st)
-{
+             double beta, double *C, size_t ldc, double alpha2, double *C2, size_t ldc2, double *SA, double *SB, bool five,
+             hipStream_t st)
+{
+    std::vector<FuseRec> fm;
+    if (five && nrec >= 17) (void)fuse_match(recs, nrec, 1, fm);
     for (size_t i = 0; i < nrec; ++i) {
         const long long *r = recs + i * STRASSEN_REC;
+        const FuseRec f = i < fm.size() ? fm[i] : FuseRec{};
         int rc = 0;
-        if (r[0] == PLAN_SUM) {
+        if (r[0] == PLAN_SUM && f.group >= 0) {
+            if (i == 0 || fm[i - 1].group != f.group) {
+                rc = block_sum5(0, r, A, lda, SA, st);
+                if (!rc) rc = block_sum5(1, r + STRASSEN_REC, B, ldb, SB, st);
+            }
+        } else if (r[0] == PLAN_SUM) {
             const double *P = r[1] ? B : A;
             const size_t ld = r[1] ? ldb : lda;
             rc = block_sum((int)r[2], (int)r[3], P + r[4] + (size_t)r[5] * ld, ld, P + r[6] + (size_t)r[7] * ld, ld, (double)r[8],
                            r[1] ? SB : SA, st);
         } else if (r[0] == PLAN_PROD) {
             const int m = (int)r[7], n = (int)r[8], k = (int)r[9];
-            const double *Ap = r[1] ? SA : A + r[2] + (size_t)r[3] * lda;
-            const double *Bp = r[4] ? SB : B + r[5] + (size_t)r[6] * ldb;
+            const double *Ap = r[1] ? SA + (size_t)std::max(f.sa, 0) * (size_t)m * (size_t)k : A + r[2] + (size_t)r[3] * lda;
+            const double *Bp = r[4] ? SB + (size_t)std::max(f.sb, 0) * (size_t)n * (size_t)k : B + r[5] + (size_t)r[6] * ldb;
             const size_t la = r[1] ? (size_t)m : lda, lb = r[4] ? (size_t)n : ldb;
             double *C1 = C + r[10] + (size_t)r[11] * ldc;
             if (C2) {
@@ -615,34 +718,47 @@
     return 0;
 }
 int run_plan(const std::vector<long long> &plan, double alpha, const double *A, size_t lda, const double *B, size_t ldb,
-             double beta, double *C, size_t ldc, double *SA, double *SB, hipStream_t st)
-{
-    return run_plan(plan.data(), plan.size() / STRASSEN_REC, alpha, A, lda, B, ldb, beta, C, ldc, 0.0, nullptr, 0, SA, SB, st);
+             double beta, double *C, size_t ldc, double *SA, double *SB, bool five, hipStream_t st)
+{
+    return run_plan(plan.data(), plan.size() / STRASSEN_REC, alpha, A, lda, B, ldb, beta, C, ldc, 0.0, nullptr, 0, SA, SB, five, st);
 }
 int run_plan2(const std::vector<long long> &plan, const Plan2Cfg &c, const Need2 &nd, double alpha, const double *A, size_t lda,
-              const double *B, size_t ldb, double beta, double *C, size_t ldc, double *S, hipStream_t st)
-{
-    double *const SA = S, *const SB = S + nd.v[0], *const OA = SB + nd.v[1], *const OB = OA + nd.v[2];
+              const double *B, size_t ldb, double beta, double *C, size_t ldc, double *S, bool in5, bool out5, hipStream_t st)
+{
+    const size_t na = in5 ? 5 : 1, no = out5 ? 5 : 1;
+    double *const SA = S, *const SB = SA + na * nd.v[0], *const OA = SB + na * nd.v[1], *const OB = OA + no * nd.v[2];
     PlanCfg ci = c.in;
     ci.scratch = nd.inner();
     std::vector<long long> in;
-    for (size_t i = 0; i + STRASSEN_REC <= plan.size(); i += STRASSEN_REC) {
-        const long long *r = &plan[i];
+    const size_t nrec = plan.size() / STRASSEN_REC;
+    std::vector<FuseRec> fm;
+    if (out5 && nrec >= 17) (void)fuse_match(plan.data(), nrec, 2, fm);
+    for (size_t i = 0; i < nrec; ++i) {
+        const long long *r = &plan[i * STRASSEN_REC];
+        const FuseRec f = i < fm.size() ? fm[i] : FuseRec{};
         int rc = 0;
-        if (r[0] == PLAN2_SUM) {
+        if (r[0] == PLAN2_SUM && f.group >= 0) {
+            if (i == 0 || fm[i - 1].group != f.group) {
+                rc = block_sum5(0, r, A, lda, OA, st);
+                if (!rc) rc = block_sum5(1, r + STRASSEN_REC, B, ldb, OB, st);
+            }
+        } else if (r[0] == PLAN2_SUM) {
             const double *P = r[1] ? B : A;
             const size_t ld = r[1] ? ldb : lda;
             rc = block_sum((int)r[2], (int)r[3], P + r[4] + (size_t)r[5] * ld, ld, P + r[6] + (size_t)r[7] * ld, ld, (double)r[8],
                            r[1] ? OB : OA, st);
         } else if (r[0] == PLAN2_PROD) {
-            const double *X = r[1] ? OA : A + r[2] + (size_t)r[3] * lda;
-            const double *Y = r[4] ? OB : B + r[5] + (size_t)r[6] * ldb;
+            const double *X = r[1] ? OA + (size_t)std::max(f.sa, 0) * (size_t)r[7] * (size_t)r[9] : A + r[2] + (size_t)r[3] * lda;
+            const double *Y = r[4] ? OB + (size_t)std::max(f.sb, 0) * (size_t)r[8] * (size_t)r[9] : B + r[5] + (size_t)r[6] * ldb;
             inner_plan(r, ci, in);
             rc = run_plan(in.data(), in.size() / STRASSEN_REC, alpha * (double)r[12], X, r[1] ? (size_t)r[7] : lda, Y, r[4] ? (size_t)r[8] : ldb,
                           1.0, C + r[10] + (size_t)r[11] * ldc, ldc, alpha * (double)r[15], r[15] ? C + r[13] + (size_t)r[14] * ldc : nullptr, ldc,
-                          SA, SB, st);
+                          SA, SB, in5, st);
         } else {
-            rc = run_plan(r, 1, alpha, A, lda, B, ldb, beta, C, ldc, 0.0, nullptr, 0, SA, SB, st);
+            size_t j = i + 1;
+            while (j < nrec && plan[j * STRASSEN_REC] != PLAN2_SUM && plan[j * STRASSEN_REC] != PLAN2_PROD) ++j;
+            rc = run_plan(r, j - i, alpha, A, lda, B, ldb, beta, C, ldc, 0.0, nullptr, 0, SA, SB, in5, st);
+            i = j - 1;
         }
         if (rc) return rc;
     }
@@ -687,26 +803,82 @@
     return 0;
 }
 
-size_t strassen_scratch_doubles(int m, int n, int k, int lower, int levels)
-{
+namespace {
+void apply_set(const StrassenSet *set, long k, Plan2Cfg &c)
+{
+    if (!set) return;
+    if (set->smin > 0) c.in.smin = std::min(c.in.smin, std::max(128L, set->smin));
+    if (set->smin2 > 0) c.smin2 = std::min(c.smin2, std::max(256L, set->smin2));
+    if (set->kslab2b >= 64 && set->kslab2b % 64 == 0 && set->kslab2b < c.kslab2 && k < c.kslab2 && k >= set->kslab2b) c.kslab2 = set->kslab2b;
+}
+}
+
+void strassen_scratch_options(int m, int n, int k, int lower, size_t out[4], const StrassenSet *set)
+{
+    out[0] = out[1] = out[2] = out[3] = 0;
+    if (!strassen_on()) return;
+    Plan2Cfg c = default_cfg2();
+    apply_set(set, k, c);
     std::vector<long long> plan;
-    if (!strassen_on()) return 0;
-    if (levels >= 2 && strassen_levels() >= 2) {
-        if (strassen_outer_plan(m, n, k, lower, -1, -1, -1, -1, ~(size_t)0, plan)) return 0;
-        return plan2_need(plan, default_cfg2()).total();
-    }
-    if (strassen_plan(m, n, k, lower, -1, -1, ~(size_t)0, plan)) return 0;
-    return plan_need(plan);
-}
-
-void strassen_reserve(size_t both, size_t one, hipStream_t st)
+    if (strassen_plan(m, n, k, lower, c.in.smin, c.in.kslab, ~(size_t)0, plan)) return;
+    out[3] = plan_need(plan);
+    out[2] = out[3];
+    out[0] = out[1] = 5 * out[3];
+    if (strassen_levels() < 2 || outer_noscratch()) return;
+    if (strassen_outer_plan(m, n, k, lower, c.in.smin, c.in.kslab, c.smin2, c.kslab2, ~(size_t)0, plan)) return;
+    const Need2 nd = plan2_need(plan, c);
+    out[2] = nd.total();
+    out[1] = 5 * nd.inner() + nd.v[2] + nd.v[3];
+    out[0] = 5 * nd.total();
+}
+int strassen_levels_of(int m, int n, int k, int lower, const StrassenSet *set)
+{
+    if (!strassen_on() || (lower && m != n)) return 0;
+    Plan2Cfg c = default_cfg2();
+    apply_set(set, k, c);
+    if (std::min(m, n) / 2 < c.in.smin) return 0;
+    std::vector<long long> plan;
+    if (strassen_levels() >= 2 && !strassen_outer_plan(m, n, k, lower, c.in.smin, c.in.kslab, c.smin2, c.kslab2, ~(size_t)0, plan))
+        for (size_t i = 0; i + STRASSEN_REC <= plan.size(); i += STRASSEN_REC)
+            if (plan[i] == PLAN2_PROD) return 2;
+    if (strassen_plan(m, n, k, lower, c.in.smin, c.in.kslab, ~(size_t)0, plan)) return 0;
+    for (size_t i = 0; i + STRASSEN_REC <= plan.size(); i += STRASSEN_REC)
+        if (plan[i] == PLAN_PROD) return 1;
+    return 0;
+}
+
+void strassen_reserve(const size_t opt[4], hipStream_t st)
 {
     const int dev = device_of(st);
     if (dev < 0 || !strassen_on()) return;
     Scratch &s = g_scratch[dev];
     std::lock_guard<std::mutex> lock(s.mu);
-    if (both > one && !outer_noscratch() && scratch_ensure(s, both)) return;
-    if (one) (void)scratch_ensure(s, one);
+    s.got = 0;
+    for (int i = 0; i < 4; ++i) {
+        if (!opt[i]) continue;
+        if (i < 2 && (!fuse_on() || fuse_refused() == 1 || (i == 0 && fuse_refused()))) continue;
+        if (scratch_ensure(s, opt[i])) { s.got = i + 1; return; }
+    }
+}
+int strassen_reserved(int dev, size_t *cap)
+{
+    if (dev < 0 || dev >= 64) return 0;
+    Scratch &s = g_scratch[dev];
+    std::lock_guard<std::mutex> lock(s.mu);
+    if (cap) *cap = s.cap;
+    return s.got;
+}
+void strassen_sum_launches(long long out[2])
+{
+    out[0] = g_sum_launches[0].load(std::memory_order_relaxed);
+    out[1] = g_sum_launches[1].load(std::memory_order_relaxed);
+}
+int strassen_fuse_groups(const long long *recs, size_t nrec, int *out3)
+{
+    std::vector<FuseRec> fm;
+    const int groups = fuse_match(recs, nrec, 3, fm);
+    for (size_t i = 0; i < nrec; ++i) { out3[3 * i] = fm[i].group; out3[3 * i + 1] = fm[i].sa; out3[3 * i + 2] = fm[i].sb; }
+    return groups;
 }
 
 int strassen_trim()
@@ -715,17 +887,20 @@
         std::lock_guard<std::mutex> lock(s.mu);
         if (s.p) (void)hipFree(s.p);
         if (s.ev) (void)hipEventDestroy(s.ev);
-        s.p = nullptr; s.ev = nullptr; s.cap = 0; s.failed = 0; s.used = false; s.last = nullptr;
+        s.p = nullptr; s.ev = nullptr; s.cap = 0; s.failed = 0; s.used = false; s.last = nullptr; s.got = 0;
     }
     (void)hipGetLastError();
     return 0;
 }
 
 int gemm_nt_strassen(int m, int n, int k, double alpha, const double *A, size_t lda, const double *B, size_t ldb, double beta,
-                     double *C, size_t ldc, int lower, hipStream_t st)
+                     double *C, size_t ldc, int lower, hipStream_t st, const StrassenSet *set)
 {
     const bool aligned = ((((uintptr_t)A | (uintptr_t)B) & 15) == 0) && (((lda | ldb) & 1) == 0);
-    if (std::min(m, n) / 2 < default_cfg().smin || !strassen_on() || !aligned || beta != 1.0 || (lower && m != n))
+    Plan2Cfg c2 = default_cfg2();
+    apply_set(set, k, c2);
+    const PlanCfg &c1 = c2.in;
+    if (std::min(m, n) / 2 < c1.smin || !strassen_on() || !aligned || beta != 1.0 || (lower && m != n))
         return gemm_nt(m, n, k, alpha, A, lda, B, ldb, beta, C, ldc, lower, 0, st);
     std::vector<long long> plan;
     int rc = 0;
@@ -739,32 +914,36 @@
         s.used = true;
         return r;
     };
-    const Plan2Cfg c2 = default_cfg2();
     if (strassen_levels() >= 2 && dev >= 0 && !outer_noscratch() && std::min(lower ? m / 2 : m, lower ? n / 2 : n) / 2 >= c2.smin2) {
-        if ((rc = strassen_outer_plan(m, n, k, lower, -1, -1, -1, -1, ~(size_t)0, plan))) return rc;
+        if ((rc = strassen_outer_plan(m, n, k, lower, c1.smin, c1.kslab, c2.smin2, c2.kslab2, ~(size_t)0, plan))) return rc;
         const Need2 nd = plan2_need(plan, c2);
         if (nd.v[2] + nd.v[3]) {
             Scratch &s = g_scratch[dev];
             std::lock_guard<std::mutex> lock(s.mu);
-            if (scratch_ensure(s, nd.total()))
-                return enqueue(s, [&] { return run_plan2(plan, c2, nd, alpha, A, lda, B, ldb, beta, C, ldc, s.p, st); });
-        }
-    }
-    rc = strassen_plan(m, n, k, lower, -1, -1, ~(size_t)0, plan);
+            const bool f5 = fuse_on() && fuse_refused() != 1;
+            bool in5 = f5, out5 = f5 && !fuse_refused();
+            if (!(out5 && scratch_ensure(s, 5 * nd.total()))) out5 = false;
+            if (!out5 && !(in5 && scratch_ensure(s, 5 * nd.inner() + nd.v[2] + nd.v[3]))) in5 = false;
+            if (in5 || scratch_ensure(s, nd.total()))
+                return enqueue(s, [&] { return run_plan2(plan, c2, nd, alpha, A, lda, B, ldb, beta, C, ldc, s.p, in5, out5, st); });
+        }
+    }
+    rc = strassen_plan(m, n, k, lower, c1.smin, c1.kslab, ~(size_t)0, plan);
     if (rc) return rc;
     const size_t need = plan_need(plan);
-    if (!need) return run_plan(plan, alpha, A, lda, B, ldb, beta, C, ldc, nullptr, nullptr, st);
+    if (!need) return run_plan(plan, alpha, A, lda, B, ldb, beta, C, ldc, nullptr, nullptr, false, st);
     if (dev < 0) return gemm_nt(m, n, k, alpha, A, lda, B, ldb, beta, C, ldc, lower, 0, st);
     Scratch &s = g_scratch[dev];
     std::lock_guard<std::mutex> lock(s.mu);
-    if (!scratch_ensure(s, need)) {
-        if ((rc = strassen_plan(m, n, k, lower, -1, -1, s.cap, plan))) return rc;
-        if (!plan_need(plan)) return run_plan(plan, alpha, A, lda, B, ldb, beta, C, ldc, nullptr, nullptr, st);
+    const bool five = fuse_on() && fuse_refused() != 1 && scratch_ensure(s, 5 * need);
+    if (!five && !scratch_ensure(s, need)) {
+        if ((rc = strassen_plan(m, n, k, lower, c1.smin, c1.kslab, s.cap, plan))) return rc;
+        if (!plan_need(plan)) return run_plan(plan, alpha, A, lda, B, ldb, beta, C, ldc, nullptr, nullptr, false, st);
     }
     size_t na = 0;
     for (size_t i = 0; i + STRASSEN_REC <= plan.size(); i += STRASSEN_REC)
         if (plan[i] == PLAN_SUM && plan[i + 1] == 0) na = std::max(na, (size_t)plan[i + 2] * (size_t)plan[i + 3]);
-    return enqueue(s, [&] { return run_plan(plan, alpha, A, lda, B, ldb, beta, C, ldc, s.p, s.p + na, st); });
-}
-
-}
+    return enqueue(s, [&] { return run_plan(plan, alpha, A, lda, B, ldb, beta, C, ldc, s.p, s.p + (five ? 5 : 1) * na, five, st); });
+}
+
+}
diff --git a/sympgpr_amd/csrc/probe.hip b/sympgpr_amd/csrc/probe.hip
--- a/sympgpr_amd/csrc/probe.hip
+++ b/sympgpr_amd/csrc/probe.hip
@@ -539,6 +539,53 @@
 {
     return gemm_nt_multi(m, n, k, A, lda, B, ldb, beta, count, C, ldc, alpha, static_cast<hipStream_t>(stream));
 }
+extern "C" int sgpr_probe_strassen_fuse_groups(const long long *recs, int nrec, int *out3, int *groups)
+{
+    if (!recs || nrec < 0 || !out3 || !groups) { set_error("probe_strassen_fuse_groups: bad arguments"); return SGPR_E_ARG; }
+    *groups = strassen_fuse_groups(recs, (size_t)nrec, out3);
+    return 0;
+}
+static const StrassenSet *probe_set(long smin, long smin2, long kslab2b, StrassenSet &v)
+{
+    if (smin < 0 && smin2 < 0 && kslab2b < 0) return nullptr;
+    v.smin = std::max(smin, 0L); v.smin2 = std::max(smin2, 0L); v.kslab2b = std::max(kslab2b, 0L);
+    return &v;
+}
+extern "C" int sgpr_probe_potrf_scratch(int n, int la_max, long smin, long smin2, long kslab2b, long long out[4])
+{
+    if (n < 2 || !out) { set_error("probe_potrf_scratch: bad arguments"); return SGPR_E_ARG; }
+    size_t opt[4];
+    StrassenSet v;
+    potrf_scratch_options(n, la_max, probe_set(smin, smin2, kslab2b, v), opt);
+    for (int i = 0; i < 4; ++i) out[i] = (long long)opt[i];
+    return 0;
+}
+extern "C" int sgpr_probe_potrf_products(int n, int la_max, long smin, long smin2, long kslab2b, long long *out, int max_products,
+                                         int *count)
+{
+    if (!count) { set_error("probe_potrf_products: bad arguments"); return SGPR_E_ARG; }
+    std::vector<long long> list;
+    StrassenSet v;
+    const int rc = potrf_products(n, la_max, probe_set(smin, smin2, kslab2b, v), list);
+    if (rc) return rc;
+    *count = (int)(list.size() / 5);
+    for (size_t i = 0; out && i < list.size() && (int)(i / 5) < max_products; ++i) out[i] = list[i];
+    return 0;
+}
+extern "C" int sgpr_probe_strassen_sum_launches(long long out[2])
+{
+    if (!out) { set_error("probe_strassen_sum_launches: bad arguments"); return SGPR_E_ARG; }
+    strassen_sum_launches(out);
+    return 0;
+}
+extern "C" int sgpr_probe_strassen_reserved(int dev, long long out[2])
+{
+    if (!out) { set_error("probe_strassen_reserved: bad arguments"); return SGPR_E_ARG; }
+    size_t cap = 0;
+    out[1] = strassen_reserved(dev, &cap);
+    out[0] = (long long)cap;
+    return 0;
+}
 extern "C" unsigned sgpr_probe_map_calls(void) { return applymap_last_calls(); }
 extern "C" int sgpr_probe_map_team(int ntest, int n0) { return applymap_team(ntest, n0); }
 extern "C" int sgpr_probe_trsm_piece(int ticket, int cap, int strips, int out[5]) { if (ticket < 0 || cap < 1 || strips < 0 || !out) return SGPR_E_ARG; trsm_piece_of(ticket, cap, strips, out); return 0; }
```

After: 79.52, median of 6. About the same (+0.7%).
